# amoretti86/phylo

Measured on AMD Instinct MI355X. Metric: particle-site-likelihoods/sec, higher is better.
Workload: dtype f64; 1 GPU; primate.p N=12 S=898, GTR-init (jcmodel=false), K=2048 per GPU (K_total=2048), lambda=10, full sweep of 11 rank events; parallelism=particles sharded over 1 GPU(s), global resampling, sweeps_per_launch_set=16, contexts_in_flight=3, sweeps_in_flight=48, particles_in_flight=98304

## Files before the change

include/phylo_hip.h:

```cpp
#ifndef PHYLO_HIP_H
#define PHYLO_HIP_H

#include <stdint.h>

#ifdef __cplusplus
extern "C" {
#endif

typedef struct phylo_ctx phylo_ctx;

enum {
    PHYLO_OK = 0,
    PHYLO_EINVAL = -1,
    PHYLO_ENODEVICE = -2,
    PHYLO_EHIP = -3,
    PHYLO_ENOMEM = -4,
    PHYLO_ECOMM = -5,
    PHYLO_ESTATE = -6
};

enum {
    PHYLO_QUIRK_Q1_RAW_Q = 1u << 0,
    PHYLO_TWISTING = 1u << 1,
    PHYLO_TIME_KERNELS = 1u << 2,
// ... 31 lines not shown
                    const double* lam_r, int jc69_closed_form);

int phylo_expm_batched(phylo_ctx* ctx, const double* t, int n, double* P_nx4x4);

int phylo_cond_likelihood_K(phylo_ctx* ctx, const double* l_KxSx4, const double* r_KxSx4,
                            const double* tl_K, const double* tr_K, int K, int S, double* out_KxSx4);

int phylo_forest_loglik(phylo_ctx* ctx, const double* core_KxXxSx4, const int32_t* record_KxX, int K,
                        int X, int S, double* out_K);

int phylo_tree_loglik(phylo_ctx* ctx, int n_nodes, int n_leaves, int S, const int32_t* left,
                      const int32_t* right, const double* bl, const double* br, int root,
                      const double* leaves_LxSx4, const double* prior4, double* out_loglik,
                      double* root_data_Sx4);

int phylo_trees_loglik(phylo_ctx* ctx, int T, const int32_t* child, const double* blen, const double* prior4, double* loglik_T,
                       double* site_lik_TxS, phylo_stats* perf);
int phylo_trees_loglik_rates(phylo_ctx* ctx, int T, const int32_t* child, const double* blen, int C, const double* rate_C,
                             const double* weight_C, const double* prior4, double* loglik_T, double* site_lik_TxS,
                             double* cat_lik_TxCxS, phylo_stats* perf);
int phylo_trees_grad(phylo_ctx* ctx, int T, const int32_t* child, const double* blen, const double* prior4, double* loglik_T,
                     double* grad, double* curv, phylo_stats* perf);
int phylo_trees_grad_rates(phylo_ctx* ctx, int T, const int32_t* child, const double* blen, int C, const double* rate,
                           const double* weight, int per_tree, const double* prior4, double* loglik_T, double* grad, double* curv,
                           double* drate_TxC, double* dweight_TxC, phylo_stats* perf);
int phylo_trees_nni(phylo_ctx* ctx, int T, const int32_t* child, const double* blen, const double* prior4, double* loglik_T,
                    double* delta, phylo_stats* perf);
int phylo_trees_nni_rates(phylo_ctx* ctx, int T, const int32_t* child, const double* blen, int C, const double* rate,
                          const double* weight, int per_tree, const double* prior4, double* loglik_T, double* delta, phylo_stats* perf);
int phylo_debug_tree_schedule(int N, const int32_t* child, const double* blen, int32_t* ops, int32_t* depth);

int phylo_resample(phylo_ctx* ctx, const double* logw_K, int K, uint64_t seed, uint32_t step,
                   int64_t* idx_K);

int phylo_log_zsmc(phylo_ctx* ctx, const double* logw_RxK, int R, int K, double* out);

int phylo_sweep(phylo_ctx* ctx, uint64_t seed, uint32_t flags, int M, double* log_weights,
                double* log_lik, double* lbranch, double* rbranch, int32_t* merges, int64_t* ancestors,
                double* logZ, phylo_stats* perf);

int phylo_sweep_async(phylo_ctx* ctx, uint64_t seed, uint32_t flags, int M);
int phylo_sweep_fetch(phylo_ctx* ctx, double* log_weights, double* log_lik, double* lbranch,
                      double* rbranch, int32_t* merges, int64_t* ancestors, double* logZ,
                      phylo_stats* perf);
int phylo_synchronize(phylo_ctx* ctx);

int phylo_sweep_batch_async(phylo_ctx* ctx, const uint64_t* seeds, int G, uint32_t flags);
int phylo_sweep_batch_begin(phylo_ctx* ctx, const uint64_t* seeds, int G, uint32_t flags);
int phylo_sweep_fetch_logz(phylo_ctx* ctx, double* logZ_G, int G);

int phylo_sweep_begin(phylo_ctx* ctx, uint64_t seed, uint32_t flags, int M);
int phylo_sweep_step(phylo_ctx* ctx);
int phylo_sweep_step_a(phylo_ctx* ctx);
int phylo_sweep_step_group(phylo_ctx** ctxs, int n);
int phylo_sweep_finish(phylo_ctx* ctx);

int phylo_sweep_node(phylo_ctx* ctx, int r, int k, double* out_Sx4);

int phylo_sweep_backward(phylo_ctx* ctx, double* d_lam_l, double* d_lam_r, double* d_pi, double* d_Q,
                         phylo_stats* perf);
int phylo_sweep_backward_batch(phylo_ctx* ctx, double* d_lam_l, double* d_lam_r, double* d_pi, double* d_Q, int G,
                               phylo_stats* perf);

int phylo_vi_gradients(phylo_ctx* ctx, uint64_t seed, uint32_t flags, int M, int jc, const double* vars, double* logZ, double* grads,
                       phylo_stats* fwd, phylo_stats* bwd);
int phylo_vi_gradients_batch(phylo_ctx* ctx, const uint64_t* seeds, int G, uint32_t flags, int jc, const double* vars, double* logZ,
                             double* grads, phylo_stats* fwd, phylo_stats* bwd);
int phylo_vi_apply(int n_taxa, int jc, double* vars, const double* grads, int kind, double lr, double beta1, double beta2, double eps,
                   int64_t* t, double* m, double* v);

int phylo_debug_stamps(phylo_ctx* ctx, uint64_t* out, int n);

int phylo_debug_reverse_lists(int N, int K, const int64_t* ancestors, const int32_t* child, int early_free, int rows_form,
                              const int32_t* lookahead_nodes, int n_lookahead, int32_t* lists, int64_t n_lists, int32_t* meta,
                              int n_meta);

int phylo_debug_lookahead_lists(int N, int K, int S, int M, const int32_t* roots_ad, int32_t* slow_flag, int32_t* image,
                                int64_t n_image, int32_t* meta, int n_meta);

int phylo_debug_reverse_plan(int N, int K, int K_local, int S, int world, int twisted, int marks, uint32_t switches, int64_t n_slow,
                             int TS, int64_t coeff_wgs, int passes_in_flight, uint32_t* mask);
int phylo_debug_sweep_plan(int N, int K, int K_local, int S, int G, int M, int world, int transport, uint32_t flags, uint32_t switches,
                           uint32_t* mask, int32_t* launches);
int phylo_debug_scan_form(phylo_ctx* ctx, int Kg, int multi_min, int wanted);
int phylo_debug_persist_plan(int N, int K, int S, int G, uint32_t flags, uint32_t switches, int world, int transport, int n_cus,
                             int blocks_per_cu, int persist_wgs, int persist_nt, int64_t* out);
int phylo_debug_persist_of(phylo_ctx* ctx, int32_t* nt, int32_t* Wg, int32_t* m, int64_t* lds);
int phylo_debug_pack_leaf_codes(const uint8_t* codes, int N, int S, uint8_t* packed, int64_t cap, int64_t* need);
int phylo_debug_site_patterns(const uint8_t* codes, int N, int S, int32_t* U, int32_t* rep, uint16_t* image, uint32_t* rep_off,
                              uint8_t* rep_leaf, int64_t rep_leaf_cap);
int phylo_debug_site_patterns_rule(int S, int U, int coded, int ntiles, int sw);
int phylo_debug_site_patterns_of(phylo_ctx* ctx, int32_t* U, int32_t* taken);
int phylo_debug_reverse_plan_batch(int N, int K, int G, int S, uint32_t switches, int64_t n_slow, int TS, int64_t coeff_wgs,
                                   int passes_in_flight, uint32_t* mask);
int phylo_debug_tree_plan(int N, int K, int G, int world, int64_t n_clades, int64_t n_topologies, int kept_whole, int force_wide,
                          int64_t summary_temp, int64_t branches_temp, int64_t* scalars, int64_t* summary_slab, int64_t* branches_slab,
                          int32_t* sort_bits, int32_t* launches);
int phylo_debug_tree_branches_of(phylo_ctx* ctx, int32_t* wide, int32_t* cbits, int32_t* tbits);

int phylo_debug_device_lists(phylo_ctx* ctx, int32_t* lists, int64_t n_lists, int32_t* meta, int n_meta, int64_t* ancestors,
                             int32_t* child);
int phylo_debug_device_lists_of(phylo_ctx* ctx, const int64_t* ancestors, const int32_t* child, int32_t* lists, int64_t n_lists,
                                int32_t* meta, int n_meta);

int phylo_tree_summary(phylo_ctx* ctx, int64_t* n_clades, int32_t* n_topologies, int32_t* n_groups, phylo_stats* perf);
int phylo_tree_summary_fetch(phylo_ctx* ctx, uint64_t* clade_bits, uint64_t* clade_weight, int32_t* clade_group, uint64_t* topo_weight,
                             int32_t* topo_count, int32_t* topo_rep, int32_t* topo_group, int32_t* particle_topo, uint64_t* u, uint64_t* U);

int phylo_tree_branches(phylo_ctx* ctx, phylo_stats* perf);
int phylo_tree_branches_fetch(phylo_ctx* ctx, double* clade_stats, double* leaf_stats, int32_t* topo_clades, double* topo_stats);

int phylo_rell(phylo_ctx* ctx, int T, int S, const double* site_lik_TxS, int B, uint64_t seed, double* obs_T, int32_t* best_B,
               int64_t* wins_T, double* rep_loglik_TxB, int32_t* counts_BxS, double* site_loglik_TxS, phylo_stats* perf);
int phylo_debug_rell_host(int T, int S, const double* site_lik_TxS, int b0, int nB, uint64_t seed, int32_t* counts, double* x,
                          double* rl);

int phylo_math_probe(phylo_ctx* ctx, int op, const double* x, const double* y, int n, double* out);

int phylo_debug_frechet(phylo_ctx* ctx, int form, const double* A_nx16, const double* E_nx16, int n, double* L_nx16);

int phylo_debug_site_product(phylo_ctx* ctx, const double* p, const double* x1, const double* x2, int n, double* out_p, int32_t* out_E,
                             double* out_extra);

#define PHYLO_COMM_ID_BYTES 128
int phylo_comm_unique_id(char id[PHYLO_COMM_ID_BYTES]);
int phylo_comm_init(phylo_ctx* ctx, int rank, int world, const char id[PHYLO_COMM_ID_BYTES]);
int phylo_comm_share(phylo_ctx* ctx, phylo_ctx* owner);
int phylo_comm_allgather(phylo_ctx* ctx, const void* mine, size_t bytes, void* all);
int phylo_comm_max(phylo_ctx* ctx, double* value);
int phylo_comm_barrier(phylo_ctx* ctx);
int phylo_comm_exchange_kind(const phylo_ctx* ctx);
int phylo_debug_remote_cache(phylo_ctx* ctx, int* used, int* cap);

#ifdef __cplusplus
}
#endif
#endif
```

phylo_amd/_ffi.py:

```python
from __future__ import annotations

import ctypes as C
import os

import numpy as np

_HERE = os.path.dirname(os.path.abspath(__file__))
LIB_PATH = os.path.join(_HERE, "csrc", "libphylo_hip.so")

PHYLO_OK = 0
QUIRK_Q1_RAW_Q = 1 << 0
TWISTING = 1 << 1
TIME_KERNELS = 1 << 2
EAGER_NODES = 1 << 3
KEEP_GRAPH = 1 << 4
ONE_LAUNCH = 1 << 5
FLAGS_DEFAULT = QUIRK_Q1_RAW_Q
COMM_ID_BYTES = 128

EXPORTS = [
    "phylo_version", "phylo_last_error", "phylo_device_count", "phylo_create", "phylo_destroy",
    "phylo_set_leaves", "phylo_set_model", "phylo_expm_batched", "phylo_cond_likelihood_K",
    "phylo_forest_loglik", "phylo_tree_loglik", "phylo_trees_loglik", "phylo_trees_loglik_rates", "phylo_trees_grad", "phylo_trees_grad_rates", "phylo_trees_nni", "phylo_trees_nni_rates", "phylo_rell", "phylo_debug_rell_host", "phylo_debug_tree_schedule", "phylo_resample", "phylo_log_zsmc", "phylo_sweep",
    "phylo_sweep_async", "phylo_sweep_batch_async", "phylo_sweep_batch_begin", "phylo_sweep_fetch_logz", "phylo_sweep_begin", "phylo_sweep_step", "phylo_sweep_step_a", "phylo_sweep_step_group", "phylo_sweep_finish", "phylo_sweep_fetch",
    "phylo_synchronize", "phylo_sweep_node", "phylo_sweep_backward", "phylo_sweep_backward_batch",
    "phylo_tree_summary", "phylo_tree_summary_fetch", "phylo_tree_branches", "phylo_tree_branches_fetch",
    "phylo_math_probe", "phylo_debug_frechet", "phylo_debug_stamps", "phylo_debug_reverse_lists", "phylo_debug_lookahead_lists", "phylo_debug_reverse_plan", "phylo_debug_reverse_plan_batch", "phylo_debug_sweep_plan", "phylo_debug_pack_leaf_codes", "phylo_debug_site_patterns", "phylo_debug_site_patterns_rule", "phylo_debug_site_patterns_of", "phylo_debug_tree_plan", "phylo_debug_tree_branches_of", "phylo_debug_scan_form", "phylo_debug_persist_plan", "phylo_debug_persist_of", "phylo_debug_device_lists", "phylo_debug_device_lists_of", "phylo_debug_remote_cache", "phylo_debug_site_product",
    "phylo_vi_gradients", "phylo_vi_gradients_batch", "phylo_vi_apply",
    "phylo_site_tile", "phylo_set_site_tile", "phylo_get_site_tile",
    "phylo_comm_unique_id", "phylo_comm_init", "phylo_comm_share", "phylo_comm_allgather", "phylo_comm_max", "phylo_comm_barrier",
    "phylo_comm_exchange_kind",
]


class PhyloError(RuntimeError):
    def __init__(self, code, msg):
        super().__init__("libphylo_hip error %d: %s" % (code, msg))
        self.code = code


class Stats(C.Structure):
    _fields_ = [("sweep_ms", C.c_double), ("merge_ms", C.c_double), ("merge_launches", C.c_int32),
                ("n_launches", C.c_int32), ("units", C.c_double), ("alg_bytes", C.c_double)]


_lib = None


def load():
    global _lib
    if _lib is None:
        if not os.path.exists(LIB_PATH):
            raise OSError("%s not found: build it with phylo_amd/csrc/build.sh (needs hipcc); "
                          "there is no CPU fallback" % LIB_PATH)
        lib = C.CDLL(LIB_PATH)
        lib.phylo_version.restype = C.c_char_p
        lib.phylo_last_error.restype = C.c_char_p
        lib.phylo_last_error.argtypes = [C.c_void_p]
        _lib = lib
    return _lib


def _ptr(a):
    return None if a is None else a.ctypes.data_as(C.c_void_p)


def _f64(a):
    return np.ascontiguousarray(a, dtype=np.float64)


def debug_reverse_lists(N, K, ancestors, child, early_free=True, rows_form=True, lookahead_nodes=None):
    lib = load()
    R = N - 1
    nn = R * K
    cap = 2 * nn // 4 + 1
    n_lists = R * (K + 1) + 9 * nn + 1 + 2 * cap
    lists = np.zeros(n_lists, dtype=np.int32)
    meta = np.zeros(6 + 3 * (R + 1), dtype=np.int32)
    anc = None if R < 2 else np.ascontiguousarray(ancestors, dtype=np.int64)
    ch = np.ascontiguousarray(child, dtype=np.int32)
    la = None if lookahead_nodes is None or len(lookahead_nodes) == 0 else np.ascontiguousarray(lookahead_nodes, dtype=np.int32)
    rc = lib.phylo_debug_reverse_lists(C.c_int(N), C.c_int(K), _ptr(anc), _ptr(ch), C.c_int(int(early_free)), C.c_int(int(rows_form)),
                                       _ptr(la), C.c_int(0 if la is None else la.size), _ptr(lists), C.c_int64(n_lists), _ptr(meta),
                                       C.c_int(meta.size))
    if rc:
        raise PhyloError(rc, lib.phylo_last_error(None).decode())
    return _lists_dict(lists, meta, R, K)


def debug_lookahead_lists(N, K, S, M, roots_ad, slow_flag=None):
    lib = load()
    R = N - 1
    rad = np.ascontiguousarray(roots_ad, dtype=np.int32)
    if rad.shape != (R, K, N):
        raise ValueError("roots_ad must be [N-1][K][N]")
    flag = np.zeros(R * K, dtype=np.int32) if slow_flag is None else np.array(slow_flag, dtype=np.int32).reshape(R * K)
    n_image = R * (8 * K * N + 8192) + 1
    image = np.zeros(n_image, dtype=np.int32)
    meta = np.zeros(4 + 2 * (R + 1), dtype=np.int32)
    rc = lib.phylo_debug_lookahead_lists(C.c_int(N), C.c_int(K), C.c_int(S), C.c_int(M), _ptr(rad), _ptr(flag), _ptr(image),
                                         C.c_int64(n_image), _ptr(meta), C.c_int(meta.size))
    if rc:
        raise PhyloError(rc, lib.phylo_last_error(None).decode())
    ne, nc, nx = int(meta[0]), int(meta[1]), int(meta[2])
    out = {"n_xent": ne, "n_xchunks": nc, "n_xnodes": nx, "tw_max_chunks": int(meta[3]), "slow_flag": flag,
           "ev_chunk0": meta[4:4 + R + 1].copy(), "ev_node0": meta[4 + R + 1:4 + 2 * (R + 1)].copy()}
    o = 0
    for name, n in (("xent", ne), ("xchunk_node", nc), ("xchunk_beg", nc), ("xchunk_cnt", nc), ("xchunk_part", nc), ("xnode_id", nx),
                    ("xnode_chunk0", nx), ("xnode_nchunks", nx)):
        out[name] = image[o:o + n].copy()
        o += n
    return out


PLAN_BITS = ("rows_form", "whole", "early_free", "dev_lists", "sort_early", "bg_free", "two", "parents_first", "rows_all", "rows_overlap",
             "chunks_first", "interleave", "coeff_all")
PLAN_SWITCHES = ("rev_host_lists", "one_stream", "two_streams", "rows_chain", "coeff_chain")


def debug_reverse_plan(N, K, S, K_local=None, world=1, twisted=False, marks=True, switches=(), n_slow=0, TS=None, coeff_wgs=0,
                       passes_in_flight=1):
    lib = load()
    sw = sum(1 << PLAN_SWITCHES.index(name) for name in switches)
    mask = C.c_uint32(0)
    rc = lib.phylo_debug_reverse_plan(C.c_int(N), C.c_int(K), C.c_int(K if K_local is None else K_local), C.c_int(S), C.c_int(world),
                                      C.c_int(int(twisted)), C.c_int(int(marks)), C.c_uint32(sw), C.c_int64(n_slow),
                                      C.c_int((S + 255) // 256 if TS is None else TS), C.c_int64(coeff_wgs), C.c_int(passes_in_flight),
                                      C.byref(mask))
    if rc:
        raise PhyloError(rc, lib.phylo_last_error(None).decode())
    out = {name: bool(mask.value >> i & 1) for i, name in enumerate(PLAN_BITS)}
    out["mask"] = mask.value
    return out


SWEEP_PLAN_BITS = ("twist", "graph", "timek", "lazy", "shard_form", "replicated_book", "local_book", "book_mat", "mat_by_draws", "want_rdraw",
                   "use_rec", "sorted_prologue", "mat_grouped", "mat_draws_grouped", "step_a_work", "mat_after_book", "mat_barrier",
                   "fix_rootll", "fold_logz", "no_store_last", "final_missing", "last_graph_eager", "one_tile", "twist_ll", "twist_tables",
                   "tile_epilogue", "batched")
SWEEP_PLAN_SWITCHES = ("eager_nodes", "rehearse_sharded", "replicated_book", "jc", "coded_leaves", "device_exchange")


def debug_sweep_plan(N, K, S, K_local=None, G=1, M=1, world=1, transport=False, flags=0, switches=()):
    lib = load()
    sw = sum(1 << SWEEP_PLAN_SWITCHES.index(name) for name in switches)
    mask = C.c_uint32(0)
    launches = (C.c_int32 * (max(N, 1) + 1))()
    rc = lib.phylo_debug_sweep_plan(C.c_int(N), C.c_int(K), C.c_int(K if K_local is None else K_local), C.c_int(S), C.c_int(G), C.c_int(M),
                                    C.c_int(world), C.c_int(int(transport)), C.c_uint32(flags), C.c_uint32(sw), C.byref(mask), launches)
    if rc:
        raise PhyloError(rc, lib.phylo_last_error(None).decode())
    out = {name: bool(mask.value >> i & 1) for i, name in enumerate(SWEEP_PLAN_BITS)}
    out["book_width"] = (mask.value >> 28) * 8
    out["mask"] = mask.value
    out["launches"] = list(launches)
    return out


def debug_pack_leaf_codes(codes):
    lib = load()
    cd = np.ascontiguousarray(codes, dtype=np.uint8)
    if cd.ndim != 2:
        raise ValueError("codes must be [N][S]")
    N, S = cd.shape
    need = C.c_int64(0)
    rc = lib.phylo_debug_pack_leaf_codes(_ptr(cd), C.c_int(N), C.c_int(S), None, C.c_int64(0), C.byref(need))
    if rc:
        raise PhyloError(rc, lib.phylo_last_error(None).decode())
    out = np.full(need.value, 0xff, dtype=np.uint8)
    rc = lib.phylo_debug_pack_leaf_codes(_ptr(cd), C.c_int(N), C.c_int(S), _ptr(out), C.c_int64(out.size), C.byref(need))
    if rc:
        raise PhyloError(rc, lib.phylo_last_error(None).decode())
    return out.reshape(N, -1, 64, 16)


SITE_PATTERN_SWITCH = {"0": 0, None: 1, "force": 2}


def debug_site_patterns(codes):
    lib = load()
    cd = np.ascontiguousarray(codes, dtype=np.uint8)
    if cd.ndim != 2:
        raise ValueError("codes must be [N][S]")
    N, S = cd.shape
    nC = -(-(-(-S // 64)) // 16)
    U = C.c_int32(0)
    rep = np.full(S, -1, dtype=np.int32)
    image = np.full(nC * 1024, 0xffff, dtype=np.uint16)
    rep_off = np.full(1024, 0xffffffff, dtype=np.uint32)
    rep_leaf = np.full(N * 1024, 0xff, dtype=np.uint8)
    rc = lib.phylo_debug_site_patterns(_ptr(cd), C.c_int(N), C.c_int(S), C.byref(U), _ptr(rep), _ptr(image), _ptr(rep_off), _ptr(rep_leaf),
                                       C.c_int64(rep_leaf.size))
    if rc:
        raise PhyloError(rc, lib.phylo_last_error(None).decode())
    u = U.value
    return {"U": u, "rep": rep[:u].copy(), "image": image.reshape(nC, 2, 64, 8) if u <= 8191 else None,
            "rep_off": rep_off if u <= 512 else None,
            "rep_leaf": rep_leaf[:N * 1024 * (-(-(-(-u // 64)) // 16))].reshape(N, -1, 64, 16) if u <= 512 else None}


def debug_site_patterns_rule(S, U, coded=True, ntiles=1, switch=None):
    lib = load()
    rc = lib.phylo_debug_site_patterns_rule(C.c_int(S), C.c_int(U), C.c_int(int(coded)), C.c_int(ntiles), C.c_int(SITE_PATTERN_SWITCH[switch]))
    if rc < 0:
        raise PhyloError(rc, lib.phylo_last_error(None).decode())
    return bool(rc)


TREE_SUMMARY_BUFS = ("u", "U", "bits", "kA", "kB", "val", "scan", "weight", "srt", "hp", "o_cbits", "o_cw", "o_tw", "child", "slot", "o_cg",
                     "o_tn", "o_trep", "o_tg", "o_ptopo", "vA", "vB", "flag", "sid", "cid", "seg_start", "count", "group", "first", "tid", "pos",
                     "err", "vC", "vD", "temp")
TREE_BRANCHES_BUFS = ("ebr", "lbr", "gbl", "gbr", "o_cs", "o_ls", "o_ts", "wA", "wB", "cpos", "kA", "kB", "vA", "vB", "cstart", "toff", "o_tc",
                      "temp")


def debug_tree_plan(N, K, G=1, world=1, n_clades=1, n_topologies=1, kept_whole=False, summary_temp=0, branches_temp=0, force_wide=False):
    lib = load()
    ns, nb = len(TREE_SUMMARY_BUFS), len(TREE_BRANCHES_BUFS)
    sc = (C.c_int64 * 13)()
    ss, bs = (C.c_int64 * (2 * ns + 1))(), (C.c_int64 * (2 * nb + 1))()
    bits, launches = (C.c_int32 * 17)(), (C.c_int32 * 2)()
    rc = lib.phylo_debug_tree_plan(C.c_int(N), C.c_int(K), C.c_int(G), C.c_int(world), C.c_int64(n_clades), C.c_int64(n_topologies),
                                   C.c_int(int(kept_whole)), C.c_int(int(force_wide)), C.c_int64(summary_temp), C.c_int64(branches_temp),
                                   sc, ss, bs, bits, launches)
    if rc:
        raise PhyloError(rc, lib.phylo_last_error(None).decode())
    out = dict(zip(("R", "L", "W", "E", "Emax", "Kg", "cbits", "tbits"), sc[:8]))
    out["wide"], out["gather"] = bool(sc[8]), bool(sc[9])
    if (sc[11], sc[12]) != (ns, nb):
        raise RuntimeError("TREE_SUMMARY_BUFS / TREE_BRANCHES_BUFS do not name the library's buffers")
    for key, names, a in (("summary_slab", TREE_SUMMARY_BUFS, ss), ("branches_slab", TREE_BRANCHES_BUFS, bs)):
        n = len(names)
        out[key] = {"offsets": dict(zip(names, a[:n])), "sizes": dict(zip(names, a[n:2 * n])), "total": a[2 * n]}
    out["sort_bits"] = list(bits[:sc[10]])
    out["summary_launches"], out["branches_launches"] = launches[0], launches[1]
    return out


SCAN_FORMS = ("multi", "lds512", "lds1024", "in_place")
# ... 539 lines not shown
                                                       _ptr(z), _ptr(grads), C.byref(fwd), C.byref(bwd)))
        self._last_batch = G
        return z, grads, fwd, bwd

    def debug_device_lists(self, ancestors=None, child=None):
        R, K = self.N - 1, self.K
        nn = R * K
        cap = 2 * nn // 4 + 1
        n_lists = R * (K + 1) + 9 * nn + 1 + 2 * cap
        lists = np.zeros(n_lists, dtype=np.int32)
        meta = np.zeros(6 + 3 * (R + 1), dtype=np.int32)
        if child is not None:
            anc = np.ascontiguousarray(ancestors if R > 1 else np.zeros((0, K)), dtype=np.int64).reshape(max(R - 1, 0), K)
            child = np.ascontiguousarray(child, dtype=np.int32).reshape(R, K, 2)
            self._check(self._lib.phylo_debug_device_lists_of(self._h, _ptr(anc) if R > 1 else None, _ptr(child), _ptr(lists),
                                                              C.c_int64(n_lists), _ptr(meta), C.c_int(meta.size)))
        else:
            anc = np.zeros((max(R - 1, 0), K), dtype=np.int64)
            child = np.zeros((R, K, 2), dtype=np.int32)
            self._check(self._lib.phylo_debug_device_lists(self._h, _ptr(lists), C.c_int64(n_lists), _ptr(meta), C.c_int(meta.size),
                                                           _ptr(anc) if R > 1 else None, _ptr(child)))
        out = _lists_dict(lists, meta, R, K)
        out['ancestors'] = anc
        out['child'] = child
        return out

    def debug_stamps(self):
        out = np.zeros((self.N, 16), dtype=np.uint64)
        self._check(self._lib.phylo_debug_stamps(self._h, _ptr(out), C.c_int(out.size)))
        return out

    def comm_init(self, rank, world, comm_id):
        buf = C.create_string_buffer(bytes(comm_id), COMM_ID_BYTES)
        self._check(self._lib.phylo_comm_init(self._h, C.c_int(rank), C.c_int(world), buf))
        self.K_local = self.K // world
        self.k0 = rank * self.K_local

    def comm_share(self, owner):
        self._check(self._lib.phylo_comm_share(self._h, owner._h))
        self._owner = owner
        world = owner.K // owner.K_local
        self.K_local = self.K // world
        self.k0 = (owner.k0 // owner.K_local) * self.K_local

    def comm_allgather_columns(self, a):
        a = np.ascontiguousarray(a)
        world = self.K // self.K_local
        if world == 1:
            return a
        out = np.empty((world,) + a.shape, dtype=a.dtype)
        self._check(self._lib.phylo_comm_allgather(self._h, _ptr(a), C.c_size_t(a.nbytes), _ptr(out)))
        return np.concatenate(list(out), axis=-1)

    def comm_allgather_blob(self, a):
        a = np.ascontiguousarray(a)
        world = self.K // self.K_local
        if world == 1:
            return a[None]
        out = np.empty((world,) + a.shape, dtype=a.dtype)
        self._check(self._lib.phylo_comm_allgather(self._h, _ptr(a), C.c_size_t(a.nbytes), _ptr(out)))
        return out

    def debug_remote_cache(self):
        used, cap = C.c_int(0), C.c_int(0)
        self._check(self._lib.phylo_debug_remote_cache(self._h, C.byref(used), C.byref(cap)))
        return used.value, cap.value

    def debug_site_patterns(self):
        U, taken = C.c_int32(0), C.c_int32(0)
        self._check(self._lib.phylo_debug_site_patterns_of(self._h, C.byref(U), C.byref(taken)))
        return U.value, bool(taken.value)

    def debug_tree_branches(self):
        wide, cbits, tbits = C.c_int32(0), C.c_int32(0), C.c_int32(0)
        self._check(self._lib.phylo_debug_tree_branches_of(self._h, C.byref(wide), C.byref(cbits), C.byref(tbits)))
        return {'wide': bool(wide.value), 'cbits': cbits.value, 'tbits': tbits.value}

    def debug_scan_form(self, Kg, wanted=True):
        rc = self._lib.phylo_debug_scan_form(self._h, C.c_int(Kg), C.c_int(0), C.c_int(int(wanted)))
        if rc < 0:
            raise PhyloError(rc, self._lib.phylo_last_error(self._h).decode())
        return SCAN_FORMS[rc]

    def debug_persist(self):
        nt, Wg, m, lds = C.c_int32(0), C.c_int32(0), C.c_int32(0), C.c_int64(0)
        self._check(self._lib.phylo_debug_persist_of(self._h, C.byref(nt), C.byref(Wg), C.byref(m), C.byref(lds)))
        return {'nt': nt.value, 'Wg': Wg.value, 'm': m.value, 'lds': lds.value}

    def comm_exchange_kind(self):
        return ('none', 'rccl', 'hostshm', 'p2p')[int(self._lib.phylo_comm_exchange_kind(self._h))]

    def comm_max(self, value):
        v = C.c_double(float(value))
        self._check(self._lib.phylo_comm_max(self._h, C.byref(v)))
        return v.value

    def comm_barrier(self):
        self._check(self._lib.phylo_comm_barrier(self._h))


def sweep_step_group(ctxs):
    arr = (C.c_void_p * len(ctxs))(*[c._h for c in ctxs])
    rc = load().phylo_sweep_step_group(arr, C.c_int(len(ctxs)))
    if rc != PHYLO_OK:
        raise PhyloError(rc, (load().phylo_last_error(None) or b"").decode())


def comm_unique_id():
    buf = C.create_string_buffer(COMM_ID_BYTES)
    rc = load().phylo_comm_unique_id(buf)
    if rc != PHYLO_OK:
        raise PhyloError(rc, (load().phylo_last_error(None) or b"").decode())
    return buf.raw
```

phylo_amd/csrc/phylo_hip.hip:

```cpp
#include "../../include/phylo_hip.h"

#include <cstring>
#include <hip/hip_runtime.h>
#include <hip/hip_ext.h>
#include <rocprim/device/device_radix_sort.hpp>

#include <cstdarg>
#include <cstdio>
#include <cstdlib>
#include <atomic>
#include <chrono>
#include <mutex>
#include <string>
#include <vector>

#include "phylo_comm.h"
#include "phylo_kernels.h"
#include "phylo_packed_codes.h"
#include "phylo_site_patterns.h"
#include "phylo_persist.h"
#include "phylo_grad.h"
#include "phylo_revlists_dev.h"
#include "phylo_sweep_plan.h"
#include "phylo_train.h"
#include "phylo_trees.h"
#include "phylo_trees_plan.h"
#include "phylo_treeset.h"
#include "phylo_rell.h"
#include "phylo_treegrad.h"
#include "phylo_treegrad_rates.h"
#include "phylo_treenni.h"
#include "phylo_treenni_rates.h"

#include <algorithm>
#include <type_traits>

namespace {

thread_local std::string g_last_error;

struct DevBuf {
    void* p = nullptr;
    size_t bytes = 0;
};

}

struct sweep_run {
    uint64_t seed = 0;
    uint32_t flags = 0;
    int M = 1, launches = 0, next_r = 0;
    bool active = false;
    int a_done_r = -1;
    sweep_plan plan{};
};

struct env_switches {
    bool eager_nodes = false, rehearse_sharded = false, replicated_book = false, no_leaf_codes = false, one_launch = false,
         persist_stamps = false, grad_one_stream = false, grad_two_streams = false, rev_host_lists = false, no_remote_cache = false,
         no_p2p = false, grad_rows_chain = false, grad_coeff_chain = false, tree_wide_keys = false;
    int persist_wgs = 0;
    unsigned long long p2p_wait_ticks = PK_P2P_WAIT_TICKS;
    size_t p2p_copy_words = 65536;
    int persist_nt = 256;
    int remote_cache_cap = 0;
    int scan_multi_min = 4096;
    int site_patterns = PK_PAT_AUTO;
    int trees_chunk = 0;
    int rell_chunk = 0;
    void read() {
        eager_nodes = getenv("PHYLO_EAGER_NODES") != nullptr;
        rehearse_sharded = getenv("PHYLO_REHEARSE_SHARDED") != nullptr;
        replicated_book = getenv("PHYLO_REPLICATED_BOOK") != nullptr;
        grad_rows_chain = getenv("PHYLO_GRAD_ROWS_CHAIN") != nullptr;
        grad_coeff_chain = getenv("PHYLO_GRAD_COEFF_CHAIN") != nullptr;
        no_leaf_codes = getenv("PHYLO_NO_LEAF_CODES") != nullptr;
        one_launch = getenv("PHYLO_ONE_LAUNCH") != nullptr;
        persist_stamps = getenv("PHYLO_PERSIST_STAMPS") != nullptr;
        grad_one_stream = getenv("PHYLO_GRAD_ONE_STREAM") != nullptr;
        grad_two_streams = getenv("PHYLO_GRAD_TWO_STREAMS") != nullptr;
        rev_host_lists = getenv("PHYLO_REV_HOST_LISTS") != nullptr;
        no_remote_cache = getenv("PHYLO_NO_REMOTE_CACHE") != nullptr;
        { const char* e = getenv("PHYLO_TREE_WIDE_KEYS"); tree_wide_keys = e && atoi(e) != 0; }
        { const char* e = getenv("PHYLO_REMOTE_CACHE_CAP"); remote_cache_cap = e ? atoi(e) : 0; }
        { const char* e = getenv("PHYLO_SITE_PATTERNS"); site_patterns = !e ? PK_PAT_AUTO : !strcmp(e, "force") ? PK_PAT_FORCE : atoi(e) == 0 ? PK_PAT_OFF : PK_PAT_AUTO; }
        { const char* e = getenv("PHYLO_SCAN_MULTI_MIN"); scan_multi_min = e ? atoi(e) : 4096; }
        { const char* e = getenv("PHYLO_TREES_CHUNK"); trees_chunk = e ? atoi(e) : 0; }
        { const char* e = getenv("PHYLO_RELL_CHUNK"); rell_chunk = e ? atoi(e) : 0; }
        { const char* e = getenv("PHYLO_P2P"); no_p2p = e && atoi(e) == 0; }
        { const char* e = getenv("PHYLO_P2P_COPY_WORDS"); p2p_copy_words = e ? (size_t)atol(e) : 65536; }
        { const char* e = getenv("PHYLO_P2P_WAIT_S"); p2p_wait_ticks = e && atof(e) > 0 ? (unsigned long long)(atof(e) * 1e8) : PK_P2P_WAIT_TICKS; }
        const char* w = getenv("PHYLO_PERSIST_WGS");
        persist_wgs = w ? atoi(w) : 0;
        const char* t = getenv("PHYLO_PERSIST_NT");
        persist_nt = persist_nt_of(t ? atoi(t) : 0);
    }
};

struct phylo_ctx {
    int device = 0;
    env_switches env;
    int n_cus = 0;
    unsigned long long* d_rdraw = nullptr;
    unsigned long long* d_pctr = nullptr;
    unsigned long long pctr_base = 0;
    int pctr_Wg = 0, pctr_G = 0;
    bool pctr_dirty = false;
    int persist_blocks_per_cu = -1;
    bool last_persistent = false;
    int last_pp_nt = 0, last_pp_Wg = 0, last_pp_m = 0;
    size_t last_pp_lds = 0;
    unsigned long long* d_stamps = nullptr;
    int K = 0, N = 0, S = 0, A = 4;
    int Kloc = 0, k0 = 0;
    int rank = 0, world = 1;
    uint32_t flags = 0;
    hipStream_t stream = nullptr;
    hipEvent_t ev0 = nullptr, ev1 = nullptr;
    std::vector<hipEvent_t> kev;
    std::string err;
    bool have_leaves = false, have_model = false, swept = false, state_ready = false;
    int jc = 0;
    std::vector<double> h_lam_l, h_lam_r, h_ldf;
    double *d_Q = nullptr, *d_pi = nullptr, *d_lam_l = nullptr, *d_lam_r = nullptr, *d_ldf = nullptr;
    double* d_leaves = nullptr;
    uint8_t* d_leaf_codes = nullptr;
    uint8_t* d_leaf_packed = nullptr;
    uint8_t* d_pat = nullptr;
    int pat_U = 0;
    bool leaves_coded = false;
    uint32_t* d_pair_hist = nullptr;
    bool hist_ready = false, codes_valid = false;
    double* d_pool = nullptr;
    double* d_nodell = nullptr;
    double *d_bl = nullptr, *d_br = nullptr, *d_Pmat = nullptr;
    double *d_logw = nullptr, *d_ll = nullptr;
    double* d_aux = nullptr;
    unsigned long long* d_rec = nullptr;
    int tile_override = 0;
    int site_tile = 0, ntiles = 1;
    double* d_tilev = nullptr;
    double* d_lse = nullptr;
    uint64_t* d_group_seeds = nullptr;
    char* d_tables = nullptr;
    int32_t *d_roots[2] = {nullptr, nullptr}, *d_cnt[2] = {nullptr, nullptr};
    double* d_rootll[2] = {nullptr, nullptr};
    const char** d_tab_ptrs = nullptr;
    int32_t* d_child = nullptr;
    unsigned int* d_mark = nullptr;
    double* d_sync = nullptr;
    bool p2p = false;
    char* d_xslab = nullptr;
    size_t xslab_bytes = 0, x_flag_off[2] = {0, 0};
    char** d_xslab_ptrs = nullptr;
    unsigned long long x_epoch[2] = {0, 0};
    bool last_lazy = false;
    bool leaves_newer = false;
    int32_t* d_merges = nullptr;
    int64_t* d_anc = nullptr;
    uint64_t* d_cdf[2] = {nullptr, nullptr};
    unsigned int* d_counter = nullptr;
    const double** d_pool_ptrs = nullptr;
    int32_t* d_mirror = nullptr;
    double* d_cache = nullptr;
    int cache_cap = 0;
    int32_t *d_roots_ad = nullptr, *d_cnt_ad = nullptr;
    double *d_rootll_ad = nullptr, *d_chosen = nullptr, *d_tw_b = nullptr, *d_tw_P = nullptr, *d_pot = nullptr;
    size_t tw_capacity = 0;
    double* d_twbuf = nullptr;
    size_t twbuf_cap = 0;
    double *d_htw_b = nullptr, *d_htw_P = nullptr, *d_hpot = nullptr, *d_hchosen = nullptr;
    int32_t* d_hroots_ad = nullptr;
    double *d_tau = nullptr, *d_ctw = nullptr, *d_twpart = nullptr, *d_twnode = nullptr;
    int64_t* d_joff = nullptr;
    size_t htw_rows = 0;
    std::vector<int64_t> h_joff;
    bool last_graph_twist = false, last_graph_marks = false;
    bool last_graph_eager = false;
    int last_M = 1;
    int32_t *d_hroots = nullptr, *d_hcnt = nullptr, *d_pos = nullptr;
    double* d_hrootll = nullptr;
    double *d_adj = nullptr, *d_om = nullptr, *d_G = nullptr, *d_C = nullptr, *d_part = nullptr, *d_nodeg = nullptr;
    double *d_leafpi = nullptr, *d_leafterm = nullptr, *d_terms = nullptr, *d_gout = nullptr;
    int32_t *d_ad_off = nullptr, *d_ad_idx = nullptr, *d_par_off = nullptr, *d_par_idx = nullptr;
    int32_t *d_heavy = nullptr, *d_chunk_beg = nullptr, *d_chunk_cnt = nullptr;
    int32_t *d_slow_flag = nullptr, *d_slow_idx = nullptr, *d_adp = nullptr;
    bool graph_ready = false, last_graph = false;
    int last_G = 1;
    bool last_final_missing = false;
    std::vector<uint64_t> h_group_seeds;
    int64_t* h_anc_p = nullptr;
    std::vector<int64_t> h_anc_glob;
    std::vector<double> h_gout;
    double* h_model_p = nullptr;
    double* h_leaves_p = nullptr;
    hipEvent_t ev_leaves = nullptr;
    uint32_t *h_pub = nullptr, *hd_pub = nullptr;
    int32_t *h_dlmeta = nullptr, *hd_dlmeta = nullptr;
    const int32_t* d_dlmeta = nullptr;
    unsigned int* d_row_done = nullptr;
    unsigned int row_epoch = 0;
    hipEvent_t ev_dl = nullptr;
    size_t dl_temp_p = 0, dl_temp_nn = 0;
    hipGraphExec_t dl_graph = nullptr;
    const void* dl_graph_key[4] = {nullptr, nullptr, nullptr, nullptr};
    bool dl_no_graph = false;
    uint32_t *hd_csr = nullptr, *hd_anc = nullptr, *hd_child = nullptr, *hd_rad = nullptr;
    int32_t *h_child_p = nullptr, *h_rad_p = nullptr, *h_csr_p = nullptr;
    size_t h_csr_cap = 0;
    hipEvent_t ev_gcopy = nullptr;
    std::vector<int32_t> h_cur;
    std::vector<double> h_vi_lam;
    std::vector<double> h_vi_raw;
    int32_t* d_gchild = nullptr;
    double *d_gbl = nullptr, *d_gbr = nullptr, *d_gPmat = nullptr;
    int64_t* d_ganc = nullptr;
    unsigned long long* d_gx = nullptr;
    const unsigned long long** d_gx_src = nullptr;
    size_t gx_seg = 0, gx_cl = 0;
    std::vector<int32_t> h_xlists;
    hipEvent_t evb0 = nullptr, evb1 = nullptr, ev_model = nullptr;
    hipStream_t gstream = nullptr;
    hipEvent_t ev_gfork = nullptr, ev_gjoin = nullptr, ev_gup = nullptr;
    hipStream_t bgstream = nullptr;
    hipEvent_t ev_bgfork = nullptr, ev_bgdone = nullptr;
    std::vector<hipEvent_t> ev_coeff;
    phylo_stats stats{};
    sweep_run run;
    int n_merge_events = 0;
    DevBuf scratch[20];
    phylo_comm comm;
    pt_bufs ts;
    bool ts_done = false;
    int ts_G = 1, ts_nt = 0;
    long long ts_nc = 0;
    hipEvent_t ev_ts0 = nullptr, ev_ts1 = nullptr;
    pb_bufs tb;
    bool tb_done = false;
    int tb_wide = -1, tb_cbits = 0, tb_tbits = 0;
    unsigned long long sweep_serial = 0, ts_serial = 0;
    hipEvent_t ev_tb0 = nullptr, ev_tb1 = nullptr;
    hipEvent_t ev_tl0 = nullptr, ev_tl1 = nullptr;
    hipEvent_t ev_rl0 = nullptr, ev_rl1 = nullptr;
// ... 67 lines not shown
}

int launch_check(phylo_ctx* ctx, const char* what) {
    hipError_t e = hipGetLastError();
    if (e != hipSuccess) return fail(ctx, PHYLO_EHIP, "launch of %s failed: %s", what, hipGetErrorString(e));
    return PHYLO_OK;
}

void free_sweep_state(phylo_ctx* c) {
    if (c->gstream) (void)hipStreamSynchronize(c->gstream);
    if (c->bgstream) (void)hipStreamSynchronize(c->bgstream);
    if (c->d_xslab) {
        (void)hipFree(c->d_xslab);
        c->d_xslab = nullptr;
        c->d_logw = c->d_ll = c->d_nodell = c->d_sync = nullptr;
        c->d_chosen = nullptr;
    }
    if (c->d_xslab_ptrs) (void)hipFree((void*)c->d_xslab_ptrs);
    c->d_xslab_ptrs = nullptr;
    c->xslab_bytes = 0;
    c->x_epoch[0] = c->x_epoch[1] = 0;
    if (c->d_twbuf) (void)hipFree(c->d_twbuf);
    c->d_twbuf = nullptr;
    c->twbuf_cap = 0;
    void* tw[] = {c->d_roots_ad, c->d_cnt_ad, c->d_rootll_ad, c->d_chosen, c->d_tw_b, c->d_tw_P, c->d_pot};
    for (void* p : tw)
        if (p) (void)hipFree(p);
    c->d_roots_ad = c->d_cnt_ad = nullptr;
    c->d_rootll_ad = c->d_chosen = c->d_tw_b = c->d_tw_P = c->d_pot = nullptr;
    c->tw_capacity = 0;
    void* ht[] = {c->d_htw_b, c->d_htw_P, c->d_hpot, c->d_hchosen, c->d_hroots_ad, c->d_tau, c->d_ctw, c->d_twpart, c->d_twnode, c->d_joff};
    for (void* p : ht)
        if (p) (void)hipFree(p);
    c->d_htw_b = c->d_htw_P = c->d_hpot = c->d_hchosen = c->d_tau = c->d_ctw = c->d_twpart = c->d_twnode = nullptr;
    c->d_hroots_ad = nullptr;
    c->d_joff = nullptr;
    c->htw_rows = 0;
    c->last_graph_twist = false;
    void* gr[] = {c->d_hroots, c->d_hcnt, c->d_pos, c->d_hrootll, c->d_adj, c->d_om, c->d_G, c->d_C, c->d_part, c->d_nodeg,
                  c->d_leafpi, c->d_leafterm, c->d_terms, c->d_gout, c->d_ad_off, c->d_gchild, c->d_gbl, c->d_gbr, c->d_gPmat,
                  c->d_ganc, c->d_gx, (void*)c->d_gx_src};
    for (void* p : gr)
        if (p) (void)hipFree(p);
    c->d_hroots = c->d_hcnt = c->d_pos = nullptr;
    c->d_hrootll = c->d_adj = c->d_om = c->d_G = c->d_C = c->d_part = c->d_nodeg = nullptr;
    c->d_leafpi = c->d_leafterm = c->d_terms = c->d_gout = nullptr;
    c->d_gchild = nullptr; c->d_gbl = c->d_gbr = c->d_gPmat = nullptr; c->d_ganc = nullptr;
    c->d_gx = nullptr; c->d_gx_src = nullptr; c->gx_seg = c->gx_cl = 0;
    c->d_ad_off = c->d_ad_idx = c->d_par_off = c->d_par_idx = nullptr;
    c->d_heavy = c->d_chunk_beg = c->d_chunk_cnt = nullptr;
    c->d_slow_flag = c->d_slow_idx = c->d_adp = nullptr;
    if (c->h_csr_p) (void)hipHostFree(c->h_csr_p);
    if (c->h_anc_p) (void)hipHostFree(c->h_anc_p);
    if (c->h_child_p) (void)hipHostFree(c->h_child_p);
    if (c->h_rad_p) (void)hipHostFree(c->h_rad_p);
    if (c->h_pub) (void)hipHostFree(c->h_pub);
    if (c->d_row_done) (void)hipFree(c->d_row_done);
    c->d_row_done = nullptr;
    if (c->h_dlmeta) (void)hipHostFree(c->h_dlmeta);
    c->h_dlmeta = c->hd_dlmeta = nullptr;
    if (c->ev_dl) (void)hipEventDestroy(c->ev_dl);
    c->ev_dl = nullptr;
    if (c->dl_graph) (void)hipGraphExecDestroy(c->dl_graph);
    c->dl_graph = nullptr;
    c->h_pub = c->hd_pub = nullptr;
    c->h_csr_p = c->h_child_p = c->h_rad_p = nullptr;
    c->h_anc_p = nullptr;
    if (c->ev_gcopy) (void)hipEventDestroy(c->ev_gcopy);
    c->ev_gcopy = nullptr;
    c->graph_ready = false;
    c->last_graph = false;
    if (c->d_stamps) (void)hipFree(c->d_stamps);
    c->d_stamps = nullptr;
    if (c->d_rdraw) (void)hipFree(c->d_rdraw);
    if (c->d_pctr) (void)hipFree(c->d_pctr);
    c->d_rdraw = c->d_pctr = nullptr;
    c->pctr_base = 0;
    c->pctr_Wg = c->pctr_G = 0;
    c->pctr_dirty = false;
    if (c->d_tilev) (void)hipFree(c->d_tilev);
    c->d_tilev = nullptr;
    void* ptrs[] = {c->d_pool, c->d_nodell, c->d_bl, c->d_br, c->d_Pmat, c->d_logw, c->d_ll, c->d_aux, c->d_lse, c->d_group_seeds,
                    c->d_tables, (void*)c->d_tab_ptrs, c->d_child, c->d_merges, c->d_anc,
                    c->d_cdf[0], c->d_cdf[1], c->d_counter, (void*)c->d_pool_ptrs, c->d_mark, c->d_sync, c->d_mirror, c->d_cache, c->d_rec};
    for (void* p : ptrs)
        if (p) (void)hipFree(p);
    c->d_pool = c->d_nodell = c->d_bl = c->d_br = c->d_Pmat = c->d_logw = c->d_ll = c->d_aux = c->d_lse = nullptr;
    c->d_group_seeds = nullptr;
    c->d_rec = nullptr;
    c->d_roots[0] = c->d_roots[1] = c->d_cnt[0] = c->d_cnt[1] = c->d_child = c->d_merges = nullptr;
    c->d_anc = nullptr;
    c->d_cdf[0] = c->d_cdf[1] = nullptr;
    c->d_counter = nullptr;
    c->d_rootll[0] = c->d_rootll[1] = nullptr;
    c->d_tables = nullptr;
    c->d_tab_ptrs = nullptr;
    c->d_pool_ptrs = nullptr;
    c->d_mark = nullptr;
    c->d_sync = nullptr;
    c->d_mirror = nullptr;
    c->d_cache = nullptr;
    c->cache_cap = 0;
}

int alloc_sweep_state(phylo_ctx* c) {
    free_sweep_state(c);
    c->state_ready = false;
    const size_t R = (size_t)c->N - 1, K = c->K, Kl = c->Kloc, N = c->N, S = c->S;
    CHK(dalloc(c, &c->d_pool, R * Kl * S * 4));
    c->p2p = c->comm.transport != 0 && c->world > 1 && !c->env.no_p2p && R >= 2;
    if (c->p2p) {
        const size_t al = 32;
        auto up = [&](size_t n) { return (n + al - 1) / al * al; };
        const size_t n_logw = up(R * K), n_nod = up(N + R * K), n_ch = up(K), n_sy = up((size_t)c->world), n_fl = up((size_t)c->world);
        const size_t total = 2 * n_logw + n_nod + n_ch + n_sy + 2 * n_fl;
        void* slab = nullptr;
        if (hipExtMallocWithFlags(&slab, total * 8, hipDeviceMallocFinegrained) != hipSuccess) {
            (void)hipGetLastError();
            HIPCHK(c, hipMalloc(&slab, total * 8));
        }
        HIPCHK(c, hipMemset(slab, 0, total * 8));
        c->d_xslab = (char*)slab;
        c->xslab_bytes = total * 8;
        double* base = (double*)slab;
        c->d_logw = base; c->d_ll = base + n_logw; c->d_nodell = base + 2 * n_logw;
        c->d_chosen = c->d_nodell + n_nod;
        c->d_sync = c->d_chosen + n_ch;
        c->x_flag_off[0] = (size_t)((char*)(c->d_sync + n_sy) - c->d_xslab);
        c->x_flag_off[1] = c->x_flag_off[0] + n_fl * 8;
        c->x_epoch[0] = c->x_epoch[1] = 0;
    } else {
    CHK(dalloc(c, &c->d_nodell, N + R * K));
    }
    CHK(dalloc(c, &c->d_bl, R * Kl));
    CHK(dalloc(c, &c->d_br, R * Kl));
    CHK(dalloc(c, &c->d_Pmat, R * Kl * 32));
    if (!c->p2p) {
        CHK(dalloc(c, &c->d_logw, R * K));
        CHK(dalloc(c, &c->d_ll, R * K));
    }
    CHK(dalloc(c, &c->d_aux, Kl * PK_AUX));
    CHK(dalloc(c, &c->d_rec, Kl * PK_REC));
    if (c->ntiles > 1) CHK(dalloc(c, &c->d_tilev, Kl * (size_t)c->ntiles));
    CHK(dalloc(c, &c->d_lse, (R + 1) * PK_MAX_GROUPS));
    CHK(dalloc(c, &c->d_group_seeds, PK_MAX_GROUPS));
    CHK(dalloc(c, &c->d_tables, 32 * K * N));
    for (int i = 0; i < 2; ++i) {
        c->d_rootll[i] = reinterpret_cast<double*>(c->d_tables) + (size_t)i * K * N;
        c->d_roots[i] = reinterpret_cast<int32_t*>(c->d_tables + 16 * K * N) + (size_t)i * K * N;
        c->d_cnt[i] = reinterpret_cast<int32_t*>(c->d_tables + 24 * K * N) + (size_t)i * K * N;
    }
    CHK(dalloc(c, &c->d_child, R * Kl * 2));
    CHK(dalloc(c, &c->d_mark, ((R * K + R + 3) & ~(size_t)3)));
    if (!c->p2p) CHK(dalloc(c, &c->d_sync, (size_t)c->world));
    CHK(dalloc(c, &c->d_merges, R * Kl * 2));
    CHK(dalloc(c, &c->d_anc, (R > 0 ? R - 1 : 0) * Kl));
    CHK(dalloc(c, &c->d_cdf[0], K));
    CHK(dalloc(c, &c->d_cdf[1], K));
    CHK(dalloc(c, &c->d_counter, ((size_t)N + 3) & ~(size_t)3));
    HIPCHK(c, hipMemset(c->d_counter, 0, (((size_t)N + 3) & ~(size_t)3) * sizeof(unsigned int)));
    CHK(dalloc(c, &c->d_pool_ptrs, (size_t)c->world));
    std::vector<void*> ptrs;
    int rc = phylo_comm_map_pools(c->comm, c->d_pool, &ptrs, c->stream, &c->err);
    if (rc != PHYLO_OK) return rc;
    HIPCHK(c, hipMemcpy((void*)c->d_pool_ptrs, ptrs.data(), ptrs.size() * sizeof(void*), hipMemcpyHostToDevice));
    if ((c->world > 1 || c->env.rehearse_sharded) && !c->env.no_remote_cache) {
        const size_t node_bytes = (size_t)S * 32;
        size_t cap = ((size_t)512 << 20) / node_bytes;
        if (c->env.remote_cache_cap > 0) cap = (size_t)c->env.remote_cache_cap;
        if (cap > R * K) cap = R * K;
        if (cap < 1) cap = 1;
        c->cache_cap = (int)cap;
        CHK(dalloc(c, &c->d_mirror, R * K + 4));
        CHK(dalloc(c, &c->d_cache, cap * (size_t)S * 4));
    }
    CHK(dalloc(c, &c->d_tab_ptrs, (size_t)c->world));
    rc = phylo_comm_map_extra(c->comm, c->d_tables, &ptrs, c->stream, &c->err);
    if (rc != PHYLO_OK) return rc;
    HIPCHK(c, hipMemcpy((void*)c->d_tab_ptrs, ptrs.data(), ptrs.size() * sizeof(void*), hipMemcpyHostToDevice));
    if (c->p2p) {
        CHK(dalloc(c, &c->d_xslab_ptrs, (size_t)c->world));
        rc = phylo_comm_map_extra(c->comm, c->d_xslab, &ptrs, c->stream, &c->err);
        if (rc != PHYLO_OK) return rc;
        HIPCHK(c, hipMemcpy((void*)c->d_xslab_ptrs, ptrs.data(), ptrs.size() * sizeof(void*), hipMemcpyHostToDevice));
    }
    c->state_ready = true;
    return PHYLO_OK;
}

int ensure_sweep_state(phylo_ctx* c) {
    if (c->state_ready) return PHYLO_OK;
    return alloc_sweep_state(c);
}

int ensure_graph_state(phylo_ctx* c) {
    if (c->graph_ready) return PHYLO_OK;
    const size_t R = (size_t)c->N - 1, K = c->K, N = c->N, S = c->S;
    const size_t T = (S + PG_NT - 1) / PG_NT;
    CHK(dalloc(c, &c->d_hroots, (R + 1) * K * N));
    CHK(dalloc(c, &c->d_hcnt, (R + 1) * K * N));
    CHK(dalloc(c, &c->d_hrootll, (R + 1) * K * N));
    CHK(dalloc(c, &c->d_pos, R * K * N));
    CHK(dalloc(c, &c->d_adj, R * K * S * 4));
    CHK(dalloc(c, &c->d_om, R * K));
    CHK(dalloc(c, &c->d_G, R * K));
    CHK(dalloc(c, &c->d_C, R * K * N));
    CHK(dalloc(c, &c->d_part, R * K * T * PG_PART));
    CHK(dalloc(c, &c->d_nodeg, R * K * PG_NODEG));
    CHK(dalloc(c, &c->d_leafpi, N * 4));
    CHK(dalloc(c, &c->d_leafterm, K * 4));
    CHK(dalloc(c, &c->d_terms, R * K * 2));
    CHK(dalloc(c, &c->d_gout, (2 * R + 21) * PK_MAX_GROUPS));
    {
        c->h_csr_cap = pg_lists_ints(R, K);
        CHK(dalloc(c, &c->d_ad_off, c->h_csr_cap));
        HIPCHK(c, hipHostMalloc((void**)&c->h_csr_p, c->h_csr_cap * 4));
        HIPCHK(c, hipHostMalloc((void**)&c->h_anc_p, (R > 1 ? (R - 1) * K : 1) * 8));
        HIPCHK(c, hipHostMalloc((void**)&c->h_child_p, R * K * 2 * 4));
        HIPCHK(c, hipHostGetDevicePointer((void**)&c->hd_csr, c->h_csr_p, 0));
        HIPCHK(c, hipHostGetDevicePointer((void**)&c->hd_anc, c->h_anc_p, 0));
        HIPCHK(c, hipHostGetDevicePointer((void**)&c->hd_child, c->h_child_p, 0));
        HIPCHK(c, hipHostMalloc((void**)&c->h_pub, 16));
        HIPCHK(c, hipHostGetDevicePointer((void**)&c->hd_pub, c->h_pub, 0));
        HIPCHK(c, hipEventCreateWithFlags(&c->ev_gcopy, hipEventDisableTiming));
        HIPCHK(c, hipHostMalloc((void**)&c->h_dlmeta, ((size_t)PG_DL_META_INTS(R) + 4) * 4));
        c->h_dlmeta[PG_DL_META_INTS(R)] = 0;
        HIPCHK(c, hipHostGetDevicePointer((void**)&c->hd_dlmeta, c->h_dlmeta, 0));
        HIPCHK(c, hipEventCreateWithFlags(&c->ev_dl, hipEventDisableTiming));
        c->dl_temp_nn = 0;
        const pg_lists D = pg_lists_carve(c->d_ad_off, R, K);
        c->d_ad_idx = D.ad_idx; c->d_par_off = D.par_off; c->d_par_idx = D.par_idx;
        c->d_heavy = D.heavy; c->d_chunk_beg = D.chunk_beg; c->d_chunk_cnt = D.chunk_cnt;
        c->d_slow_flag = D.slow_flag; c->d_slow_idx = D.slow_idx; c->d_adp = D.adp;
    }
    if (c->world > 1) {
        const size_t Kl = c->Kloc, W = c->world;
        CHK(dalloc(c, &c->d_gchild, R * K * 2));
        CHK(dalloc(c, &c->d_gbl, R * K));
        CHK(dalloc(c, &c->d_gbr, R * K));
        CHK(dalloc(c, &c->d_gPmat, R * K * 32));
        CHK(dalloc(c, &c->d_ganc, (R > 1 ? R - 1 : 1) * K));
        c->gx_seg = R * Kl * 36 + (R > 1 ? (R - 1) * Kl : 0);
        c->gx_cl = c->gx_seg < PHYLO_SHM_SLOT / 8 ? c->gx_seg : PHYLO_SHM_SLOT / 8;
        const size_t words = (c->gx_seg + c->gx_cl - 1) / c->gx_cl * c->gx_cl * W;
        void* buf = nullptr;
        if (hipExtMallocWithFlags(&buf, words * 8, hipDeviceMallocFinegrained) != hipSuccess) {
            (void)hipGetLastError();
            HIPCHK(c, hipMalloc(&buf, words * 8));
        }
        c->d_gx = (unsigned long long*)buf;
        CHK(dalloc(c, &c->d_gx_src, W));
        std::vector<void*> src(W, buf);
        if (c->p2p) {
            int rc = phylo_comm_map_extra(c->comm, buf, &src, c->stream, &c->err);
            if (rc != PHYLO_OK) return rc;
        }
        HIPCHK(c, hipMemcpy((void*)c->d_gx_src, src.data(), W * sizeof(void*), hipMemcpyHostToDevice));
    }
    if (!c->evb0) {
        HIPCHK(c, hipEventCreate(&c->evb0));
        HIPCHK(c, hipEventCreate(&c->evb1));
        HIPCHK(c, hipStreamCreateWithFlags(&c->gstream, hipStreamNonBlocking));
        HIPCHK(c, hipEventCreateWithFlags(&c->ev_gfork, hipEventDisableTiming));
        HIPCHK(c, hipEventCreateWithFlags(&c->ev_gjoin, hipEventDisableTiming));
        HIPCHK(c, hipEventCreateWithFlags(&c->ev_gup, hipEventDisableTiming));
        {
            int least = 0, greatest = 0;
            HIPCHK(c, hipDeviceGetStreamPriorityRange(&least, &greatest));
            HIPCHK(c, hipStreamCreateWithPriority(&c->bgstream, hipStreamNonBlocking, least));
        }
        HIPCHK(c, hipEventCreateWithFlags(&c->ev_bgfork, hipEventDisableTiming));
        HIPCHK(c, hipEventCreateWithFlags(&c->ev_bgdone, hipEventDisableTiming));
        c->ev_coeff.assign((size_t)R, nullptr);
        for (auto& e : c->ev_coeff) HIPCHK(c, hipEventCreateWithFlags(&e, hipEventDisableTiming));
    }
    c->graph_ready = true;
    return PHYLO_OK;
}

template <typename... P, typename... A>
void launch_stamped(void (*kernel)(P...), dim3 grid, dim3 block, size_t lds, hipStream_t s, hipEvent_t e0, hipEvent_t e1, A&&... args) {
    if (e0) hipExtLaunchKernelGGL(kernel, grid, block, lds, s, e0, e1, 0, args...);
    else hipLaunchKernelGGL(kernel, grid, block, lds, s, args...);
}

static sweep_limits sweep_limits_of() {
    sweep_limits L{};
    L.max_groups = PK_MAX_GROUPS; L.twist_max_m = PK_TWIST_MAX_M; L.twist_max_j = PK_TWIST_MAX_J;
    L.mat_group = PK_MAT_GROUP; L.scan_fold_max_kg = PP_SCAN_KERNEL_MAX_KG; L.kept_bits_taxa = PG_KEPT_BITS_TAXA;
    L.scan_lds512_max_kg = 4096;
    L.one_tile_max_s = 4096;
    L.small_max_kg = 4096; L.small_max_kloc = 8192;
    L.book_packed8_min = 8192;
    L.sorted_min_draws = 262144;
    return L;
}
static const sweep_limits k_sweep_limits = sweep_limits_of();

int launch_scan(phylo_ctx* c, const double* logw, int Kg, int G, uint64_t* cdf, double* lse, int lse_stride, int logz_R = 0) {
    const sweep_scan_form form = sweep_scan_form_of(Kg, c->env.scan_multi_min, cdf || lse, k_sweep_limits);
    if (form == SCAN_MULTI) {
        pp_scan_multi_args a{};
        a.logw = logw; a.Kg = Kg; a.B = (Kg + PP_SCAN_TILE - 1) / PP_SCAN_TILE;
        void* ws = nullptr;
        const size_t nb = (size_t)G * a.B;
        CHK(scratch_get(c, 11, (nb * 2 + (size_t)G * Kg) * 8, &ws));
        a.gmax = (double*)ws; a.bsum = (unsigned long long*)ws + nb; a.wbits = (unsigned long long*)ws + 2 * nb;
        a.cdf = (unsigned long long*)cdf; a.lse_out = lse; a.lse_stride = lse_stride; a.logz_R = logz_R;
        hipLaunchKernelGGL(pp_scan_multi_max, dim3(a.B, G), dim3(512), 0, c->stream, a);
        CHK(launch_check(c, "pp_scan_multi_max"));
        hipLaunchKernelGGL(pp_scan_multi_exp, dim3(a.B, G), dim3(512), 0, c->stream, a);
        CHK(launch_check(c, "pp_scan_multi_exp"));
        if (cdf) hipLaunchKernelGGL(pp_scan_multi_cdf, dim3(a.B + 1, G), dim3(512), 0, c->stream, a);
        else { a.lse_only = 1; hipLaunchKernelGGL(pp_scan_multi_cdf, dim3(1, G), dim3(512), 0, c->stream, a); }
        return launch_check(c, "pp_scan_multi_cdf");
    }
    if (form == SCAN_LDS_512) {
        hipLaunchKernelGGL(pp_resample_scan<512>, dim3(G), dim3(512), pp_resample_scan_lds(Kg), c->stream, logw, Kg, cdf, lse, lse_stride, logz_R);
        return launch_check(c, "pp_resample_scan");
    }
    if (form == SCAN_LDS_1024) {
        const size_t lds = pp_resample_scan_lds(Kg);
        static bool raised = false;
        if (lds > 65536 && !raised) {
            HIPCHK(c, hipFuncSetAttribute((const void*)pp_resample_scan<1024>, hipFuncAttributeMaxDynamicSharedMemorySize,
                                          (int)pp_resample_scan_lds(PP_SCAN_KERNEL_MAX_KG)));
            raised = true;
        }
        hipLaunchKernelGGL(pp_resample_scan<1024>, dim3(G), dim3(1024), lds, c->stream, logw, Kg, cdf, lse, lse_stride, logz_R);
        return launch_check(c, "pp_resample_scan");
    }
    if (G > 1) hipLaunchKernelGGL(pk_resample_scan_groups, dim3(G), dim3(PK_COLS), 0, c->stream, logw, Kg, cdf, lse, lse_stride);
    else hipLaunchKernelGGL(pk_resample_scan, dim3(1), dim3(PK_COLS), 0, c->stream, logw, Kg, cdf, lse);
    return launch_check(c, "pk_resample_scan");
}

int wait_event_spin(phylo_ctx* c, hipEvent_t ev) {
    const auto t0 = std::chrono::steady_clock::now();
    for (;;) {
        const hipError_t e = hipEventQuery(ev);
        if (e == hipSuccess) return PHYLO_OK;
        if (e != hipErrorNotReady) return fail(c, PHYLO_EHIP, "hipEventQuery: %s", hipGetErrorString(e));
        if (std::chrono::steady_clock::now() - t0 > std::chrono::milliseconds(2)) break;
        __builtin_ia32_pause();
    }
    HIPCHK(c, hipEventSynchronize(ev));
    return PHYLO_OK;
}

int tile_for(const phylo_ctx* c, int S) { return c->tile_override ? c->tile_override : pm_site_tile(S); }

int refresh_leaf_ll(phylo_ctx* c) {
    if (!(c->have_leaves && c->have_model && c->state_ready)) return PHYLO_OK;
    hipLaunchKernelGGL(pk_row_loglik, dim3(c->N), dim3(64), 0, c->stream, c->d_leaves, c->d_pi, c->S, c->site_tile,
                       c->d_nodell);
    return launch_check(c, "pk_row_loglik(leaves)");
}

}

extern "C" {

const char* phylo_version(void) { return "phylo_hip 0.1 (gfx950)"; }

const char* phylo_last_error(const phylo_ctx* ctx) { return ctx ? ctx->err.c_str() : g_last_error.c_str(); }

int phylo_device_count(void) {
    int n = 0;
    if (hipGetDeviceCount(&n) != hipSuccess) return 0;
    return n;
}

int phylo_create(const int* device_ids, int n_gpus, int K, int N, int S, int A, uint32_t flags,
                 phylo_ctx** out) {
    if (!out) return fail(nullptr, PHYLO_EINVAL, "out is NULL");
    *out = nullptr;
    if (n_gpus != 1)
        return fail(nullptr, PHYLO_EINVAL, "n_gpus must be 1 (one process per GPU; join ranks with phylo_comm_init)");
    if (A != 4) return fail(nullptr, PHYLO_EINVAL, "A must be 4 (DNA alphabet), got %d", A);
    if (K < 1 || N < 2 || S < 1) return fail(nullptr, PHYLO_EINVAL, "need K >= 1, N >= 2, S >= 1 (K=%d N=%d S=%d)", K, N, S);
    if (N > PK_MAX_TAXA) return fail(nullptr, PHYLO_EINVAL, "N = %d exceeds the supported maximum %d", N, PK_MAX_TAXA);
    if ((double)(N - 1) * K + N > 2.0e9) return fail(nullptr, PHYLO_EINVAL, "node ids overflow int32");
    int ndev = 0;
    hipError_t e = hipGetDeviceCount(&ndev);
    if (e != hipSuccess || ndev < 1)
        return fail(nullptr, PHYLO_ENODEVICE, "no HIP device available (%s); this library has no CPU path",
                    e != hipSuccess ? hipGetErrorString(e) : "device count 0");
    const int dev = device_ids ? device_ids[0] : 0;
    if (dev < 0 || dev >= ndev) return fail(nullptr, PHYLO_ENODEVICE, "device id %d out of range [0,%d)", dev, ndev);
    phylo_ctx* c = new phylo_ctx();
    c->device = dev;
    c->K = K; c->N = N; c->S = S; c->A = A;
    c->Kloc = K; c->k0 = 0;
    c->flags = flags;
    c->env.read();
    {
        const char* t = getenv("PHYLO_SITE_TILE");
        int T = t ? atoi(t) : pm_site_tile(S);
        if (T < 64 || (T & 63) || T > PK_MAX_SITE_TILE) { delete c; return fail(nullptr, PHYLO_EINVAL, "PHYLO_SITE_TILE must be a multiple of 64 in [64, %d] (got %d)", PK_MAX_SITE_TILE, T); }
        c->tile_override = t ? T : 0;
        c->site_tile = T;
        c->ntiles = (S + T - 1) / T;
    }
    int rc = PHYLO_OK;
    do {
        if ((rc = bind(c)) != PHYLO_OK) break;
        {
            hipDeviceProp_t prop;
            if (hipGetDeviceProperties(&prop, dev) != hipSuccess) { rc = fail(c, PHYLO_EHIP, "hipGetDeviceProperties failed"); break; }
            c->n_cus = prop.multiProcessorCount;
// ... 1200 lines not shown
        CHK(dalloc(c, &c->d_hpot, rows));
        CHK(dalloc(c, &c->d_tau, rows));
        CHK(dalloc(c, &c->d_twpart, rows * PG_PART));
        c->htw_rows = rows;
    }
    if (!c->d_hroots_ad) {
        CHK(dalloc(c, &c->d_hroots_ad, (size_t)R * K * N));
        CHK(dalloc(c, &c->d_hchosen, (size_t)R * K));
        CHK(dalloc(c, &c->d_ctw, (size_t)R * K * N));
        CHK(dalloc(c, &c->d_twnode, (size_t)R * K * PG_NODEG));
        CHK(dalloc(c, &c->d_joff, (size_t)R + 1));
        HIPCHK(c, hipHostMalloc((void**)&c->h_rad_p, (size_t)R * K * N * 4));
        HIPCHK(c, hipHostGetDevicePointer((void**)&c->hd_rad, c->h_rad_p, 0));
    }
    HIPCHK(c, hipMemcpyAsync(c->d_joff, c->h_joff.data(), ((size_t)R + 1) * 8, hipMemcpyHostToDevice, c->stream));
    return PHYLO_OK;
}

static int sweep_alloc(phylo_ctx* c, const sweep_plan& p, int M) {
    if (p.twist) CHK(sweep_alloc_twist(c, M));
    while (p.timek && (int)c->kev.size() < 2 * p.R) {
        hipEvent_t e;
        HIPCHK(c, hipEventCreate(&e));
        c->kev.push_back(e);
    }
    if (p.graph) {
        CHK(ensure_graph_state(c));
        if (p.twist) CHK(sweep_alloc_twist_history(c, M));
    }
    if (p.want_rdraw && !c->d_rdraw) CHK(dalloc(c, &c->d_rdraw, (size_t)p.R * c->K));
    return PHYLO_OK;
}

static int sweep_prologue(phylo_ctx* c, const sweep_plan& p, uint64_t seed, const uint64_t* group_seeds) {
    const int N = c->N, K = c->K, Kl = c->Kloc, R = p.R, G = p.G;
    const size_t mark_words = ((size_t)R * K + R + 3) & ~(size_t)3;
    int32_t* t_roots = p.graph ? c->d_hroots : c->d_roots[0];
    int32_t* t_cnt = p.graph ? c->d_hcnt : c->d_cnt[0];
    double* t_rootll = p.graph ? c->d_hrootll : c->d_rootll[0];
    if (!p.twist) {
        if (G > 1) HIPCHK(c, hipMemcpyAsync(c->d_group_seeds, group_seeds, (size_t)G * 8, hipMemcpyHostToDevice, c->stream));
        pk_prologue_args pa{};
        pa.Q = c->d_Q; pa.lam_l = c->d_lam_l; pa.lam_r = c->d_lam_r; pa.jc = c->jc; pa.seed = seed; pa.R = R; pa.Kloc = Kl; pa.k0 = c->k0;
        pa.bl = c->d_bl; pa.br = c->d_br; pa.Pmat = c->d_Pmat; pa.Kg = p.Kg;
        pa.group_seeds = G > 1 ? (const uint64_t*)c->d_group_seeds : (const uint64_t*)nullptr;
        pa.rdraw = p.want_rdraw ? c->d_rdraw : (unsigned long long*)nullptr;
        pa.roots = t_roots; pa.cnt = t_cnt; pa.rootll = t_rootll; pa.nodell = c->d_nodell; pa.K = K; pa.N = N;
        pa.mark = p.lazy ? c->d_mark : (unsigned int*)nullptr;
        pa.mark_words = p.lazy ? (unsigned int)mark_words : 0u;
        const int NT = p.sorted_prologue ? 256 : 64;
        pa.draw_blocks = p.sorted_prologue ? cdiv(2L * R * Kl, PK_DRAW_ITEMS) : cdiv(2L * R * Kl, 64);
        pa.init_blocks = cdiv((long)K * N, 4 * NT);
        pa.mark_blocks = p.lazy ? cdiv((long)mark_words, 4 * NT) : 0;
        const int rdraw_blocks = p.want_rdraw ? cdiv((long)(R - 1) * K, NT) : 0;
        const dim3 pgrid(pa.draw_blocks + pa.init_blocks + pa.mark_blocks + rdraw_blocks);
        if (p.sorted_prologue) hipLaunchKernelGGL(pk_sweep_prologue_sorted, pgrid, dim3(256), 0, c->stream, pa);
        else hipLaunchKernelGGL(pk_sweep_prologue, pgrid, dim3(64), 0, c->stream, pa);
        CHK(launch_check(c, "pk_sweep_prologue"));
    } else {
        if (p.lazy) HIPCHK(c, hipMemsetAsync(c->d_mark, 0, mark_words * sizeof(unsigned int), c->stream));
        hipLaunchKernelGGL(pk_init_tables, dim3(cdiv((long)K * N, 256)), dim3(256), 0, c->stream, t_roots, t_cnt, t_rootll,
                           (const double*)c->d_nodell, K, N);
    }
    CHK(launch_check(c, "pk_init_tables"));
    if (c->d_mirror) HIPCHK(c, hipMemsetAsync(c->d_mirror, 0, ((size_t)R * K + 4) * 4, c->stream));
    return PHYLO_OK;
}

static int sweep_begin_impl(phylo_ctx* c, uint64_t seed, uint32_t flags, int M, const uint64_t* group_seeds, int G) {
    CHK(sweep_bind(c));
    const sweep_facts f = sweep_facts_of(c, flags, M, G);
    char why[160];
    if (sweep_refuses_batch(f, k_sweep_limits, why, sizeof why)) return fail(c, PHYLO_EINVAL, "%s", why);
    CHK(sweep_ready(c));
    if (sweep_refuses_form(f, k_sweep_limits, why, sizeof why)) return fail(c, PHYLO_EINVAL, "%s", why);
    const sweep_plan p = sweep_plan_form(f, k_sweep_limits);
    CHK(sweep_alloc(c, p, M));
    c->swept = false; ++c->sweep_serial;
    HIPCHK(c, hipEventRecord(c->ev0, c->stream));
    CHK(sweep_prologue(c, p, seed, group_seeds));
    c->run = sweep_run{};
    c->run.seed = seed; c->run.flags = flags; c->run.M = M;
    c->run.plan = p;
    c->run.launches = sweep_plan_launches(p, -1);
    c->run.active = true;
    c->last_persistent = false;
    return PHYLO_OK;
}

static std::mutex g_persist_mu;
static hipEvent_t g_persist_done[64] = {};
static int persist_chain(phylo_ctx* c, bool after_launch) {
    std::lock_guard<std::mutex> lock(g_persist_mu);
    if (c->device < 0 || c->device >= 64) return fail(c, PHYLO_EINVAL, "device id out of range for the one-launch sweep");
    hipEvent_t& ev = g_persist_done[c->device];
    if (!after_launch) {
        if (ev) HIPCHK(c, hipStreamWaitEvent(c->stream, ev, 0));
        return PHYLO_OK;
    }
    if (!ev) HIPCHK(c, hipEventCreateWithFlags(&ev, hipEventDisableTiming));
    HIPCHK(c, hipEventRecord(ev, c->stream));
    return PHYLO_OK;
}

static size_t persist_lds_bytes(int N, int m, int Kg) { return pp_layout(N, m, Kg).total; }
static const persist_limits k_persist_limits = {32, PP_MAX_KG, PP_MAX_M, 8192, (size_t)150 * 1024, persist_lds_bytes};

static persist_facts persist_facts_flags(int N, int K, int S, int G, int world, bool transport, uint32_t flags, bool env_one_launch,
                                         bool env_eager_nodes) {
    persist_facts f{};
    f.N = N; f.K = K; f.S = S; f.G = G; f.world = world; f.transport = transport;
    f.one_launch = env_one_launch || (flags & PHYLO_ONE_LAUNCH);
    f.twisting = (flags & PHYLO_TWISTING) != 0; f.keep_graph = (flags & PHYLO_KEEP_GRAPH) != 0;
    f.time_kernels = (flags & PHYLO_TIME_KERNELS) != 0; f.eager_nodes = (flags & PHYLO_EAGER_NODES) != 0;
    f.env_eager_nodes = env_eager_nodes;
    return f;
}

static bool persist_plan(phylo_ctx* c, uint32_t flags, int G, int* Wg_out, int* m_out) {
    persist_facts f = persist_facts_flags(c->N, c->K, c->S, G, c->world, c->comm.transport != 0, flags, c->env.one_launch, c->env.eager_nodes);
    if (persist_refuses_shape(f, k_persist_limits)) return false;
    if (c->persist_blocks_per_cu < 0) {
        int nb = 0;
        const size_t lds = pp_layout(c->N, PP_CHUNK, 2048).total;
        hipError_t e = c->env.persist_nt == 512
            ? hipOccupancyMaxActiveBlocksPerMultiprocessor(&nb, pp_sweep<512>, 512, lds)
            : hipOccupancyMaxActiveBlocksPerMultiprocessor(&nb, pp_sweep<256>, 256, lds);
        c->persist_blocks_per_cu = (e == hipSuccess && nb >= 1) ? (nb >= 3 ? 2 : 1) : 0;
    }
    f.n_cus = c->n_cus; f.blocks_per_cu = c->persist_blocks_per_cu;
    f.persist_wgs = c->env.persist_wgs; f.persist_nt = c->env.persist_nt;
    const persist_grid p = persist_plan_of(f, k_persist_limits);
    if (!p.taken) return false;
    *Wg_out = p.Wg;
    *m_out = p.m;
    return true;
}

static int sweep_persistent(phylo_ctx* c, uint64_t seed, uint32_t flags, const uint64_t* group_seeds, int G, int Wg, int m) {
    CHK(sweep_bind(c));
    CHK(sweep_ready(c));
    const int N = c->N, K = c->K, S = c->S, R = N - 1, Kg = K / G;
    if (!c->d_rdraw) CHK(dalloc(c, &c->d_rdraw, (size_t)R * K));
    if (!c->d_pctr) {
        CHK(dalloc(c, &c->d_pctr, (size_t)PK_MAX_GROUPS * PP_CTR_STRIDE));
        c->pctr_Wg = 0;
    }
    if (c->pctr_Wg != Wg || c->pctr_G != G || c->pctr_dirty) {
        HIPCHK(c, hipMemsetAsync(c->d_pctr, 0, (size_t)PK_MAX_GROUPS * PP_CTR_STRIDE * 8, c->stream));
        c->pctr_base = 0;
        c->pctr_Wg = Wg;
        c->pctr_G = G;
        c->pctr_dirty = false;
    }
    pp_args a{};
    a.N = N; a.S = S; a.K = K; a.Kg = Kg; a.G = G; a.R = R; a.Wg = Wg; a.m = m;
    a.T = c->site_tile;
    a.seed = seed; a.flags = flags; a.jc = c->jc;
    if (G > 1) {
        HIPCHK(c, hipMemcpyAsync(c->d_group_seeds, group_seeds, (size_t)G * 8, hipMemcpyHostToDevice, c->stream));
        a.group_seeds = c->d_group_seeds;
    }
    a.Q = c->d_Q; a.lam_l = c->d_lam_l; a.lam_r = c->d_lam_r; a.pi = c->d_pi; a.ldf = c->d_ldf;
    a.leaves = c->d_leaves; a.leaf_codes = c->leaves_coded ? c->d_leaf_codes : nullptr; a.pool = c->d_pool;
    for (int i = 0; i < 2; ++i) { a.roots[i] = c->d_roots[i]; a.cnt[i] = c->d_cnt[i]; a.rootll[i] = c->d_rootll[i]; }
    a.nodell = c->d_nodell; a.bl = c->d_bl; a.br = c->d_br; a.Pmat = c->d_Pmat; a.logw = c->d_logw; a.ll = c->d_ll;
    a.child = c->d_child; a.merges = c->d_merges; a.anc = c->d_anc; a.mark = c->d_mark;
    a.rdraw = c->d_rdraw;
    a.lse = c->d_lse; a.lse_stride = R + 1;
    a.ctr = c->d_pctr; a.ctr_base = c->pctr_base;
    a.timeout_word = c->d_counter + 1;
    if (c->env.persist_stamps) {
        if (!c->d_stamps) CHK(dalloc(c, &c->d_stamps, (size_t)(R + 1) * PP_NSTAMP));
        a.stamps = c->d_stamps;
    }
    const size_t lds = pp_layout(N, m, Kg).total;
    c->swept = false; ++c->sweep_serial;
    CHK(persist_chain(c, false));
    HIPCHK(c, hipEventRecord(c->ev0, c->stream));
    if (c->env.persist_nt == 512) hipLaunchKernelGGL((pp_sweep<512>), dim3(G * Wg), dim3(512), lds, c->stream, a);
    else hipLaunchKernelGGL((pp_sweep<256>), dim3(G * Wg), dim3(256), lds, c->stream, a);
    CHK(launch_check(c, "pp_sweep"));
    HIPCHK(c, hipEventRecord(c->ev1, c->stream));
    CHK(persist_chain(c, true));
    c->pctr_base += (unsigned long long)R * Wg;
    sweep_publish(c, true, false, G, false, 0, 1, (double)K * S * R);
    c->last_persistent = true;
    c->last_pp_nt = c->env.persist_nt; c->last_pp_Wg = Wg; c->last_pp_m = m; c->last_pp_lds = lds;
    return PHYLO_OK;
}


int phylo_sweep_begin(phylo_ctx* c, uint64_t seed, uint32_t flags, int M) { return sweep_begin_impl(c, seed, flags, M, nullptr, 1); }

static int comm_exchange(phylo_ctx* c, double* const* arrays, int n_arrays, size_t count, int purpose) {
    if (c->comm.transport == 0) return PHYLO_OK;
    if (!c->p2p) {
        if (n_arrays == 0) { double* rows[1] = {c->d_sync}; return phylo_comm_allgather_inplace(c->comm, rows, 1, 1, c->stream, &c->err); }
        return phylo_comm_allgather_inplace(c->comm, arrays, n_arrays, count, c->stream, &c->err);
    }
    if (n_arrays > 4) return fail(c, PHYLO_EINVAL, "comm_exchange: at most four arrays");
    pk_p2p_args a{};
    a.slabs = c->d_xslab_ptrs; a.world = c->world; a.me = c->rank;
    a.n_seg = n_arrays; a.seg_count = (int)count;
    for (int i = 0; i < n_arrays; ++i) {
        const ptrdiff_t off = (const char*)arrays[i] - c->d_xslab;
        if (off < 0 || (size_t)off + (size_t)c->world * count * 8 > c->xslab_bytes) return fail(c, PHYLO_EINVAL, "comm_exchange: array outside the exchange slab");
        a.seg_off[i] = (size_t)off;
    }
    a.flag_off = c->x_flag_off[purpose];
    a.epoch = ++c->x_epoch[purpose];
    a.timeout_word = c->d_counter + 1;
    a.wait_ticks = c->env.p2p_wait_ticks;
    const size_t words = (size_t)n_arrays * count * (size_t)(c->world - 1);
    if (words > c->env.p2p_copy_words) {
        const size_t wgs = (words + 4095) / 4096;
        hipLaunchKernelGGL(pk_p2p_copy, dim3((unsigned)(wgs < 512 ? wgs : 512)), dim3(1024), 0, c->stream, a);
        CHK(launch_check(c, "pk_p2p_copy"));
        a.n_seg = 0;
    }
    hipLaunchKernelGGL(pk_p2p_exchange, dim3(1), dim3(1024), 0, c->stream, a);
    return launch_check(c, "pk_p2p_exchange");
}

static bool pat_on(const phylo_ctx* c) { return pk_pat_take(c->S, c->pat_U, c->leaves_coded, c->ntiles, c->env.site_patterns); }

static pk_rank_args rank_args(const phylo_ctx* c, int r) {
    const sweep_plan& p = c->run.plan;
    const int N = c->N, K = c->K, Kl = c->Kloc, cur = r & 1, nxt = cur ^ 1;
    const size_t plane = (size_t)K * N;
    pk_rank_args b{};
    b.r = r; b.n = N - r; b.N = N; b.S = c->S; b.K = K; b.Kloc = Kl; b.k0 = c->k0;
    b.seed = c->run.seed; b.flags = c->run.flags;
    b.Kg = p.Kg; b.group_seeds = p.G > 1 ? c->d_group_seeds : nullptr;
    b.no_store = (r == p.R - 1 && p.no_store_last) ? 1 : 0;
    if (p.graph) {
        b.roots_old = c->d_hroots + plane * r; b.cnt_old = c->d_hcnt + plane * r;
        b.roots_new = c->d_hroots + plane * (r + 1); b.cnt_new = c->d_hcnt + plane * (r + 1);
        b.rootll_old = c->d_hrootll + plane * r; b.rootll_new = c->d_hrootll + plane * (r + 1);
        b.pos_hist = c->d_pos + plane * r;
    } else {
        b.roots_old = c->d_roots[cur]; b.cnt_old = c->d_cnt[cur];
        b.roots_new = c->d_roots[nxt]; b.cnt_new = c->d_cnt[nxt];
        b.rootll_old = c->d_rootll[cur]; b.rootll_new = c->d_rootll[nxt];
    }
    if (p.local_book) {
        b.tab_ptrs = c->d_tab_ptrs;
        b.tab_off_rootll = (size_t)cur * K * N * 8;
        b.tab_off_roots = (size_t)16 * K * N + (size_t)cur * K * N * 4;
        b.tab_off_cnt = (size_t)24 * K * N + (size_t)cur * K * N * 4;
    }
    b.cdf = c->d_cdf[cur];
    b.rdraw = p.want_rdraw ? c->d_rdraw + (size_t)r * K : nullptr;
    b.ll_prev = r > 0 ? c->d_ll + (size_t)(r - 1) * K : nullptr;
    b.nodell = c->d_nodell;
    b.ldf = c->d_ldf; b.ldf_n = N;
    b.bl = c->d_bl; b.br = c->d_br;
    b.lam_l = c->h_lam_l[r]; b.lam_r = c->h_lam_r[r];
    b.loglam_l = pm_log(b.lam_l); b.loglam_r = pm_log(b.lam_r);
    b.ll_tilde0 = pm_log(1.0 / (double)p.Kg);
    b.leaves = c->d_leaves; b.pool = c->d_pool; b.pool_ptrs = c->d_pool_ptrs;
    b.mirror = (p.twist || p.replicated_book) ? nullptr : c->d_mirror; b.cache = c->d_cache; b.cache_cap = c->cache_cap;
    b.leaf_codes = c->leaves_coded ? c->d_leaf_codes : nullptr;
    b.leaf_packed = c->leaves_coded ? c->d_leaf_packed : nullptr;
    b.packed_leaf_bytes = pk_packed_leaf_bytes(c->S);
    b.Pmat = c->d_Pmat + (size_t)r * Kl * 32;
    b.pi = c->d_pi;
    b.logw_r = c->d_logw + (size_t)r * K;
    b.ll_r = c->d_ll + (size_t)r * K;
    b.merges = c->d_merges; b.ancestors = c->d_anc;
    b.child = c->d_child + (size_t)r * Kl * 2; b.aux = c->d_aux;
    b.rec = p.use_rec ? c->d_rec : nullptr;
    b.lazy = p.lazy ? 1 : 0; b.mark = c->d_mark; b.child_all = c->d_child; b.Pmat_all = c->d_Pmat;
    b.T = c->site_tile; b.ntiles = c->ntiles; b.tilev = c->d_tilev;
    return b;
}

static int step_materialize(phylo_ctx* c, const pk_rank_args& b) {
    const sweep_plan& p = c->run.plan;
    const int Kl = c->Kloc, S = c->S;
    if (p.mat_by_draws) {
        const int grouped = p.mat_draws_grouped ? 1 : 0;
        hipLaunchKernelGGL(pk_materialize_by_draws, dim3(grouped ? Kl / PK_MAT_GROUP : Kl), dim3(PK_COLS), 0, c->stream, b, grouped);
        CHK(launch_check(c, "pk_materialize_by_draws"));
    } else {
        if (p.step_a_work) {
            hipLaunchKernelGGL(pk_all_marks, dim3(cdiv(c->K, 4)), dim3(64), 0, c->stream, b);
            CHK(launch_check(c, "pk_all_marks"));
        }
        if (p.mat_grouped) hipLaunchKernelGGL(pk_materialize_adopted_grouped, dim3(cdiv(Kl, PK_MAT_GROUP)), dim3(PK_COLS), 0, c->stream, b);
        else hipLaunchKernelGGL(pk_materialize_adopted, dim3(p.one_tile ? 1 : cdiv(S, PK_MAT_TILE), Kl), dim3(PK_COLS), 0, c->stream, b);
        CHK(launch_check(c, "pk_materialize_adopted"));
    }
    if (p.mat_barrier) CHK(comm_exchange(c, nullptr, 0, 0, 1));
    return PHYLO_OK;
}

static int sweep_step_a(phylo_ctx* c) {
    CHK(bind(c));
    if (!c->run.active) return fail(c, PHYLO_ESTATE, "phylo_sweep_step without phylo_sweep_begin");
    const int R = c->N - 1, r = c->run.next_r;
    if (r >= R) return fail(c, PHYLO_ESTATE, "all %d rank events of this sweep have been issued", R);
    c->run.a_done_r = r;
    if (!c->run.plan.step_a_work || r == 0) return PHYLO_OK;
    return step_materialize(c, rank_args(c, r));
}

static int step_twist(phylo_ctx* c, const pk_rank_args& b) {
    const sweep_plan& p = c->run.plan;
    const int N = c->N, K = c->K, Kl = c->Kloc, r = b.r;
    pk_twist_args ta{};
    ta.a = b;
    ta.M = c->run.M;
    ta.J = ((N - r) * (N - r - 1) / 2) * ta.M;
    ta.roots_ad = c->d_roots_ad; ta.cnt_ad = c->d_cnt_ad; ta.rootll_ad = c->d_rootll_ad;
    ta.tw_b = c->d_tw_b; ta.tw_P = c->d_tw_P; ta.pot = c->d_pot; ta.chosen = c->d_chosen;
    if (p.graph) {
        const size_t j0 = (size_t)c->h_joff[r];
        ta.tw_b = c->d_htw_b + j0 * 2; ta.tw_P = c->d_htw_P + j0 * 32; ta.pot = c->d_hpot + j0;
        ta.roots_ad = c->d_hroots_ad + (size_t)K * N * r; ta.chosen = c->d_hchosen + (size_t)r * K;
    }
    ta.Pmat_r = c->d_Pmat + (size_t)r * Kl * 32;
    ta.pair_hist = p.twist_ll ? c->d_pair_hist : nullptr;
    ta.codes = p.twist_ll ? c->d_leaf_codes : nullptr;
    ta.bl_r = c->d_bl + (size_t)r * Kl; ta.br_r = c->d_br + (size_t)r * Kl;
    ta.own_tables = p.twist_tables ? 0 : 1;
    ta.wbuf = c->d_twbuf;
    hipLaunchKernelGGL(pk_twist_adopt_draws, dim3(K + cdiv(2L * Kl * ta.J, 64)), dim3(64), 0, c->stream, ta, (const double*)c->d_Q, c->jc);
    CHK(launch_check(c, "pk_twist_adopt_draws"));
    if (p.twist_ll) {
        hipLaunchKernelGGL(pk_twist_potentials_ll, dim3((ta.J + 7) / 8, Kl), dim3(256), 0, c->stream, ta);
        CHK(launch_check(c, "pk_twist_potentials_ll"));
    }
    const bool any_rows = !(p.twist_ll && r == 0);
    const dim3 pgrid((unsigned)((((size_t)Kl * ta.J + 7) / 8) * 8));
    if (p.timek) {
        if (any_rows) hipExtLaunchKernelGGL(pk_twist_potentials, pgrid, dim3(64), 0, c->stream, c->kev[2 * r], c->kev[2 * r + 1], 0, ta);
        else { HIPCHK(c, hipEventRecord(c->kev[2 * r], c->stream)); HIPCHK(c, hipEventRecord(c->kev[2 * r + 1], c->stream)); }
    } else if (any_rows) {
        hipLaunchKernelGGL(pk_twist_potentials, pgrid, dim3(64), 0, c->stream, ta);
    }
    CHK(launch_check(c, "pk_twist_potentials"));
    hipLaunchKernelGGL(pk_twist_choose, dim3(Kl), dim3(64), (size_t)(ta.J <= PK_TWIST_LDS_J ? ta.J : 0) * 8, c->stream, ta);
    CHK(launch_check(c, "pk_twist_choose"));
    if (p.twist_tables) {
        double* rows[1] = {c->d_chosen};
        CHK(comm_exchange(c, rows, 1, (size_t)Kl, 1));
        hipLaunchKernelGGL(pk_twist_tables, dim3(cdiv(K, 128)), dim3(128), 0, c->stream, ta);
        CHK(launch_check(c, "pk_twist_tables"));
    }
    return PHYLO_OK;
}

static int step_book(phylo_ctx* c, const pk_rank_args& b) {
    const sweep_plan& p = c->run.plan;
    const int K = c->K, w = p.book_width;
    const size_t lds = pk_book_lds_bytes(c->N);
    if (p.book_mat && b.r > 0) {
        const int lp = w < 16 ? 16 : w, per = PK_COLS / lp;
        const int bb = cdiv(K, per);
        const dim3 grid(bb + K);
        switch (lp) {
        case 16: hipLaunchKernelGGL(pk_rank_book_mat<16>, grid, dim3(PK_COLS), lds * per, c->stream, b, bb); break;
        case 32: hipLaunchKernelGGL(pk_rank_book_mat<32>, grid, dim3(PK_COLS), lds * per, c->stream, b, bb); break;
        case 64: hipLaunchKernelGGL(pk_rank_book_mat<64>, grid, dim3(PK_COLS), lds * per, c->stream, b, bb); break;
        default: return fail(c, PHYLO_ESTATE, "step_book: no pk_rank_book_mat of %d lanes", lp);
        }
        return launch_check(c, "pk_rank_book_mat");
    }
    const int per = 64 / (w > 0 ? w : 64);
    const dim3 grid(cdiv(p.local_book ? c->Kloc : K, per));
    switch (w) {
    case 8: hipLaunchKernelGGL(pk_rank_book_packed<8>, grid, dim3(64), lds * per, c->stream, b); break;
    case 16: hipLaunchKernelGGL(pk_rank_book_packed<16>, grid, dim3(64), lds * per, c->stream, b); break;
    case 32: hipLaunchKernelGGL(pk_rank_book_packed<32>, grid, dim3(64), lds * per, c->stream, b); break;
    case 64: hipLaunchKernelGGL(pk_rank_book_packed<64>, grid, dim3(64), lds * per, c->stream, b); break;
    default: return fail(c, PHYLO_ESTATE, "step_book: no pk_rank_book_packed of %d lanes", w);
    }
    return launch_check(c, "pk_rank_book_packed");
}

static int step_merge(phylo_ctx* c, const pk_rank_args& b) {
    const sweep_plan& p = c->run.plan;
    const int S = c->S;
    const dim3 mgrid((unsigned)((size_t)c->Kloc * c->ntiles));
    hipEvent_t e0 = nullptr, e1 = nullptr;
    if (p.timek && !p.twist) { e0 = c->kev[2 * b.r]; e1 = c->kev[2 * b.r + 1]; }
    if (!(b.lazy || b.no_store)) {
        const size_t lds = (size_t)(c->site_tile < S ? c->site_tile : S) * 8 + 16 + PK_STORE_STAGE_BYTES;
        launch_stamped(pk_rank_merge, mgrid, dim3(PK_COLS), lds, c->stream, e0, e1, b);
    } else if (b.rec) {
        pk_pi4 pi4;
        memcpy(pi4.v, c->h_model_p + 16, sizeof pi4.v);
        pk_pat_args pat = {nullptr, nullptr, 0, 0};
        size_t lds = 0;
        if (pat_on(c)) {
            pat.pimg = (const char*)c->d_pat;
            pat.roff = (const char*)c->d_pat + pk_pat_image_bytes(S);
            pat.rep_delta = (long long)((c->d_pat + pk_pat_image_bytes(S) + pk_pat_rep_bytes()) - c->d_leaf_packed);
            pat.U = c->pat_U;
            lds = pk_pat_lds_bytes(c->pat_U);
        }
        launch_stamped(pk_rank_merge_nostore, mgrid, dim3(64), lds, c->stream, e0, e1, (const unsigned long long*)b.rec, b.Pmat, S, b.T,
                       b.ntiles, b.tilev, pi4, pat);
    } else {
        launch_stamped(pk_rank_merge_nostore_ids, mgrid, dim3(64), 0, c->stream, e0, e1, b);
    }
    return launch_check(c, "pk_rank_merge");
}

static int step_tiles(phylo_ctx* c, const pk_rank_args& b) {
    hipLaunchKernelGGL(pk_tile_epilogue, dim3(cdiv(c->Kloc, 256)), dim3(256), 0, c->stream, b);
    return launch_check(c, "pk_tile_epilogue");
}

static int step_exchange(phylo_ctx* c, int r) {
    const size_t K = c->K;
    double* rows[3] = {c->d_logw + r * K, c->d_ll + r * K, c->d_nodell + c->N + r * K};
    return comm_exchange(c, rows, 3, (size_t)c->Kloc, 0);
}

static int step_fix_rootll(phylo_ctx* c, int r) {
    const int N = c->N, K = c->K;
    double* rootll_new = c->run.plan.graph ? c->d_hrootll + (size_t)K * N * (r + 1) : c->d_rootll[(r & 1) ^ 1];
    hipLaunchKernelGGL(pk_fix_rootll, dim3(cdiv(K, 256)), dim3(256), 0, c->stream, rootll_new,
                       (const double*)(c->d_nodell + N + (size_t)r * K), K, N, N - r, c->k0, c->Kloc);
    return launch_check(c, "pk_fix_rootll");
}

static int step_scan(phylo_ctx* c, int r) {
    const sweep_plan& p = c->run.plan;
    const bool last = r + 1 == p.R;
    return launch_scan(c, (const double*)(c->d_logw + (size_t)r * c->K), p.Kg, p.G, last ? (uint64_t*)nullptr : c->d_cdf[(r & 1) ^ 1],
                       c->d_lse + r, p.lse_stride, (last && p.fold_logz) ? p.R : 0);
}

static int sweep_step_impl(phylo_ctx* c, int phase) {
    CHK(bind(c));
    if (!c->run.active) return fail(c, PHYLO_ESTATE, "phylo_sweep_step without phylo_sweep_begin");
    const sweep_plan& p = c->run.plan;
    const int r = c->run.next_r;
    if (r >= p.R) return fail(c, PHYLO_ESTATE, "all %d rank events of this sweep have been issued", p.R);
    if (phase != 2) {
        if (c->run.a_done_r != r) CHK(sweep_step_a(c));
        const pk_rank_args b = rank_args(c, r);
        if (p.twist) CHK(step_twist(c, b));
        else CHK(step_book(c, b));
        if (p.mat_after_book && r > 0) CHK(step_materialize(c, b));
        CHK(step_merge(c, b));
        if (p.tile_epilogue) CHK(step_tiles(c, b));
    }
    if (phase == 0) CHK(step_exchange(c, r));
    if (phase == 1) return PHYLO_OK;
    if (p.fix_rootll) CHK(step_fix_rootll(c, r));
    CHK(step_scan(c, r));
    c->run.launches += sweep_plan_launches(p, r);
    ++c->run.next_r;
    return PHYLO_OK;
}

int phylo_sweep_step(phylo_ctx* c) { return sweep_step_impl(c, 0); }

int phylo_sweep_step_a(phylo_ctx* c) { return sweep_step_a(c); }

int phylo_sweep_step_group(phylo_ctx** ctxs, int n) {
    if (!ctxs || n < 1) return fail(nullptr, PHYLO_EINVAL, "phylo_sweep_step_group needs at least one context");
    for (int i = 0; i < n; ++i)
        if (!ctxs[i]) return fail(nullptr, PHYLO_EINVAL, "NULL context");
    if (n == 1 || ctxs[0]->comm.transport == 0) {
        for (int i = 0; i < n; ++i) CHK(sweep_step_impl(ctxs[i], 0));
        return PHYLO_OK;
    }
    for (int i = 0; i < n; ++i) {
        if (!ctxs[i]->run.active || ctxs[i]->run.next_r != ctxs[0]->run.next_r)
            return fail(ctxs[i], PHYLO_ESTATE, "the sweeps of a group must be at the same rank event");
        if (&phylo_comm_link(ctxs[i]->comm) != &phylo_comm_link(ctxs[0]->comm))
            return fail(ctxs[i], PHYLO_EINVAL, "the contexts of a group must share one communicator (phylo_comm_share)");
    }
    for (int i = 0; i < n; ++i) CHK(sweep_step_impl(ctxs[i], 1));
    std::vector<phylo_comm*> comms(n);
    std::vector<double*> rows((size_t)3 * n);
    std::vector<hipStream_t> streams(n);
    for (int i = 0; i < n; ++i) {
        phylo_ctx* c = ctxs[i];
        const size_t r = (size_t)c->run.next_r, K = c->K;
        comms[i] = &c->comm;
        streams[i] = c->stream;
        rows[3 * i] = c->d_logw + r * K;
        rows[3 * i + 1] = c->d_ll + r * K;
        rows[3 * i + 2] = c->d_nodell + c->N + r * K;
    }
    if (ctxs[0]->p2p) {
        for (int i = 0; i < n; ++i) {
            if (!ctxs[i]->p2p) return fail(ctxs[i], PHYLO_EINVAL, "the contexts of a group must use the same exchange");
            CHK(comm_exchange(ctxs[i], rows.data() + 3 * (size_t)i, 3, (size_t)ctxs[i]->Kloc, 0));
        }
    } else {
        phylo_ctx* c0 = ctxs[0];
        std::vector<size_t> counts(n);
        for (int i = 0; i < n; ++i) counts[i] = (size_t)ctxs[i]->Kloc;
        int rc = phylo_comm_allgather_group(comms.data(), rows.data(), 3, counts.data(), streams.data(), n, &c0->err);
        if (rc != PHYLO_OK) { g_last_error = c0->err; return rc; }
    }
    for (int i = 0; i < n; ++i) CHK(sweep_step_impl(ctxs[i], 2));
    return PHYLO_OK;
}

static int graph_gather(phylo_ctx* c) {
    const int K = c->K, Kl = c->Kloc, R = c->N - 1;
    pk_gx_args a{};
    a.world = c->world; a.me = c->rank; a.Kloc = Kl; a.K = K;
    a.seg = c->gx_seg; a.cl = c->gx_cl;
    a.xbuf = c->d_gx; a.xsrc = c->d_gx_src;
    int nf = 0;
    auto field = [&](const void* src, size_t stride, size_t off, void* dst, int rows, int w, int wide) {
        pk_gx_field& f = a.f[nf++];
        f.src = src; f.src_stride = stride; f.src_off = off; f.dst = dst; f.rows = rows; f.w = w; f.wide = wide;
// ... 899 lines not shown
int phylo_debug_reverse_lists(int N, int K, const int64_t* ancestors, const int32_t* child, int early_free, int rows_form,
                              const int32_t* lookahead_nodes, int n_lookahead, int32_t* lists, int64_t n_lists, int32_t* meta, int n_meta) {
    if (N < 2 || K < 1 || !child || !lists || !meta || (N > 2 && !ancestors) || (n_lookahead > 0 && !lookahead_nodes))
        return fail(nullptr, PHYLO_EINVAL, "phylo_debug_reverse_lists: bad arguments");
    const int R = N - 1;
    if (n_lists < (int64_t)pg_lists_ints((size_t)R, (size_t)K) || n_meta < 6 + 3 * (R + 1))
        return fail(nullptr, PHYLO_EINVAL, "phylo_debug_reverse_lists: lists needs %zu ints, meta %d", pg_lists_ints((size_t)R, (size_t)K), 6 + 3 * (R + 1));
    const pg_lists L = pg_lists_carve(lists, (size_t)R, (size_t)K);
    pg_lists_clear(L, R, K);
    std::vector<int32_t> cur;
    pg_list_counts n;
    pg_build_adopters(R, K, ancestors, L, cur, n);
    if (early_free) pg_mark_adopted(R, K, ancestors, L);
    for (int i = 0; i < n_lookahead; ++i) {
        if (lookahead_nodes[i] < N || lookahead_nodes[i] >= N + R * K) return fail(nullptr, PHYLO_EINVAL, "phylo_debug_reverse_lists: node id out of range");
        L.slow_flag[lookahead_nodes[i] - N] |= 2;
    }
    pg_build_parents(N, R, K, child, rows_form != 0, rows_form != 0 && early_free != 0, L, cur, n);
    debug_lists_meta(n, L.cap, R, meta);
    return PHYLO_OK;
}

int phylo_debug_lookahead_lists(int N, int K, int S, int M, const int32_t* roots_ad, int32_t* slow_flag, int32_t* image, int64_t n_image,
                                int32_t* meta, int n_meta) {
    if (N < 2 || K < 1 || S < 1 || M < 1 || !roots_ad || !slow_flag || !image || !meta)
        return fail(nullptr, PHYLO_EINVAL, "phylo_debug_lookahead_lists: bad arguments");
    const int R = N - 1;
    if (n_meta < 4 + 2 * (R + 1)) return fail(nullptr, PHYLO_EINVAL, "phylo_debug_lookahead_lists: meta needs %d ints", 4 + 2 * (R + 1));
    for (int r = 1; r < R; ++r)
        for (int k = 0; k < K; ++k)
            for (int i = 0; i < N - r; ++i) {
                const int32_t x = roots_ad[((size_t)r * K + k) * N + i];
                if (x < 0 || x >= N + r * K) return fail(nullptr, PHYLO_EINVAL, "phylo_debug_lookahead_lists: root id out of range");
            }
    std::vector<int32_t> pk;
    pg_lookahead x;
    pg_build_lookahead(N, K, S, PG_XCH, roots_ad, slow_flag, pk, x);
    if ((int64_t)pk.size() > n_image) return fail(nullptr, PHYLO_EINVAL, "phylo_debug_lookahead_lists: image needs %zu ints", pk.size());
    memcpy(image, pk.data(), pk.size() * 4);
    meta[0] = (int32_t)x.n_xent; meta[1] = (int32_t)x.n_xchunks; meta[2] = (int32_t)x.n_xnodes; meta[3] = (int32_t)x.max_chunks;
    for (int r = 0; r <= R; ++r) {
        meta[4 + r] = x.ev_chunk0[r];
        meta[4 + (R + 1) + r] = x.ev_node0[r];
    }
    return PHYLO_OK;
}

int phylo_debug_reverse_plan(int N, int K, int K_local, int S, int world, int twisted, int marks, uint32_t switches, int64_t n_slow, int TS,
                             int64_t coeff_wgs, int passes_in_flight, uint32_t* mask) {
    if (N < 2 || K < 1 || K_local < 1 || S < 1 || world < 1 || TS < 1 || n_slow < 0 || coeff_wgs < 0 || !mask)
        return fail(nullptr, PHYLO_EINVAL, "phylo_debug_reverse_plan: bad arguments");
    pg_plan_in in{};
    in.N = N; in.K = K; in.K_local = K_local; in.S = S; in.world = world;
    in.twist = twisted != 0; in.marks = marks != 0;
    in.rev_host_lists = switches & 1; in.one_stream = switches & 2; in.two_streams = switches & 4;
    in.rows_chain = switches & 8; in.coeff_chain = switches & 16;
    in.dl_max_k = PG_DL_MAX_K;
    pg_plan p = pg_plan_form(in);
    pg_plan_chains(p, (long)n_slow, TS, (long)coeff_wgs, passes_in_flight, N - 1);
    *mask = pg_plan_mask(p);
    return PHYLO_OK;
}

int phylo_debug_sweep_plan(int N, int K, int K_local, int S, int G, int M, int world, int transport, uint32_t flags, uint32_t switches,
                           uint32_t* mask, int32_t* launches) {
    if (N < 2 || N > PK_MAX_TAXA || K < 1 || K_local < 1 || K_local > K || S < 1 || world < 1 || !mask || !launches)
        return fail(nullptr, PHYLO_EINVAL, "phylo_debug_sweep_plan: bad arguments");
    sweep_facts f{};
    f.N = N; f.K = K; f.Kloc = K_local; f.S = S; f.G = G; f.M = M; f.world = world;
    f.ntiles = (S + pm_site_tile(S) - 1) / pm_site_tile(S);
    f.transport = transport != 0;
    sweep_facts_flags(f, flags);
    f.env_eager_nodes = switches & 1; f.env_rehearse_sharded = switches & 2; f.env_replicated_book = switches & 4;
    f.jc = switches & 8; f.coded_leaves = switches & 16; f.device_exchange = switches & 32;
    char why[160];
    if (sweep_refuses_batch(f, k_sweep_limits, why, sizeof why) || sweep_refuses_form(f, k_sweep_limits, why, sizeof why))
        return fail(nullptr, PHYLO_EINVAL, "%s", why);
    const sweep_plan p = sweep_plan_form(f, k_sweep_limits);
    *mask = sweep_plan_mask(p);
    for (int r = -1; r <= p.R; ++r) launches[r + 1] = sweep_plan_launches(p, r);
    return PHYLO_OK;
}

int phylo_debug_pack_leaf_codes(const uint8_t* codes, int N, int S, uint8_t* packed, int64_t cap, int64_t* need) {
    if (N < 1 || S < 1 || !need || (packed && !codes)) return fail(nullptr, PHYLO_EINVAL, "phylo_debug_pack_leaf_codes: bad arguments");
    *need = (int64_t)pk_packed_bytes(N, S);
    if (!packed) return PHYLO_OK;
    if (cap < *need) return fail(nullptr, PHYLO_EINVAL, "phylo_debug_pack_leaf_codes: the image takes %lld bytes (got %lld)", (long long)*need, (long long)cap);
    pk_pack_leaf_codes(codes, N, S, packed);
    return PHYLO_OK;
}

int phylo_debug_site_patterns(const uint8_t* codes, int N, int S, int32_t* U, int32_t* rep, uint16_t* image, uint32_t* rep_off,
                              uint8_t* rep_leaf, int64_t rep_leaf_cap) {
    if (N < 1 || S < 1 || !codes || !U) return fail(nullptr, PHYLO_EINVAL, "phylo_debug_site_patterns: bad arguments");
    std::vector<int32_t> pat((size_t)S), rp((size_t)S);
    *U = pk_pat_columns(codes, N, S, pat.data(), rp.data());
    if (rep) memcpy(rep, rp.data(), (size_t)*U * sizeof(int32_t));
    if (image && *U <= PK_PAT_IMAGE_MAX_U) pk_pat_pack_image(pat.data(), S, *U, image);
    if (rep_off && *U <= PK_PAT_MAX_U) pk_pat_rep_offsets(rp.data(), *U, rep_off);
    if (rep_leaf && *U <= PK_PAT_MAX_U) {
        if (rep_leaf_cap < (int64_t)pk_packed_bytes(N, *U))
            return fail(nullptr, PHYLO_EINVAL, "phylo_debug_site_patterns: the representative leaf image takes %lld bytes (got %lld)",
                        (long long)pk_packed_bytes(N, *U), (long long)rep_leaf_cap);
        pk_pat_rep_leaf_image(codes, N, S, rp.data(), *U, rep_leaf, pk_packed_leaf_bytes(*U));
    }
    return PHYLO_OK;
}

int phylo_debug_site_patterns_rule(int S, int U, int coded, int ntiles, int sw) {
    if (S < 1 || U < 0 || ntiles < 1 || sw < PK_PAT_OFF || sw > PK_PAT_FORCE) {
        (void)fail(nullptr, PHYLO_EINVAL, "phylo_debug_site_patterns_rule: bad arguments");
        return -1;
    }
    return pk_pat_take(S, U, coded != 0, ntiles, sw) ? 1 : 0;
}

int phylo_debug_site_patterns_of(phylo_ctx* c, int32_t* U, int32_t* taken) {
    if (!c || !U || !taken) return fail(c, PHYLO_EINVAL, "phylo_debug_site_patterns_of: NULL argument");
    if (!c->have_leaves) return fail(c, PHYLO_ESTATE, "phylo_debug_site_patterns_of needs leaves");
    *U = c->pat_U;
    *taken = pat_on(c) ? 1 : 0;
    return PHYLO_OK;
}

int phylo_debug_tree_plan(int N, int K, int G, int world, int64_t n_clades, int64_t n_topologies, int kept_whole, int force_wide,
                          int64_t summary_temp, int64_t branches_temp, int64_t* scalars, int64_t* summary_slab, int64_t* branches_slab,
                          int32_t* sort_bits, int32_t* launches) {
    if (K < 1 || G < 1 || K % G != 0 || N > PK_MAX_TAXA || world < 1 || summary_temp < 0 || branches_temp < 0 || !scalars || !summary_slab ||
        !branches_slab || !sort_bits || !launches)
        return fail(nullptr, PHYLO_EINVAL, "phylo_debug_tree_plan: bad arguments");
    char why[160];
    const pt_facts f{N, K, G, world};
    if (pt_refuses(f, why, sizeof why)) return fail(nullptr, PHYLO_EINVAL, "%s", why);
    const pb_facts fb{N, K, G, world, n_clades, n_topologies, kept_whole != 0, force_wide != 0};
    if (pb_refuses(fb, why, sizeof why)) return fail(nullptr, PHYLO_ESTATE, "%s", why);
    pt_plan p = pt_plan_form(f);
    pt_plan_slab(p, (size_t)summary_temp);
    pb_plan q = pb_plan_form(fb);
    pb_plan_slab(q, (size_t)branches_temp);
    unsigned bits[PT_MAX_WORDS + 9];
    const int n_sorts = pt_plan_sorts(p, bits);
    for (int i = 0; i < n_sorts; ++i) sort_bits[i] = (int32_t)bits[i];
    const int64_t sc[] = {p.R, p.L, p.W, p.E, p.Emax, p.Kg, q.cbits, q.tbits, q.wide, q.gather, n_sorts, pt_slab::NBUF, pb_slab::NBUF};
    memcpy(scalars, sc, sizeof sc);
    for (int i = 0; i < pt_slab::NBUF; ++i) { summary_slab[i] = (int64_t)p.slab.off[i]; summary_slab[pt_slab::NBUF + i] = (int64_t)p.slab.bytes[i]; }
    summary_slab[2 * pt_slab::NBUF] = (int64_t)p.slab.total;
    for (int i = 0; i < pb_slab::NBUF; ++i) { branches_slab[i] = (int64_t)q.slab.off[i]; branches_slab[pb_slab::NBUF + i] = (int64_t)q.slab.bytes[i]; }
    branches_slab[2 * pb_slab::NBUF] = (int64_t)q.slab.total;
    launches[0] = pt_plan_launches(p);
    launches[1] = pb_plan_launches(q);
    return PHYLO_OK;
}

int phylo_debug_scan_form(phylo_ctx* c, int Kg, int multi_min, int wanted) {
    if (Kg < 1) {
        (void)fail(c, PHYLO_EINVAL, "phylo_debug_scan_form: bad arguments");
        return -1;
    }
    return (int)sweep_scan_form_of(Kg, c ? c->env.scan_multi_min : multi_min, wanted != 0, k_sweep_limits);
}

int phylo_debug_persist_plan(int N, int K, int S, int G, uint32_t flags, uint32_t switches, int world, int transport, int n_cus,
                             int blocks_per_cu, int persist_wgs, int persist_nt, int64_t* out) {
    if (N < 1 || K < 1 || S < 1 || G < 1 || K % G != 0 || world < 1 || !out)
        return fail(nullptr, PHYLO_EINVAL, "phylo_debug_persist_plan: bad arguments");
// ... 651 lines not shown
```

phylo_amd/csrc/phylo_kernels.h:

```cpp
#pragma once
#include <hip/hip_runtime.h>
#include <stdint.h>

#include "phylo_math.h"
#include "phylo_packed_codes.h"
#include "phylo_site_patterns.h"

#define PK_COLS 256
#define PK_AUX 8
#define PK_MAX_TAXA 512
#define PK_MAX_GROUPS 64

enum { AUX_SUM_REM = 0, AUX_FPRIOR, AUX_LPRIOR, AUX_RPRIOR, AUX_LL_TILDE, AUX_PAREN, AUX_LOGV, AUX_Q };
#define PK_REC 16
enum { REC_BASE_L = PK_AUX, REC_BASE_R, REC_NODELL, REC_ROOTLL, REC_LL, REC_LOGW, REC_FLAGS  };
#define PK_REC_SLOTS (REC_FLAGS + 1)
static_assert(PK_REC_SLOTS <= PK_REC && PK_REC_SLOTS <= 16, "one lane per slot: with 16 lanes or more per particle the bookkeeping writes the record in one trip (pk_book_tail)");

__device__ __forceinline__ double pk_block_canon_sum(double col, double* sh4) {
#pragma unroll
    for (int off = 1; off < 64; off <<= 1) col = col + __shfl_xor(col, off, 64);
    __syncthreads();
    if ((threadIdx.x & 63) == 0) sh4[threadIdx.x >> 6] = col;
    __syncthreads();
// ... 473 lines not shown
        if (cdf[mid] > thr) hi = mid; else lo = mid + 1;
    }
    return lo < K ? lo : K - 1;
}

__global__ void pk_resample_search(const uint64_t* __restrict__ cdf, int K, int n_draw, int k0, uint64_t seed,
                                   uint32_t step, int64_t* __restrict__ idx) {
    const int k = blockIdx.x * blockDim.x + threadIdx.x;
    if (k >= n_draw) return;
    const pm_u32x4 x = pm_philox4x32((uint32_t)(k0 + k), step, PM_STREAM_RESAMPLE, 0u, seed);
    const uint64_t R = ((uint64_t)x.y << 32) | x.x;
    idx[k] = pk_cdf_search(cdf, K, pm_mulhi64(R, cdf[K - 1]));
}

__global__ void pk_logz_total(const double* __restrict__ lse, int R, double* __restrict__ out) {
    if (threadIdx.x == 0 && blockIdx.x == 0) {
        double z = 0.0;
        for (int r = 0; r < R; ++r) z = z + lse[r];
        *out = z;
    }
}

__global__ void pk_logz_total_groups(double* __restrict__ lse, int R, int stride) {
    if (threadIdx.x == 0) {
        double* l = lse + (size_t)blockIdx.x * stride;
        double z = 0.0;
        for (int r = 0; r < R; ++r) z = z + l[r];
        l[R] = z;
    }
}

__global__ void pk_init_tables(int32_t* __restrict__ roots, int32_t* __restrict__ cnt, double* __restrict__ rootll,
                               const double* __restrict__ nodell, int K, int N) {
    const int i = blockIdx.x * blockDim.x + threadIdx.x;
    if (i >= K * N) return;
    roots[i] = i % N;
    cnt[i] = 1;
    rootll[i] = nodell[i % N];
}

struct pk_rank_args {
    int r, n, N, S, K , Kloc, k0;
    uint64_t seed;
    uint32_t flags;
    const int32_t* roots_old; const int32_t* cnt_old;
    int32_t* roots_new; int32_t* cnt_new;
    const double* rootll_old; double* rootll_new;
    const uint64_t* cdf;
    const double* ll_prev;
    double* nodell;
    const double* ldf; int ldf_n;
    const double* bl; const double* br;
    double lam_l, lam_r, loglam_l, loglam_r, ll_tilde0;
    const double* leaves;
    const uint8_t* leaf_codes;
    const uint8_t* leaf_packed;
    size_t packed_leaf_bytes;
    double* pool;
    const double* const* pool_ptrs;
    int32_t* mirror;
    double* cache;
    int cache_cap;
    const double* Pmat;
    const double* pi;
    double* logw_r; double* ll_r;
    int32_t* merges;
    int64_t* ancestors;
    int lazy;
    unsigned int* mark;
    const int32_t* child_all;
    const double* Pmat_all;
    int32_t* child;
    double* aux;
    int32_t* pos_hist;
    const char* const* tab_ptrs;
    size_t tab_off_rootll, tab_off_roots, tab_off_cnt;
    int Kg;
    const uint64_t* group_seeds;
    int no_store;
    const unsigned long long* rdraw;
    int T, ntiles;
    double* tilev;
    unsigned long long* rec;
};

struct pk_book_lds {
    double *ord_ll, *ord_ldf, *hbl, *hbr, *anc_ll, *ldf;
    uint32_t* key; int32_t *ro, *co, *ord_cnt;
    double* aux; int32_t* misc;
};
__host__ __device__ inline size_t pk_book_lds_bytes(int N) {
    const size_t n4 = ((size_t)N + 3) & ~(size_t)3;
    return (6 * n4 + 4) * 8 + PK_AUX * 8 + (4 * n4) * 4 + 16 ;
}
__device__ __forceinline__ pk_book_lds pk_book_carve(char* base, int N) {
    const size_t n4 = ((size_t)N + 3) & ~(size_t)3;
    pk_book_lds L;
    L.ord_ll = (double*)base;
    L.ord_ldf = L.ord_ll + n4;
    L.hbl = L.ord_ldf + n4;
    L.hbr = L.hbl + n4;
    L.anc_ll = L.hbr + n4;
    L.ldf = L.anc_ll + n4;
    L.aux = L.ldf + n4 + 4;
    L.key = (uint32_t*)(L.aux + PK_AUX);
    L.ro = (int32_t*)(L.key + n4);
    L.co = L.ro + n4;
    L.ord_cnt = L.co + n4;
    L.misc = L.ord_cnt + n4;
    return L;
}

__device__ __forceinline__ void pk_rec_write(const pk_rank_args& a, int k, int kg, int t, const pk_book_lds& L) {
    const size_t node_sz = (size_t)a.S * 4;
    unsigned long long v;
    if (t < PK_AUX) {
        v = (unsigned long long)__double_as_longlong(L.aux[t]);
    } else if (t <= REC_BASE_R) {
        const int id = L.misc[t - REC_BASE_L];
        if (id >= a.N) v = (unsigned long long)(a.pool + (size_t)(id - a.N) * node_sz);
        else if (a.leaf_codes) v = (unsigned long long)(a.leaf_packed + (size_t)id * a.packed_leaf_bytes);
        else v = (unsigned long long)(a.leaves + (size_t)id * node_sz);
    } else if (t == REC_NODELL) {
        v = (unsigned long long)(a.nodell + (a.N + a.r * a.K + kg));
    } else if (t == REC_ROOTLL) {
        v = (unsigned long long)(a.rootll_new + ((size_t)kg * a.N + (a.n - 2)));
    } else if (t == REC_LL) {
        v = (unsigned long long)(a.ll_r + kg);
    } else if (t == REC_LOGW) {
        v = (unsigned long long)(a.logw_r + kg);
    } else {
        v = a.leaf_codes ? (unsigned long long)((L.misc[0] < a.N ? 1 : 0) | (L.misc[1] < a.N ? 2 : 0)) : 0ull;
    }
    a.rec[(size_t)k * PK_REC + t] = v;
}


template <int LP>
__device__ __forceinline__ int pk_cdf_search_group(const uint64_t* cdf, int K, uint64_t R, int sl, int lane) {
    const int gshift = lane & ~(LP - 1);
    const unsigned long long gmask = LP == 64 ? ~0ull : ((1ull << (LP & 63)) - 1ull);
    int lo = 0, hi = K;
    int step = (K + LP - 1) / LP;
    int p = (sl + 1) * step - 1;
    if (p > K - 1) p = K - 1;
    const uint64_t total = cdf[K - 1];
    uint64_t c = cdf[p];
    const uint64_t thr = pm_mulhi64(R, total);
    bool done = false;
    for (;;) {
        const unsigned long long ball = __ballot(!done && c > thr);
        if (!done) {
            const unsigned long long mask = (ball >> gshift) & gmask;
            const int f = mask ? __ffsll((long long)mask) - 1 : LP - 1;
            int pf = lo + (f + 1) * step - 1;
            if (pf > hi - 1) pf = hi - 1;
            lo = lo + f * step;
            hi = pf + 1;
            if (lo >= hi) lo = hi - 1;
            if (hi - lo <= 1) done = true;
            else {
                step = (hi - lo + LP - 1) / LP;
                p = lo + (sl + 1) * step - 1;
                if (p > hi - 1) p = hi - 1;
                c = cdf[p];
            }
        }
        if (__all(done)) break;
    }
    return lo;
}

template <int LP, bool KEY_LOOP>
__device__ __forceinline__ void pk_book_packed(const pk_rank_args& a, int kg, bool local, const pk_book_lds& L, int sl, int lane) {
    const int n = a.n, N = a.N, k = kg - a.k0;
    const int grp = a.group_seeds ? kg / a.Kg : 0;
    const int gbase = grp * a.Kg;
    const uint64_t seed = a.group_seeds ? a.group_seeds[grp] : a.seed;
    const uint32_t kin = (uint32_t)(kg - gbase);
    {
        #pragma unroll 1
        for (int j = sl; j <= a.r; j += LP) {
            L.hbl[j] = local ? a.bl[(size_t)j * a.Kloc + k] : 0.0;
            L.hbr[j] = local ? a.br[(size_t)j * a.Kloc + k] : 0.0;
        }
        #pragma unroll 1
        for (int j = sl; j <= a.ldf_n; j += LP) L.ldf[j] = a.ldf[j];
        const int nb = (n + 3) / 4;
        uint64_t Rdraw;
        if (KEY_LOOP && nb > LP - 1) {
            #pragma unroll 1
            for (int b = sl; b < nb; b += LP) {
                const pm_u32x4 x = pm_philox4x32(kin, (uint32_t)a.r, PM_STREAM_PAIR, (uint32_t)b, seed);
                L.key[b * 4 + 0] = x.x; L.key[b * 4 + 1] = x.y; L.key[b * 4 + 2] = x.z; L.key[b * 4 + 3] = x.w;
            }
            const pm_u32x4 x = pm_philox4x32(kin, (uint32_t)a.r, PM_STREAM_RESAMPLE, 0u, seed);
            Rdraw = ((uint64_t)x.y << 32) | x.x;
        } else {
            const bool res = sl == LP - 1;
            const pm_u32x4 x = pm_philox4x32(kin, (uint32_t)a.r, res ? PM_STREAM_RESAMPLE : PM_STREAM_PAIR, res ? 0u : (uint32_t)sl, seed);
            if (sl < nb) { L.key[sl * 4 + 0] = x.x; L.key[sl * 4 + 1] = x.y; L.key[sl * 4 + 2] = x.z; L.key[sl * 4 + 3] = x.w; }
            const int src = (lane & ~(LP - 1)) + LP - 1;
            Rdraw = ((uint64_t)(uint32_t)__shfl((int)x.y, src, 64) << 32) | (uint32_t)__shfl((int)x.x, src, 64);
        }
        int anc = kg;
        if (a.r > 0) anc = gbase + pk_cdf_search_group<LP>(a.cdf + gbase, a.group_seeds ? a.Kg : a.K, Rdraw, sl, lane);
        const int32_t* ro = a.roots_old + (size_t)anc * N;
        const int32_t* co = a.cnt_old + (size_t)anc * N;
        const double* rl = a.rootll_old + (size_t)anc * N;
        if (a.tab_ptrs) {
            const char* base = a.tab_ptrs[anc / a.Kloc];
            ro = reinterpret_cast<const int32_t*>(base + a.tab_off_roots) + (size_t)anc * N;
            co = reinterpret_cast<const int32_t*>(base + a.tab_off_cnt) + (size_t)anc * N;
            rl = reinterpret_cast<const double*>(base + a.tab_off_rootll) + (size_t)anc * N;
        }
        #pragma unroll 1
        for (int i = sl; i < n; i += LP) { L.ro[i] = ro[i]; L.co[i] = co[i]; L.anc_ll[i] = rl[i]; }
        if (sl == 0) {
            L.misc[3] = anc;
            if (local) L.aux[AUX_LL_TILDE] = (a.r > 0) ? a.ll_prev[anc] : a.ll_tilde0;
        }
    }
    __syncthreads();
    {
        unsigned long long best = 0ull;
        #pragma unroll 1
        for (int i = sl; i < n; i += LP) {
            const unsigned long long c = ((unsigned long long)L.key[i] << 32) | (0xffffffffu - (uint32_t)i);
            best = c > best ? c : best;
        }
#pragma unroll
        for (int off = 1; off < LP; off <<= 1) {
            const unsigned long long o = __shfl_xor(best, off, 64);
            best = o > best ? o : best;
        }
        const int il = (int)(0xffffffffu - (uint32_t)best);
        best = 0ull;
        #pragma unroll 1
        for (int i = sl; i < n; i += LP) {
            const unsigned long long c = ((unsigned long long)L.key[i] << 32) | (0xffffffffu - (uint32_t)i);
            if (i != il) best = c > best ? c : best;
        }
#pragma unroll
        for (int off = 1; off < LP; off <<= 1) {
            const unsigned long long o = __shfl_xor(best, off, 64);
            best = o > best ? o : best;
        }
        const int ir = (int)(0xffffffffu - (uint32_t)best);
        int32_t* rn = a.roots_new + (size_t)kg * N;
        int32_t* cn = a.cnt_new + (size_t)kg * N;
        double* rln = a.rootll_new + (size_t)kg * N;
        #pragma unroll 1
        for (int i = sl; i < n; i += LP) {
            if (i == il || i == ir) continue;
            const unsigned long long mine = ((unsigned long long)L.key[i] << 32) | (uint32_t)i;
            int rank = 0;
            #pragma unroll 1
            for (int j = 0; j < n; ++j) {
                const unsigned long long cj = ((unsigned long long)L.key[j] << 32) | (uint32_t)j;
                rank += (j != il && j != ir && cj < mine) ? 1 : 0;
            }
            const int node = L.ro[i], c = L.co[i];
            const double xll = L.anc_ll[i];
            rn[rank] = node;
            cn[rank] = c;
            rln[rank] = xll;
            if (a.pos_hist) a.pos_hist[(size_t)kg * N + i] = rank;
            L.ord_cnt[rank] = c;
            L.ord_ll[rank] = xll;
            L.ord_ldf[rank] = L.ldf[c < a.ldf_n ? c : a.ldf_n];
        }
        if (sl == 0) {
            const int cnew = L.co[il] + L.co[ir];
            rn[n - 2] = N + a.r * a.K + kg;
            cn[n - 2] = cnew;
            L.ord_cnt[n - 2] = cnew;
            L.ord_ldf[n - 2] = L.ldf[cnew < a.ldf_n ? cnew : a.ldf_n];
            L.misc[0] = L.ro[il];
            L.misc[1] = L.ro[ir];
            if (a.pos_hist) { a.pos_hist[(size_t)kg * N + il] = -1; a.pos_hist[(size_t)kg * N + ir] = -1; }
            if (local) {
                a.merges[((size_t)a.r * a.Kloc + k) * 2 + 0] = il;
                a.merges[((size_t)a.r * a.Kloc + k) * 2 + 1] = ir;
                if (a.r > 0) a.ancestors[(size_t)(a.r - 1) * a.Kloc + k] = L.misc[3] - gbase;
            }
        }
    }
    __syncthreads();
    if (local) {
// ... 204 lines not shown
    const int tid = threadIdx.x;
    const int grp = a.group_seeds ? kg / a.Kg : 0, gbase = grp * a.Kg, Kg = a.group_seeds ? a.Kg : a.K, kin = kg - gbase;
    const unsigned long long lo = kin > 0 ? a.cdf[gbase + kin - 1] : 0ull, hi = a.cdf[gbase + kin], total = a.cdf[gbase + Kg - 1];
    unsigned int hit = 0u;
    #pragma unroll 4
    for (int i = tid; i < Kg; i += PK_COLS) {
        const unsigned long long t = pm_mulhi64(a.rdraw[gbase + i], total);
        hit |= (unsigned int)(t >= lo) & (unsigned int)(t < hi);
    }
    if (!__syncthreads_or((int)hit)) return;
    pk_materialize_node<1>(a, a.r - 1, kg, tid, PK_COLS, 0, a.S);
    if (tid == 0) a.mark[(size_t)(a.r - 1) * a.K + kg] = 1u;
}
__device__ __forceinline__ void pk_mat_by_thresholds_grouped(const pk_rank_args& a, int k0) {
    __shared__ unsigned long long gcdf[PK_MAT_GROUP];
    __shared__ unsigned int maskw[2];
    const int tid = threadIdx.x;
    const int grp = a.group_seeds ? k0 / a.Kg : 0, gbase = grp * a.Kg, Kg = a.group_seeds ? a.Kg : a.K, kin0 = k0 - gbase;
    const int cnt = Kg - kin0 < PK_MAT_GROUP ? Kg - kin0 : PK_MAT_GROUP;
    if (tid < PK_MAT_GROUP) gcdf[tid] = a.cdf[gbase + kin0 + (tid < cnt ? tid : cnt - 1)];
    if (tid < 2) maskw[tid] = 0u;
    const unsigned long long lo = kin0 > 0 ? a.cdf[gbase + kin0 - 1] : 0ull, total = a.cdf[gbase + Kg - 1];
    __syncthreads();
    const unsigned long long hi = gcdf[cnt - 1];
    unsigned long long mine = 0ull;
    #pragma unroll 2
    for (int i = tid; i < Kg; i += PK_COLS) {
        const unsigned long long t = pm_mulhi64(a.rdraw[gbase + i], total);
        if (t >= lo && t < hi) {
            int l = 0, h = cnt - 1;
            while (l < h) {
                const int m = (l + h) >> 1;
                if (gcdf[m] > t) h = m; else l = m + 1;
            }
            mine |= 1ull << l;
        }
    }
#pragma unroll
    for (int off = 1; off < 64; off <<= 1) mine |= __shfl_xor(mine, off, 64);
    if ((tid & 63) == 0 && mine) {
        if ((unsigned int)mine) atomicOr(&maskw[0], (unsigned int)mine);
        if ((unsigned int)(mine >> 32)) atomicOr(&maskw[1], (unsigned int)(mine >> 32));
    }
    __syncthreads();
    unsigned long long todo = ((unsigned long long)maskw[1] << 32) | maskw[0];
    while (todo) {
        const int j = __ffsll((long long)todo) - 1;
        todo &= todo - 1;
        pk_materialize_node<1>(a, a.r - 1, k0 + j, tid, PK_COLS, 0, a.S);
        if (tid == 0) a.mark[(size_t)(a.r - 1) * a.K + k0 + j] = 1u;
    }
}
__global__ __launch_bounds__(PK_COLS) void pk_materialize_by_draws(const pk_rank_args a, int grouped) {
    if (grouped) pk_mat_by_thresholds_grouped(a, a.k0 + (int)blockIdx.x * PK_MAT_GROUP);
    else pk_mat_by_thresholds(a, a.k0 + (int)blockIdx.x);
}

template <int LP>
__global__ __launch_bounds__(PK_COLS, 5) void pk_rank_book_mat(const pk_rank_args a, int book_blocks) {
    extern __shared__ __attribute__((aligned(16))) char smem[];
    if ((int)blockIdx.x >= book_blocks) {
        pk_mat_by_thresholds(a, (int)blockIdx.x - book_blocks);
        return;
    }
    const int tid = threadIdx.x, lane = tid & 63, sub = tid / LP, sl = tid & (LP - 1);
    int idx = blockIdx.x * (PK_COLS / LP) + sub;
    if (idx >= a.K) idx = a.K - 1;
    const int kg = idx;
    const pk_book_lds L = pk_book_carve(smem + (size_t)sub * pk_book_lds_bytes(a.N), a.N);
    pk_book_packed<LP, false>(a, kg, true, L, sl, lane);
    pk_book_tail<LP>(a, kg, true, a.r > 0, false, L, sl, lane);
}

__device__ __forceinline__ const double* pk_node_ptr(const pk_rank_args& a, int id) {
    const size_t node_sz = (size_t)a.S * 4;
    if (id < a.N) return a.leaves + (size_t)id * node_sz;
    if (a.Kloc == a.K) return a.pool + (size_t)(id - a.N) * node_sz;
    const int x = id - a.N, rho = x / a.K, kap = x - rho * a.K, owner = kap / a.Kloc;
    if (a.mirror && owner * a.Kloc != a.k0) {
        const int slot = a.mirror[x];
        if (slot > 0) return a.cache + (size_t)(slot - 1) * node_sz;
    }
    return a.pool_ptrs[owner] + ((size_t)rho * a.Kloc + (kap - owner * a.Kloc)) * node_sz;
}

__device__ __forceinline__ void pk_build_leaf_table(const double* __restrict__ P , double (*tab)[4], int t) {
    if (t < 16) tab[t >> 2][t & 3] = P[t];
    else if (t < 20) {
        const int j = t - 16;
        tab[4][j] = pm_fma(1.0, P[12 + j], pm_fma(1.0, P[8 + j], pm_fma(1.0, P[4 + j], 1.0 * P[j])));
    }
}

__device__ __forceinline__ void pk_merge_epilogue(const pk_rank_args& a, int k, int kg, double tot) {
    const double* ax = a.aux + (size_t)k * PK_AUX;
    const double fl = ax[AUX_SUM_REM] + tot;
    const double ll = ((fl + ax[AUX_FPRIOR]) + ax[AUX_LPRIOR]) + ax[AUX_RPRIOR];
    const double lw = (((ll - ax[AUX_LL_TILDE]) - ax[AUX_PAREN]) + ax[AUX_LOGV]) - ax[AUX_Q];
    a.nodell[a.N + a.r * a.K + kg] = tot;
    a.rootll_new[(size_t)kg * a.N + (a.n - 2)] = tot;
    a.ll_r[kg] = ll;
    a.logw_r[kg] = lw;
}

__global__ __launch_bounds__(256) void pk_tile_epilogue(const pk_rank_args a) {
    const int k = blockIdx.x * blockDim.x + threadIdx.x;
    if (k >= a.Kloc) return;
    const double* tv = a.tilev + (size_t)k * a.ntiles;
    double tot = tv[0];
    for (int t = 1; t < a.ntiles; ++t) tot = tot + tv[t];
    pk_merge_epilogue(a, k, a.k0 + k, tot);
}

__global__ void pk_fix_rootll(double* __restrict__ rootll_new, const double* __restrict__ nodell_row, int K, int N, int n,
                              int k0, int Kloc) {
    const int kg = blockIdx.x * blockDim.x + threadIdx.x;
    if (kg >= K || (kg >= k0 && kg < k0 + Kloc)) return;
    rootll_new[(size_t)kg * N + (n - 2)] = nodell_row[kg];
}

#define PK_TWIST_MAX_M 1024
#define PK_TWIST_MAX_J (1 << 20)
#define PK_TWIST_LDS_J 8192
#define PK_TWIST_DRAW_BLOCK 0xFFFFFFFFu

struct pk_twist_args {
    pk_rank_args a;
    int M, J;
    int32_t* roots_ad; int32_t* cnt_ad; double* rootll_ad;
    double* tw_b;
    double* tw_P;
    double* pot;
    double* chosen;
    double* Pmat_r;
    double* bl_r; double* br_r;
    const uint32_t* pair_hist;
    const uint8_t* codes;
    int own_tables;
    double* wbuf;
};

__global__ __launch_bounds__(256) void pk_pair_hist(const uint8_t* __restrict__ codes, int N, int S, uint32_t* __restrict__ hist) {
    __shared__ unsigned int h[32];
    const int a = blockIdx.x, b = blockIdx.y, tid = threadIdx.x;
    if (tid < 32) h[tid] = 0u;
    __syncthreads();
    const uint8_t* ca = codes + (size_t)a * S;
    const uint8_t* cb = codes + (size_t)b * S;
    for (int s = tid; s < S; s += 256) atomicAdd(&h[ca[s] * 5 + cb[s]], 1u);
    __syncthreads();
    if (tid < 32) hist[((size_t)a * N + b) * 32 + tid] = h[tid];
}

__device__ __forceinline__ void pk_twist_adopt_body(const pk_twist_args& ta, int kg) {
    const pk_rank_args& a = ta.a;
    const int lane = threadIdx.x, N = a.N, n = a.n;
    int anc = kg;
    if (a.r > 0) {
        const pm_u32x4 x = pm_philox4x32((uint32_t)kg, (uint32_t)a.r, PM_STREAM_RESAMPLE, 0u, a.seed);
        anc = pk_cdf_search_group<64>(a.cdf, a.K, ((uint64_t)x.y << 32) | x.x, lane, lane);
    }
    for (int i = lane; i < n; i += 64) {
        ta.roots_ad[(size_t)kg * N + i] = a.roots_old[(size_t)anc * N + i];
        ta.cnt_ad[(size_t)kg * N + i] = a.cnt_old[(size_t)anc * N + i];
        ta.rootll_ad[(size_t)kg * N + i] = a.rootll_old[(size_t)anc * N + i];
    }
// ... 1289 lines not shown
```

phylo_amd/csrc/phylo_persist.h:

```cpp
#pragma once
#include "phylo_kernels.h"

#define PP_CHUNK 16
#define PP_CTR_STRIDE 16
#define PP_MAX_M 1024
#define PP_MAX_KG 8192
#define PP_SPIN_LIMIT (1u << 21)

struct pp_args {
    int N, S, K, Kg, G, R;
    int T;
    int Wg, m;
    uint64_t seed;
    const uint64_t* group_seeds;
    uint32_t flags;
    int jc;
    const double* Q; const double* lam_l; const double* lam_r; const double* pi; const double* ldf;
    const double* leaves; const uint8_t* leaf_codes; double* pool;
    int32_t* roots[2]; int32_t* cnt[2]; double* rootll[2];
    double* nodell; double* bl; double* br; double* Pmat; double* logw; double* ll;
    int32_t* child; int32_t* merges; int64_t* anc; unsigned int* mark;
    unsigned long long* rdraw;
    double* lse; int lse_stride;
    unsigned long long* ctr;
// ... 159 lines not shown
    double v[E];
    double m = -pm_inf();
    for (int base = 0; base < Kg; base += 2048) {
#pragma unroll
        for (int j = 0; j < E; ++j) {
            const int k = base + tid + NT * j;
            v[j] = pp_gld(logw + (k < Kg ? k : Kg - 1));
        }
#pragma unroll
        for (int j = 0; j < E; ++j) {
            if (base + tid + NT * j >= Kg) v[j] = pm_nan();
            if (!pm_isnan(v[j]) && v[j] > m) m = v[j];
        }
    }
    m = pp_wave_max(m);
    if (lane == 0) sh->d[wv] = m;
    __syncthreads();
    m = sh->d[0];
#pragma unroll
    for (int i = 1; i < NW; ++i) m = sh->d[i] > m ? sh->d[i] : m;
    const bool all_bad = !(m > -pm_inf()) || m == pm_inf();
    for (int base = 0; base < Kg; base += 2048) {
        if (!one_tile) {
#pragma unroll
            for (int j = 0; j < E; ++j) {
                const int k = base + tid + NT * j;
                v[j] = pp_gld(logw + (k < Kg ? k : Kg - 1));
            }
        }
        double w[E];
#pragma unroll
        for (int j = 0; j < E; ++j) {
            const bool nan = pm_isnan(v[j]);
            const double e = pm_exp_nonpos(nan ? 0.0 : v[j] - m);
            w[j] = all_bad ? 1.0 : (nan ? 0.0 : e);
        }
#pragma unroll
        for (int j = 0; j < E; ++j) {
            const int k = base + tid + NT * j;
            if (k < Kg) cdf[k] = pm_bits(w[j]);
        }
    }
    __syncthreads();
    if (tid < 256) {
        double col = 0.0;
        for (int k = tid; k < Kg; k += 256) col = col + pm_from_bits(cdf[k]);
        col = pp_wave_tree_sum(col);
        if (lane == 0) sh->d[wv] = col;
    }
    __syncthreads();
    if (tid == 0 && lse_out) {
        const double sum = ((sh->d[0] + sh->d[1]) + sh->d[2]) + sh->d[3];
        const double mm = all_bad ? 0.0 : m;
        *lse_out = (mm + pp_log(sum)) - pp_log((double)Kg);
    }
    if (!want_cdf) return;
    unsigned long long carry = 0;
    for (int base = 0; base < Kg; base += 2048) {
        const int lo = base + E * tid;
        unsigned long long e[E];
#pragma unroll
        for (int j = 0; j < E; ++j)
            e[j] = (lo + j < Kg) ? (all_bad ? 1ull : (unsigned long long)(pm_from_bits(cdf[lo + j]) * PM_CDF_SCALE)) : 0ull;
#pragma unroll
        for (int j = 1; j < E; ++j) e[j] += e[j - 1];
        const unsigned long long local = e[E - 1];
        const unsigned long long incl = pp_wave_incl_scan_u64(local, lane);
        if (base > 0) __syncthreads();
        if (lane == 63) sh->u[wv] = incl;
        __syncthreads();
        unsigned long long run = carry + incl - local, all = 0;
#pragma unroll
        for (int i = 0; i < NW; ++i) {
            if (i < wv) run += sh->u[i];
            all += sh->u[i];
        }
#pragma unroll
        for (int j = 0; j < E; ++j)
            if (lo + j < Kg) cdf[lo + j] = run + e[j];
        carry += all;
    }
}

template <int NT>
__global__ __launch_bounds__(NT) void pp_resample_scan(const double* logw, int Kg, uint64_t* __restrict__ cdf, double* lse_out, int lse_stride,
                                                       int logz_R) {
    extern __shared__ __attribute__((aligned(16))) char smem[];
    pp_scan_lds* sh = reinterpret_cast<pp_scan_lds*>(smem);
    unsigned long long* lcdf = reinterpret_cast<unsigned long long*>(smem + ((sizeof(pp_scan_lds) + 15) & ~(size_t)15));
    const int g = blockIdx.x;
    pp_scan<NT>(logw + (size_t)g * Kg, Kg, lcdf, lse_out ? lse_out + (size_t)g * lse_stride : (double*)nullptr, sh, cdf != nullptr);
    if (logz_R > 0 && lse_out && threadIdx.x == 0) {
        double* row = lse_out + (size_t)g * lse_stride - (logz_R - 1);
        double z = 0.0;
        for (int r = 0; r < logz_R; ++r) z = z + row[r];
        row[logz_R] = z;
    }
    if (!cdf) return;
    __syncthreads();
    unsigned long long* out = reinterpret_cast<unsigned long long*>(cdf) + (size_t)g * Kg;
    for (int k = threadIdx.x; k < Kg; k += NT) out[k] = lcdf[k];
}
#define PP_SCAN_TILE 2048
struct pp_scan_multi_args {
    const double* logw;
    int Kg, B;
    double* gmax;
    unsigned long long* bsum;
    unsigned long long* wbits;
    unsigned long long* cdf;
    double* lse_out;
    int lse_stride, logz_R;
    int lse_only;
};
__device__ __forceinline__ double pp_scan_multi_group_max(const pp_scan_multi_args& a, int g) {
    double m = pp_gld(a.gmax + (size_t)g * a.B);
    for (int b = 1; b < a.B; ++b) {
        const double o = pp_gld(a.gmax + (size_t)g * a.B + b);
        m = o > m ? o : m;
    }
    return m;
}
__global__ __launch_bounds__(512) void pp_scan_multi_max(const pp_scan_multi_args a) {
    __shared__ double sh[8];
    const int b = blockIdx.x, g = blockIdx.y, tid = threadIdx.x, lane = tid & 63, wv = tid >> 6;
    const double* logw = a.logw + (size_t)g * a.Kg;
    double m = -pm_inf();
#pragma unroll
    for (int j = 0; j < 4; ++j) {
        const int k = b * PP_SCAN_TILE + tid + 512 * j;
        const double v = pp_gld(logw + (k < a.Kg ? k : a.Kg - 1));
        if (k < a.Kg && !pm_isnan(v) && v > m) m = v;
    }
    m = pp_wave_max(m);
    if (lane == 0) sh[wv] = m;
    __syncthreads();
    if (tid == 0) {
        m = sh[0];
#pragma unroll
        for (int i = 1; i < 8; ++i) m = sh[i] > m ? sh[i] : m;
        a.gmax[(size_t)g * a.B + b] = m;
    }
}
__global__ __launch_bounds__(512) void pp_scan_multi_exp(const pp_scan_multi_args a) {
    __shared__ unsigned long long sh[8];
    const int b = blockIdx.x, g = blockIdx.y, tid = threadIdx.x, lane = tid & 63, wv = tid >> 6;
    const double* logw = a.logw + (size_t)g * a.Kg;
    const double m = pp_scan_multi_group_max(a, g);
    const bool all_bad = !(m > -pm_inf()) || m == pm_inf();
    double v[4], w[4];
#pragma unroll
    for (int j = 0; j < 4; ++j) {
        const int k = b * PP_SCAN_TILE + tid + 512 * j;
        v[j] = pp_gld(logw + (k < a.Kg ? k : a.Kg - 1));
    }
#pragma unroll
    for (int j = 0; j < 4; ++j) {
        const bool nan = pm_isnan(v[j]);
        const double e = pm_exp_nonpos(nan ? 0.0 : v[j] - m);
        w[j] = all_bad ? 1.0 : (nan ? 0.0 : e);
    }
    unsigned long long local = 0;
#pragma unroll
    for (int j = 0; j < 4; ++j) {
        const int k = b * PP_SCAN_TILE + tid + 512 * j;
        if (k < a.Kg) {
            a.wbits[(size_t)g * a.Kg + k] = pm_bits(w[j]);
            local += all_bad ? 1ull : (unsigned long long)(w[j] * PM_CDF_SCALE);
        }
    }
    const unsigned long long incl = pp_wave_incl_scan_u64(local, lane);
    if (lane == 63) sh[wv] = incl;
    __syncthreads();
    if (tid == 0) {
        unsigned long long t = 0;
#pragma unroll
        for (int i = 0; i < 8; ++i) t += sh[i];
        a.bsum[(size_t)g * a.B + b] = t;
    }
}
__global__ __launch_bounds__(512) void pp_scan_multi_cdf(const pp_scan_multi_args a) {
    __shared__ pp_scan_lds sh;
    const int b = blockIdx.x, g = blockIdx.y, tid = threadIdx.x, lane = tid & 63, wv = tid >> 6;
    const unsigned long long* wb = a.wbits + (size_t)g * a.Kg;
    const double m = pp_scan_multi_group_max(a, g);
    const bool all_bad = !(m > -pm_inf()) || m == pm_inf();
    if (b == a.B || a.lse_only) {
        if (!a.lse_out) return;
        if (tid < 256) {
            double col = 0.0;
            for (int k0 = tid; k0 < a.Kg; k0 += 256 * 16) {
                unsigned long long q[16];
#pragma unroll
                for (int u = 0; u < 16; ++u) {
                    const int k = k0 + 256 * u;
                    q[u] = pp_gld(wb + (k < a.Kg ? k : a.Kg - 1));
                }
#pragma unroll
                for (int u = 0; u < 16; ++u)
                    if (k0 + 256 * u < a.Kg) col = col + pm_from_bits(q[u]);
            }
            col = pp_wave_tree_sum(col);
            if (lane == 0) sh.d[wv] = col;
        }
        __syncthreads();
        if (tid == 0) {
            const double sum = ((sh.d[0] + sh.d[1]) + sh.d[2]) + sh.d[3];
            const double mm = all_bad ? 0.0 : m;
            double* out = a.lse_out + (size_t)g * a.lse_stride;
            *out = (mm + pp_log(sum)) - pp_log((double)a.Kg);
            if (a.logz_R > 0) {
                double* row = out - (a.logz_R - 1);
                double z = 0.0;
                for (int r = 0; r < a.logz_R; ++r) z = z + row[r];
                row[a.logz_R] = z;
            }
        }
        return;
    }
    unsigned long long carry = 0;
    for (int i = 0; i < b; ++i) carry += pp_gld(a.bsum + (size_t)g * a.B + i);
    const int lo = b * PP_SCAN_TILE + 4 * tid;
    unsigned long long e[4];
#pragma unroll
    for (int j = 0; j < 4; ++j)
        e[j] = (lo + j < a.Kg) ? (all_bad ? 1ull : (unsigned long long)(pm_from_bits(pp_gld(wb + lo + j)) * PM_CDF_SCALE)) : 0ull;
#pragma unroll
    for (int j = 1; j < 4; ++j) e[j] += e[j - 1];
    const unsigned long long local = e[3];
    const unsigned long long incl = pp_wave_incl_scan_u64(local, lane);
    if (lane == 63) sh.u[wv] = incl;
    __syncthreads();
    unsigned long long run = carry + incl - local;
#pragma unroll
    for (int i = 0; i < 8; ++i)
        if (i < wv) run += sh.u[i];
    unsigned long long* out = a.cdf + (size_t)g * a.Kg;
#pragma unroll
    for (int j = 0; j < 4; ++j)
        if (lo + j < a.Kg) out[lo + j] = run + e[j];
}
#define PP_SCAN_KERNEL_MAX_KG 16384
__host__ inline size_t pp_resample_scan_lds(int Kg) { return ((sizeof(pp_scan_lds) + 15) & ~(size_t)15) + (size_t)Kg * 8; }

template <bool STAGE>
__device__ __forceinline__ void pp_part_a(const pp_args& a, int r, int kg, uint32_t kin, uint64_t seed, const pp_slot& L, int lane,
                                          double lam_l, double lam_r, double loglam_l, double loglam_r) {
    const int N = a.N, n = N - r, K = a.K;
    const int nb = (n + 3) / 4;
    pp_stamp(a, r, 13);
    if (lane < nb) {
        const pm_u32x4 x = pm_philox4x32(kin, (uint32_t)r, PM_STREAM_PAIR, (uint32_t)lane, seed);
        L.key[lane * 4 + 0] = x.x; L.key[lane * 4 + 1] = x.y; L.key[lane * 4 + 2] = x.z; L.key[lane * 4 + 3] = x.w;
    }
    const double hbl = lane <= r ? pp_gld(a.bl + (size_t)lane * K + kg) : 0.0;
    const double hbr = lane <= r ? pp_gld(a.br + (size_t)lane * K + kg) : 0.0;
    if constexpr (STAGE) { if (lane < 32) L.P[lane] = pp_gld(a.Pmat + ((size_t)r * K + kg) * 32 + lane); }
    pp_lds_fence();
    unsigned long long best = lane < n ? (((unsigned long long)L.key[lane] << 32) | (0xffffffffu - (uint32_t)lane)) : 0ull;
#pragma unroll
    for (int off = 1; off < 64; off <<= 1) {
        const unsigned long long o = __shfl_xor(best, off, 64);
        best = o > best ? o : best;
    }
    const int il = (int)(0xffffffffu - (uint32_t)best);
    best = (lane < n && lane != il) ? (((unsigned long long)L.key[lane] << 32) | (0xffffffffu - (uint32_t)lane)) : 0ull;
#pragma unroll
    for (int off = 1; off < 64; off <<= 1) {
        const unsigned long long o = __shfl_xor(best, off, 64);
        best = o > best ? o : best;
    }
    const int ir = (int)(0xffffffffu - (uint32_t)best);
    if (lane < n) {
        int rank = -1;
        if (lane != il && lane != ir) {
            const unsigned long long mine = ((unsigned long long)L.key[lane] << 32) | (uint32_t)lane;
            rank = 0;
            #pragma unroll 1
            for (int j = 0; j < n; ++j) {
                const unsigned long long cj = ((unsigned long long)L.key[j] << 32) | (uint32_t)j;
                rank += (j != il && j != ir && cj < mine) ? 1 : 0;
            }
            L.inv[rank] = lane;
        }
        L.rank[lane] = rank;
    }
    if constexpr (STAGE) {
        if (lane < 20) pk_build_leaf_table(L.P, reinterpret_cast<double (*)[4]>(L.tab), lane);
        else if (lane >= 32 && lane < 52) pk_build_leaf_table(L.P + 16, reinterpret_cast<double (*)[4]>(L.tab + 20), lane - 32);
        pp_lds_fence();
        pk_build_lik25(reinterpret_cast<const double (*)[4]>(L.tab), reinterpret_cast<const double (*)[4]>(L.tab + 20), a.pi, L.lik25, lane);
    }
    double lp = 0.0, rp = 0.0;
    #pragma unroll 1
    for (int j = 0; j <= r; ++j) {
        lp = lp + ((-lam_l) * pp_readlane(hbl, j) + loglam_l);
        rp = rp + ((-lam_r) * pp_readlane(hbr, j) + loglam_r);
    }
    const double b_l = pp_readlane(hbl, r), b_r = pp_readlane(hbr, r);
    if (lane == 0) {
        const double q = 1.0 / ((double)((n - 1) * n) / 2.0);
        L.aux[AUX_LPRIOR] = lp;
        L.aux[AUX_RPRIOR] = rp;
        L.aux[AUX_PAREN] = ((loglam_l - lam_l * b_l) + loglam_r) - lam_r * b_r;
        L.aux[AUX_Q] = (a.flags & 1u) ? q : pp_log(q);
        L.misc[0] = il;
        L.misc[1] = ir;
    }
    pp_lds_fence();
    pp_stamp(a, r, 14);
}

template <bool CL, bool CR, int BS>
struct pp_blk {
    pk_d2 La[CL ? 1 : BS][2], Ra[CR ? 1 : BS][2];
    int cl[CL ? BS : 1], cr[CR ? BS : 1];
};
template <bool CL, bool CR, int BS>
__device__ __forceinline__ void pp_blk_load(pp_blk<CL, CR, BS>& b, int s0, int s1, int it0, const double* Lp, const double* Rp, const uint8_t* Lc,
                                            const uint8_t* Rc, int lane) {
#pragma unroll
    for (int u = 0; u < BS; ++u) {
        int s = s0 + lane + 64 * (it0 + u);
        s = s < s1 ? s : s1 - 1;
        if constexpr (CL) b.cl[u] = Lc[s]; else { b.La[u][0] = pk_gload2(Lp + (size_t)s * 4); b.La[u][1] = pk_gload2(Lp + (size_t)s * 4 + 2); }
        if constexpr (CR) b.cr[u] = Rc[s]; else { b.Ra[u][0] = pk_gload2(Rp + (size_t)s * 4); b.Ra[u][1] = pk_gload2(Rp + (size_t)s * 4 + 2); }
// ... 389 lines not shown
```

phylo_amd/csrc/phylo_sweep_plan.h:

```cpp
#pragma once

#include <cstddef>
#include <cstdint>
#include <cstdio>

struct sweep_limits {
    int max_groups;
    int twist_max_m, twist_max_j;
    int mat_group;
    int scan_fold_max_kg;
    int scan_lds512_max_kg;
    int kept_bits_taxa;
    int one_tile_max_s;
    int small_max_kg, small_max_kloc;
    int book_packed8_min;
    int sorted_min_draws;
};

struct sweep_facts {
    int N, K, Kloc, S, G, M, world;
    int ntiles;
    bool transport;
    bool device_exchange;
    bool jc;
// ... 37 lines not shown

inline int sweep_book_width(int N, int nbook, const sweep_limits& L) {
    if (N <= 16) return nbook >= L.book_packed8_min ? 8 : 16;
    return N <= 32 ? 32 : 64;
}

inline bool sweep_refuses_batch(const sweep_facts& f, const sweep_limits& L, char* msg, size_t n) {
    const bool sharded = f.world != 1;
    if (f.G < 1 || f.G > L.max_groups || f.K % f.G != 0)
        return snprintf(msg, n, "a batch needs 1 <= G <= %d sweeps and K = %d divisible by G (got %d)", L.max_groups, f.K, f.G), true;
    if (f.G > 1 && f.twisting) return snprintf(msg, n, "batched sweeps need the plain proposal (PHYLO_TWISTING is set)"), true;
    if (f.G > 1 && f.keep_graph) {
        if (sharded || f.transport) return snprintf(msg, n, "batched sweeps with PHYLO_KEEP_GRAPH need an unsharded context"), true;
        if (f.S > L.one_tile_max_s)
            return snprintf(msg, n, "batched sweeps with PHYLO_KEEP_GRAPH need S <= 4096 sites (got %d)", f.S), true;
    }
    return false;
}
inline bool sweep_refuses_form(const sweep_facts& f, const sweep_limits& L, char* msg, size_t n) {
    const bool sharded = f.world != 1;
    if (f.twisting) {
        if (f.M < 1 || f.M > L.twist_max_m)
            return snprintf(msg, n, "twisting needs 1 <= M <= %d (got %d)", L.twist_max_m, f.M), true;
        const size_t Jmax = (size_t)(f.N * (f.N - 1) / 2) * (size_t)f.M;
        if (Jmax > (size_t)L.twist_max_j) return snprintf(msg, n, "twisting: C(N,2)*M = %zu exceeds %d", Jmax, L.twist_max_j), true;
    }
    if (f.keep_graph && sharded) {
        if (f.twisting) return snprintf(msg, n, "PHYLO_KEEP_GRAPH with PHYLO_TWISTING needs an unsharded context"), true;
        if (f.S > L.one_tile_max_s)
            return snprintf(msg, n, "PHYLO_KEEP_GRAPH on a sharded context needs S <= 4096 sites (got %d)", f.S), true;
    }
    return false;
}

inline sweep_plan sweep_plan_form(const sweep_facts& f, const sweep_limits& L) {
    sweep_plan p{};
    const int N = f.N, K = f.K, Kl = f.Kloc, S = f.S;
    p.R = N - 1; p.G = f.G; p.Kg = K / f.G;
    p.twist = f.twisting; p.graph = f.keep_graph; p.timek = f.time_kernels;
    const bool eager = sweep_eager_nodes(f.eager_nodes, f.env_eager_nodes);
    const bool one_tile = p.one_tile = S <= L.one_tile_max_s;
    p.lazy = !p.twist && (!p.graph || one_tile) && !eager;
    p.shard_form = f.world > 1 || (f.transport && f.env_rehearse_sharded);
    p.replicated_book = f.env_replicated_book || (p.graph && f.world > 1);
    p.local_book = !p.twist && p.shard_form && !p.replicated_book;
    p.book_mat = p.lazy && f.world == 1 && !f.transport && N <= 64 && one_tile && f.G == 1 && Kl <= L.small_max_kloc;
    const bool mat_small = p.Kg <= L.small_max_kg && Kl <= L.small_max_kloc;
    p.mat_by_draws = p.lazy && p.local_book && one_tile && (mat_small || (p.Kg % L.mat_group == 0 && Kl % L.mat_group == 0));
    p.mat_draws_grouped = !mat_small;
    p.want_rdraw = p.book_mat || p.mat_by_draws;
    p.no_store_last = !p.graph && !eager;
    p.final_missing = p.no_store_last && !p.lazy;
    p.use_rec = !p.twist && Kl == K && p.lazy;
    p.sorted_prologue = !p.twist && !f.jc && 2L * p.R * Kl >= L.sorted_min_draws;
    p.mat_grouped = one_tile && Kl > L.small_max_kloc;
    p.step_a_work = p.lazy && p.local_book;
    p.mat_after_book = p.lazy && !p.local_book && !p.book_mat;
    p.mat_barrier = f.transport;
    p.book_width = p.twist ? 0 : sweep_book_width(N, p.local_book ? Kl : K, L);
    p.twist_ll = p.twist && f.coded_leaves;
    p.twist_tables = p.twist && f.transport;
    p.tile_epilogue = f.ntiles > 1;
    p.fix_rootll = f.transport && !p.local_book;
    p.fold_logz = p.Kg <= L.scan_fold_max_kg;
    p.lse_stride = f.G > 1 ? p.R + 1 : 0;
    p.last_graph_eager = p.graph && !p.lazy && !p.twist && one_tile && f.world == 1 && Kl == K && N > L.kept_bits_taxa;
    p.gather_launches = (p.graph && f.world > 1) ? (f.device_exchange ? 4 : 2) : 0;
    return p;
}

enum sweep_scan_form {
    SCAN_MULTI = 0,
    SCAN_LDS_512 = 1,
    SCAN_LDS_1024 = 2,
    SCAN_IN_PLACE = 3
};
inline sweep_scan_form sweep_scan_form_of(int Kg, int multi_min, bool wanted, const sweep_limits& L) {
    if (Kg > multi_min && wanted) return SCAN_MULTI;
    if (Kg <= L.scan_lds512_max_kg) return SCAN_LDS_512;
    if (Kg <= L.scan_fold_max_kg) return SCAN_LDS_1024;
    return SCAN_IN_PLACE;
}

inline int sweep_plan_launches(const sweep_plan& p, int r) {
    if (r < 0) return 1;
    if (r >= p.R) return (p.fold_logz ? 0 : 1) + p.gather_launches;
    int n = 0;
    if (p.step_a_work && r > 0) n += p.mat_by_draws ? 1 : 2;
    n += p.twist ? 3 + (p.twist_ll ? 1 : 0) + (p.twist_tables ? 1 : 0) : 1;
    if (p.mat_after_book && r > 0) n += 1;
    n += 1 + (p.tile_epilogue ? 1 : 0);
    n += (p.fix_rootll ? 1 : 0) + 1;
    return n;
}

struct persist_limits {
    int max_taxa;
    int max_kg;
    int max_m;
    int max_s;
    size_t max_lds;
    size_t (*lds_bytes)(int N, int m, int Kg);
};

struct persist_facts {
    int N, K, S, G, world;
    bool transport;
    bool one_launch;
    bool twisting, keep_graph, time_kernels, eager_nodes, env_eager_nodes;
    int n_cus;
    int blocks_per_cu;
    int persist_wgs;
    int persist_nt;
};

struct persist_grid {
    bool taken;
    int Wg, m, nt;
    size_t lds;
};

inline int persist_nt_of(int requested) { return requested == 512 ? 512 : 256; }

inline bool persist_refuses_shape(const persist_facts& f, const persist_limits& L) {
    if (!f.one_launch) return true;
    if (f.world != 1 || f.transport) return true;
    if (f.twisting || f.keep_graph || f.time_kernels) return true;
    if (sweep_eager_nodes(f.eager_nodes, f.env_eager_nodes)) return true;
    if (f.N > L.max_taxa || f.N < 2) return true;
    if (f.K / f.G > L.max_kg) return true;
    if (f.S > L.max_s) return true;
    return false;
}

inline persist_grid persist_plan_of(const persist_facts& f, const persist_limits& L) {
    const persist_grid no{};
    if (persist_refuses_shape(f, L)) return no;
    if (f.blocks_per_cu < 1 || f.n_cus < 1) return no;
    const int Kg = f.K / f.G;
    int Wt = f.persist_wgs > 0 ? f.persist_wgs : f.n_cus;
    if (Wt > f.n_cus * f.blocks_per_cu) Wt = f.n_cus * f.blocks_per_cu;
    if (Wt < f.G) return no;
    int Wg = Wt / f.G;
    if (Wg > Kg) Wg = Kg;
    while (Wg > 1 && Kg % Wg) --Wg;
    const int m = Kg / Wg;
    if (m > L.max_m) return no;
    const size_t lds = L.lds_bytes(f.N, m, Kg);
    if (lds > L.max_lds) return no;
    return persist_grid{true, Wg, m, f.persist_nt, lds};
}

inline uint32_t sweep_plan_mask(const sweep_plan& p) {
    const bool b[] = {p.twist, p.graph, p.timek, p.lazy, p.shard_form, p.replicated_book, p.local_book, p.book_mat, p.mat_by_draws,
                      p.want_rdraw, p.use_rec, p.sorted_prologue, p.mat_grouped, p.mat_draws_grouped, p.step_a_work, p.mat_after_book,
                      p.mat_barrier, p.fix_rootll, p.fold_logz, p.no_store_last, p.final_missing, p.last_graph_eager,
                      p.one_tile, p.twist_ll, p.twist_tables, p.tile_epilogue, p.lse_stride != 0};
    static_assert(sizeof b / sizeof b[0] <= 28, "bits 28..31 hold book_width / 8");
    uint32_t m = (uint32_t)(p.book_width / 8) << 28;
    for (size_t i = 0; i < sizeof b / sizeof b[0]; ++i) m |= b[i] ? 1u << i : 0u;
    return m;
}
```

Baseline: 672.5 billion particle-site-likelihoods/s.

## Draw ancestors inside the resampling scan and fold materialization into book kernel

The resampling scan kernel now also draws next-round ancestors via binary search over the LDS-resident cdf. It compacts the set of adopted parents into a per-group list. The book kernel is launched with extra workgroups that materialize only the adopted parents' partial likelihoods, and the separate materialize launch is skipped. This removes one launch per rank and avoids materializing unadopted particles, at the cost of extra LDS and serial binary-search work in the single-workgroup-per-group scan.

```diff
diff --git a/include/phylo_hip.h b/include/phylo_hip.h
--- a/include/phylo_hip.h
+++ b/include/phylo_hip.h
@@ -137,6 +137,11 @@
                              int TS, int64_t coeff_wgs, int passes_in_flight, uint32_t* mask);
 int phylo_debug_sweep_plan(int N, int K, int K_local, int S, int G, int M, int world, int transport, uint32_t flags, uint32_t switches,
                            uint32_t* mask, int32_t* launches);
+int phylo_debug_sweep_chain(int N, int K, int K_local, int S, int G, int M, int world, int transport, uint32_t flags, uint32_t switches,
+                            int multi_min, int scan_ancestors, int32_t* out);
+int phylo_debug_sweep_chain_of(phylo_ctx* ctx, int32_t* taken);
+int phylo_debug_scan_ancestors(phylo_ctx* ctx, const double* logw, int Kg, int G, const uint64_t* seeds, uint32_t r_next, int32_t* anc,
+                               int32_t* list, int32_t* cnt);
 int phylo_debug_scan_form(phylo_ctx* ctx, int Kg, int multi_min, int wanted);
 int phylo_debug_persist_plan(int N, int K, int S, int G, uint32_t flags, uint32_t switches, int world, int transport, int n_cus,
                              int blocks_per_cu, int persist_wgs, int persist_nt, int64_t* out);
diff --git a/phylo_amd/_ffi.py b/phylo_amd/_ffi.py
--- a/phylo_amd/_ffi.py
+++ b/phylo_amd/_ffi.py
@@ -25,7 +25,7 @@
     "phylo_sweep_async", "phylo_sweep_batch_async", "phylo_sweep_batch_begin", "phylo_sweep_fetch_logz", "phylo_sweep_begin", "phylo_sweep_step", "phylo_sweep_step_a", "phylo_sweep_step_group", "phylo_sweep_finish", "phylo_sweep_fetch",
     "phylo_synchronize", "phylo_sweep_node", "phylo_sweep_backward", "phylo_sweep_backward_batch",
     "phylo_tree_summary", "phylo_tree_summary_fetch", "phylo_tree_branches", "phylo_tree_branches_fetch",
-    "phylo_math_probe", "phylo_debug_frechet", "phylo_debug_stamps", "phylo_debug_reverse_lists", "phylo_debug_lookahead_lists", "phylo_debug_reverse_plan", "phylo_debug_reverse_plan_batch", "phylo_debug_sweep_plan", "phylo_debug_pack_leaf_codes", "phylo_debug_site_patterns", "phylo_debug_site_patterns_rule", "phylo_debug_site_patterns_of", "phylo_debug_tree_plan", "phylo_debug_tree_branches_of", "phylo_debug_scan_form", "phylo_debug_persist_plan", "phylo_debug_persist_of", "phylo_debug_device_lists", "phylo_debug_device_lists_of", "phylo_debug_remote_cache", "phylo_debug_site_product",
+    "phylo_math_probe", "phylo_debug_frechet", "phylo_debug_stamps", "phylo_debug_reverse_lists", "phylo_debug_lookahead_lists", "phylo_debug_reverse_plan", "phylo_debug_reverse_plan_batch", "phylo_debug_sweep_plan", "phylo_debug_sweep_chain", "phylo_debug_sweep_chain_of", "phylo_debug_scan_ancestors", "phylo_debug_pack_leaf_codes", "phylo_debug_site_patterns", "phylo_debug_site_patterns_rule", "phylo_debug_site_patterns_of", "phylo_debug_tree_plan", "phylo_debug_tree_branches_of", "phylo_debug_scan_form", "phylo_debug_persist_plan", "phylo_debug_persist_of", "phylo_debug_device_lists", "phylo_debug_device_lists_of", "phylo_debug_remote_cache", "phylo_debug_site_product",
     "phylo_vi_gradients", "phylo_vi_gradients_batch", "phylo_vi_apply",
     "phylo_site_tile", "phylo_set_site_tile", "phylo_get_site_tile",
     "phylo_comm_unique_id", "phylo_comm_init", "phylo_comm_share", "phylo_comm_allgather", "phylo_comm_max", "phylo_comm_barrier",
@@ -155,6 +155,18 @@
     out["mask"] = mask.value
     out["launches"] = list(launches)
     return out
+
+
+def debug_sweep_chain(N, K, S, K_local=None, G=1, M=1, world=1, transport=False, flags=0, switches=(), multi_min=4096, scan_ancestors=1):
+    lib = load()
+    sw = sum(1 << SWEEP_PLAN_SWITCHES.index(name) for name in switches)
+    out = (C.c_int32 * 3)()
+    rc = lib.phylo_debug_sweep_chain(C.c_int(N), C.c_int(K), C.c_int(K if K_local is None else K_local), C.c_int(S), C.c_int(G), C.c_int(M),
+                                     C.c_int(world), C.c_int(int(transport)), C.c_uint32(flags), C.c_uint32(sw), C.c_int(multi_min),
+                                     C.c_int(scan_ancestors), out)
+    if rc:
+        raise PhyloError(rc, lib.phylo_last_error(None).decode())
+    return {"taken": bool(out[0]), "item_waves": out[1], "parts": out[2]}
 
 
 def debug_pack_leaf_codes(codes):
@@ -860,6 +872,26 @@
             raise PhyloError(rc, self._lib.phylo_last_error(self._h).decode())
         return SCAN_FORMS[rc]
 
+    def debug_sweep_chain(self):
+        taken = C.c_int32(0)
+        self._check(self._lib.phylo_debug_sweep_chain_of(self._h, C.byref(taken)))
+        return bool(taken.value)
+
+    def debug_scan_ancestors(self, logw, seeds, r_next):
+        w = np.ascontiguousarray(logw, dtype=np.float64)
+        if w.ndim != 2:
+            raise ValueError("logw must be [G][Kg]")
+        G, Kg = w.shape
+        sd = np.ascontiguousarray(seeds, dtype=np.uint64)
+        if sd.shape != (G,):
+            raise ValueError("one seed per group")
+        anc = np.full((G, Kg), -2, dtype=np.int32)
+        lst = np.full((G, Kg), -2, dtype=np.int32)
+        cnt = np.full(G, -2, dtype=np.int32)
+        self._check(self._lib.phylo_debug_scan_ancestors(self._h, _ptr(w), C.c_int(Kg), C.c_int(G), _ptr(sd), C.c_uint32(r_next), _ptr(anc),
+                                                         _ptr(lst), _ptr(cnt)))
+        return anc, lst, cnt
+
     def debug_persist(self):
         nt, Wg, m, lds = C.c_int32(0), C.c_int32(0), C.c_int32(0), C.c_int64(0)
         self._check(self._lib.phylo_debug_persist_of(self._h, C.byref(nt), C.byref(Wg), C.byref(m), C.byref(lds)))
diff --git a/phylo_amd/csrc/phylo_hip.hip b/phylo_amd/csrc/phylo_hip.hip
--- a/phylo_amd/csrc/phylo_hip.hip
+++ b/phylo_amd/csrc/phylo_hip.hip
@@ -53,6 +53,7 @@
     bool active = false;
     int a_done_r = -1;
     sweep_plan plan{};
+    sweep_chain_form chain{};
 };
 
 struct env_switches {
@@ -65,6 +66,7 @@
     int persist_nt = 256;
     int remote_cache_cap = 0;
     int scan_multi_min = 4096;
+    int scan_ancestors = 1;
     int site_patterns = PK_PAT_AUTO;
     int trees_chunk = 0;
     int rell_chunk = 0;
@@ -85,6 +87,7 @@
         { const char* e = getenv("PHYLO_REMOTE_CACHE_CAP"); remote_cache_cap = e ? atoi(e) : 0; }
         { const char* e = getenv("PHYLO_SITE_PATTERNS"); site_patterns = !e ? PK_PAT_AUTO : !strcmp(e, "force") ? PK_PAT_FORCE : atoi(e) == 0 ? PK_PAT_OFF : PK_PAT_AUTO; }
         { const char* e = getenv("PHYLO_SCAN_MULTI_MIN"); scan_multi_min = e ? atoi(e) : 4096; }
+        { const char* e = getenv("PHYLO_SCAN_ANCESTORS"); scan_ancestors = e ? atoi(e) : 1; }
         { const char* e = getenv("PHYLO_TREES_CHUNK"); trees_chunk = e ? atoi(e) : 0; }
         { const char* e = getenv("PHYLO_RELL_CHUNK"); rell_chunk = e ? atoi(e) : 0; }
         { const char* e = getenv("PHYLO_P2P"); no_p2p = e && atoi(e) == 0; }
@@ -159,6 +162,10 @@
     int32_t* d_merges = nullptr;
     int64_t* d_anc = nullptr;
     uint64_t* d_cdf[2] = {nullptr, nullptr};
+    int32_t* d_anc_next = nullptr;
+    int32_t* d_adopt_list = nullptr;
+    int32_t* d_adopt_cnt = nullptr;
+    int last_chain = 0;
     unsigned int* d_counter = nullptr;
     const double** d_pool_ptrs = nullptr;
     int32_t* d_mirror = nullptr;
@@ -392,7 +399,7 @@
     c->d_tilev = nullptr;
     void* ptrs[] = {c->d_pool, c->d_nodell, c->d_bl, c->d_br, c->d_Pmat, c->d_logw, c->d_ll, c->d_aux, c->d_lse, c->d_group_seeds,
                     c->d_tables, (void*)c->d_tab_ptrs, c->d_child, c->d_merges, c->d_anc,
-                    c->d_cdf[0], c->d_cdf[1], c->d_counter, (void*)c->d_pool_ptrs, c->d_mark, c->d_sync, c->d_mirror, c->d_cache, c->d_rec};
+                    c->d_cdf[0], c->d_cdf[1], c->d_anc_next, c->d_adopt_list, c->d_adopt_cnt, c->d_counter, (void*)c->d_pool_ptrs, c->d_mark, c->d_sync, c->d_mirror, c->d_cache, c->d_rec};
     for (void* p : ptrs)
         if (p) (void)hipFree(p);
     c->d_pool = c->d_nodell = c->d_bl = c->d_br = c->d_Pmat = c->d_logw = c->d_ll = c->d_aux = c->d_lse = nullptr;
@@ -401,6 +408,7 @@
     c->d_roots[0] = c->d_roots[1] = c->d_cnt[0] = c->d_cnt[1] = c->d_child = c->d_merges = nullptr;
     c->d_anc = nullptr;
     c->d_cdf[0] = c->d_cdf[1] = nullptr;
+    c->d_anc_next = c->d_adopt_list = c->d_adopt_cnt = nullptr;
     c->d_counter = nullptr;
     c->d_rootll[0] = c->d_rootll[1] = nullptr;
     c->d_tables = nullptr;
@@ -467,6 +475,12 @@
     CHK(dalloc(c, &c->d_anc, (R > 0 ? R - 1 : 0) * Kl));
     CHK(dalloc(c, &c->d_cdf[0], K));
     CHK(dalloc(c, &c->d_cdf[1], K));
+    CHK(dalloc(c, &c->d_anc_next, K));
+    CHK(dalloc(c, &c->d_adopt_list, K));
+    CHK(dalloc(c, &c->d_adopt_cnt, (size_t)PK_MAX_GROUPS));
+    HIPCHK(c, hipMemset(c->d_anc_next, 0, K * 4));
+    HIPCHK(c, hipMemset(c->d_adopt_list, 0, K * 4));
+    HIPCHK(c, hipMemset(c->d_adopt_cnt, 0, (size_t)PK_MAX_GROUPS * 4));
     CHK(dalloc(c, &c->d_counter, ((size_t)N + 3) & ~(size_t)3));
     HIPCHK(c, hipMemset(c->d_counter, 0, (((size_t)N + 3) & ~(size_t)3) * sizeof(unsigned int)));
     CHK(dalloc(c, &c->d_pool_ptrs, (size_t)c->world));
@@ -607,8 +621,12 @@
 }
 static const sweep_limits k_sweep_limits = sweep_limits_of();
 
-int launch_scan(phylo_ctx* c, const double* logw, int Kg, int G, uint64_t* cdf, double* lse, int lse_stride, int logz_R = 0) {
+int launch_scan(phylo_ctx* c, const double* logw, int Kg, int G, uint64_t* cdf, double* lse, int lse_stride, int logz_R = 0,
+                const pp_anc_out* anc = nullptr) {
+    const pp_anc_out ao = anc ? *anc : pp_anc_out{};
     const sweep_scan_form form = sweep_scan_form_of(Kg, c->env.scan_multi_min, cdf || lse, k_sweep_limits);
+    if (ao.anc && (!cdf || logz_R > 0 || (form != SCAN_LDS_512 && form != SCAN_LDS_1024)))
+        return fail(c, PHYLO_ESTATE, "launch_scan: the resampling outcome needs a cdf and a scan that holds it in LDS (Kg = %d)", Kg);
     if (form == SCAN_MULTI) {
         pp_scan_multi_args a{};
         a.logw = logw; a.Kg = Kg; a.B = (Kg + PP_SCAN_TILE - 1) / PP_SCAN_TILE;
@@ -626,16 +644,26 @@
         return launch_check(c, "pp_scan_multi_cdf");
     }
     if (form == SCAN_LDS_512) {
-        hipLaunchKernelGGL(pp_resample_scan<512>, dim3(G), dim3(512), pp_resample_scan_lds(Kg), c->stream, logw, Kg, cdf, lse, lse_stride, logz_R);
+        if (ao.anc) hipLaunchKernelGGL(pp_resample_scan_anc<512>, dim3(G), dim3(512), pp_resample_scan_lds(Kg, true), c->stream, logw, Kg, cdf, lse, lse_stride, ao);
+        else hipLaunchKernelGGL(pp_resample_scan<512>, dim3(G), dim3(512), pp_resample_scan_lds(Kg), c->stream, logw, Kg, cdf, lse, lse_stride, logz_R);
         return launch_check(c, "pp_resample_scan");
     }
     if (form == SCAN_LDS_1024) {
-        const size_t lds = pp_resample_scan_lds(Kg);
-        static bool raised = false;
-        if (lds > 65536 && !raised) {
+        const size_t lds = pp_resample_scan_lds(Kg, ao.anc != nullptr);
+        static bool raised = false, raised_anc = false;
+        if (lds > 65536 && !raised && !ao.anc) {
             HIPCHK(c, hipFuncSetAttribute((const void*)pp_resample_scan<1024>, hipFuncAttributeMaxDynamicSharedMemorySize,
                                           (int)pp_resample_scan_lds(PP_SCAN_KERNEL_MAX_KG)));
             raised = true;
+        }
+        if (ao.anc) {
+            if (lds > 65536 && !raised_anc) {
+                HIPCHK(c, hipFuncSetAttribute((const void*)pp_resample_scan_anc<1024>, hipFuncAttributeMaxDynamicSharedMemorySize,
+                                              (int)pp_resample_scan_lds(PP_SCAN_KERNEL_MAX_KG, true)));
+                raised_anc = true;
+            }
+            hipLaunchKernelGGL(pp_resample_scan_anc<1024>, dim3(G), dim3(1024), lds, c->stream, logw, Kg, cdf, lse, lse_stride, ao);
+            return launch_check(c, "pp_resample_scan_anc");
         }
         hipLaunchKernelGGL(pp_resample_scan<1024>, dim3(G), dim3(1024), lds, c->stream, logw, Kg, cdf, lse, lse_stride, logz_R);
         return launch_check(c, "pp_resample_scan");
@@ -2002,6 +2030,8 @@
     c->run = sweep_run{};
     c->run.seed = seed; c->run.flags = flags; c->run.M = M;
     c->run.plan = p;
+    c->run.chain = sweep_chain_form_of(p, c->S, c->env.scan_multi_min, c->env.scan_ancestors, k_sweep_limits);
+    c->last_chain = c->run.chain.taken ? 1 : 0;
     c->run.launches = sweep_plan_launches(p, -1);
     c->run.active = true;
     c->last_persistent = false;
@@ -2106,6 +2136,7 @@
     c->pctr_base += (unsigned long long)R * Wg;
     sweep_publish(c, true, false, G, false, 0, 1, (double)K * S * R);
     c->last_persistent = true;
+    c->last_chain = 0;
     c->last_pp_nt = c->env.persist_nt; c->last_pp_Wg = Wg; c->last_pp_m = m; c->last_pp_lds = lds;
     return PHYLO_OK;
 }
@@ -2193,12 +2224,17 @@
     b.rec = p.use_rec ? c->d_rec : nullptr;
     b.lazy = p.lazy ? 1 : 0; b.mark = c->d_mark; b.child_all = c->d_child; b.Pmat_all = c->d_Pmat;
     b.T = c->site_tile; b.ntiles = c->ntiles; b.tilev = c->d_tilev;
+    if (c->run.chain.taken && r > 0) {
+        b.anc_in = c->d_anc_next; b.adopt_list = c->d_adopt_list; b.adopt_cnt = c->d_adopt_cnt;
+        b.item_waves = c->run.chain.item_waves; b.item_parts = c->run.chain.parts;
+    }
     return b;
 }
 
 static int step_materialize(phylo_ctx* c, const pk_rank_args& b) {
     const sweep_plan& p = c->run.plan;
     const int Kl = c->Kloc, S = c->S;
+    if (c->run.chain.taken) return PHYLO_OK;
     if (p.mat_by_draws) {
         const int grouped = p.mat_draws_grouped ? 1 : 0;
         hipLaunchKernelGGL(pk_materialize_by_draws, dim3(grouped ? Kl / PK_MAT_GROUP : Kl), dim3(PK_COLS), 0, c->stream, b, grouped);
@@ -2289,6 +2325,19 @@
         return launch_check(c, "pk_rank_book_mat");
     }
     const int per = 64 / (w > 0 ? w : 64);
+    const sweep_chain_form& ch = c->run.chain;
+    if (ch.taken) {
+        const int items = b.r > 0 ? p.G * ch.item_waves : 0;
+        const dim3 grid(items + cdiv(K, per));
+        switch (w) {
+        case 8: hipLaunchKernelGGL(pk_rank_book_chain<8>, grid, dim3(64), lds * per, c->stream, b, items); break;
+        case 16: hipLaunchKernelGGL(pk_rank_book_chain<16>, grid, dim3(64), lds * per, c->stream, b, items); break;
+        case 32: hipLaunchKernelGGL(pk_rank_book_chain<32>, grid, dim3(64), lds * per, c->stream, b, items); break;
+        case 64: hipLaunchKernelGGL(pk_rank_book_chain<64>, grid, dim3(64), lds * per, c->stream, b, items); break;
+        default: return fail(c, PHYLO_ESTATE, "step_book: no pk_rank_book_chain of %d lanes", w);
+        }
+        return launch_check(c, "pk_rank_book_chain");
+    }
     const dim3 grid(cdiv(p.local_book ? c->Kloc : K, per));
     switch (w) {
     case 8: hipLaunchKernelGGL(pk_rank_book_packed<8>, grid, dim3(64), lds * per, c->stream, b); break;
@@ -2351,8 +2400,13 @@
 static int step_scan(phylo_ctx* c, int r) {
     const sweep_plan& p = c->run.plan;
     const bool last = r + 1 == p.R;
+    pp_anc_out ao{};
+    if (c->run.chain.taken && !last) {
+        ao.anc = c->d_anc_next; ao.list = c->d_adopt_list; ao.cnt = c->d_adopt_cnt;
+        ao.group_seeds = p.G > 1 ? c->d_group_seeds : nullptr; ao.seed = c->run.seed; ao.r_next = (uint32_t)(r + 1);
+    }
     return launch_scan(c, (const double*)(c->d_logw + (size_t)r * c->K), p.Kg, p.G, last ? (uint64_t*)nullptr : c->d_cdf[(r & 1) ^ 1],
-                       c->d_lse + r, p.lse_stride, (last && p.fold_logz) ? p.R : 0);
+                       c->d_lse + r, p.lse_stride, (last && p.fold_logz) ? p.R : 0, ao.anc ? &ao : nullptr);
 }
 
 static int sweep_step_impl(phylo_ctx* c, int phase) {
@@ -3418,6 +3472,56 @@
     return PHYLO_OK;
 }
 
+int phylo_debug_sweep_chain(int N, int K, int K_local, int S, int G, int M, int world, int transport, uint32_t flags, uint32_t switches,
+                            int multi_min, int scan_ancestors, int32_t* out) {
+    if (N < 2 || N > PK_MAX_TAXA || K < 1 || K_local < 1 || K_local > K || S < 1 || world < 1 || !out)
+        return fail(nullptr, PHYLO_EINVAL, "phylo_debug_sweep_chain: bad arguments");
+    sweep_facts f{};
+    f.N = N; f.K = K; f.Kloc = K_local; f.S = S; f.G = G; f.M = M; f.world = world;
+    f.ntiles = (S + pm_site_tile(S) - 1) / pm_site_tile(S);
+    f.transport = transport != 0;
+    sweep_facts_flags(f, flags);
+    f.env_eager_nodes = switches & 1; f.env_rehearse_sharded = switches & 2; f.env_replicated_book = switches & 4;
+    f.jc = switches & 8; f.coded_leaves = switches & 16; f.device_exchange = switches & 32;
+    char why[160];
+    if (sweep_refuses_batch(f, k_sweep_limits, why, sizeof why) || sweep_refuses_form(f, k_sweep_limits, why, sizeof why))
+        return fail(nullptr, PHYLO_EINVAL, "%s", why);
+    const sweep_chain_form ch = sweep_chain_form_of(sweep_plan_form(f, k_sweep_limits), S, multi_min, scan_ancestors, k_sweep_limits);
+    out[0] = ch.taken ? 1 : 0; out[1] = ch.item_waves; out[2] = ch.parts;
+    return PHYLO_OK;
+}
+
+int phylo_debug_sweep_chain_of(phylo_ctx* c, int32_t* taken) {
+    if (!c || !taken) return fail(c, PHYLO_EINVAL, "phylo_debug_sweep_chain_of: NULL argument");
+    *taken = c->last_chain;
+    return PHYLO_OK;
+}
+
+int phylo_debug_scan_ancestors(phylo_ctx* c, const double* logw, int Kg, int G, const uint64_t* seeds, uint32_t r_next, int32_t* anc,
+                               int32_t* list, int32_t* cnt) {
+    CHK(bind(c));
+    if (!logw || !seeds || !anc || !list || !cnt || Kg < 1 || G < 1 || G > PK_MAX_GROUPS)
+        return fail(c, PHYLO_EINVAL, "phylo_debug_scan_ancestors: bad arguments");
+    const size_t K = (size_t)Kg * G;
+    void *dw, *dcdf, *dout, *dseed;
+    CHK(scratch_get(c, 0, K * 8, &dw));
+    CHK(scratch_get(c, 1, K * 8, &dcdf));
+    CHK(scratch_get(c, 2, (2 * K + (size_t)G) * 4, &dout));
+    CHK(scratch_get(c, 3, (size_t)G * 8, &dseed));
+    HIPCHK(c, hipMemcpyAsync(dw, logw, K * 8, hipMemcpyHostToDevice, c->stream));
+    HIPCHK(c, hipMemcpyAsync(dseed, seeds, (size_t)G * 8, hipMemcpyHostToDevice, c->stream));
+    HIPCHK(c, hipMemsetAsync(dout, 0xff, (2 * K + (size_t)G) * 4, c->stream));
+    pp_anc_out ao{};
+    ao.anc = (int32_t*)dout; ao.list = ao.anc + K; ao.cnt = ao.list + K;
+    ao.group_seeds = (const uint64_t*)dseed; ao.r_next = r_next;
+    CHK(launch_scan(c, (const double*)dw, Kg, G, (uint64_t*)dcdf, (double*)nullptr, 0, 0, &ao));
+    HIPCHK(c, hipMemcpyAsync(anc, ao.anc, K * 4, hipMemcpyDeviceToHost, c->stream));
+    HIPCHK(c, hipMemcpyAsync(list, ao.list, K * 4, hipMemcpyDeviceToHost, c->stream));
+    HIPCHK(c, hipMemcpyAsync(cnt, ao.cnt, (size_t)G * 4, hipMemcpyDeviceToHost, c->stream));
+    HIPCHK(c, hipStreamSynchronize(c->stream));
+    return PHYLO_OK;
+}
+
 int phylo_debug_pack_leaf_codes(const uint8_t* codes, int N, int S, uint8_t* packed, int64_t cap, int64_t* need) {
     if (N < 1 || S < 1 || !need || (packed && !codes)) return fail(nullptr, PHYLO_EINVAL, "phylo_debug_pack_leaf_codes: bad arguments");
     *need = (int64_t)pk_packed_bytes(N, S);
diff --git a/phylo_amd/csrc/phylo_kernels.h b/phylo_amd/csrc/phylo_kernels.h
--- a/phylo_amd/csrc/phylo_kernels.h
+++ b/phylo_amd/csrc/phylo_kernels.h
@@ -579,6 +579,10 @@
     int T, ntiles;
     double* tilev;
     unsigned long long* rec;
+    const int32_t* anc_in;
+    const int32_t* adopt_list;
+    const int32_t* adopt_cnt;
+    int item_waves, item_parts;
 };
 
 struct pk_book_lds {
@@ -668,7 +672,7 @@
     return lo;
 }
 
-template <int LP, bool KEY_LOOP>
+template <int LP, bool KEY_LOOP, bool ANC_IN = false>
 __device__ __forceinline__ void pk_book_packed(const pk_rank_args& a, int kg, bool local, const pk_book_lds& L, int sl, int lane) {
     const int n = a.n, N = a.N, k = kg - a.k0;
     const int grp = a.group_seeds ? kg / a.Kg : 0;
@@ -685,23 +689,29 @@
         for (int j = sl; j <= a.ldf_n; j += LP) L.ldf[j] = a.ldf[j];
         const int nb = (n + 3) / 4;
         uint64_t Rdraw;
+        if (ANC_IN) Rdraw = 0;
         if (KEY_LOOP && nb > LP - 1) {
             #pragma unroll 1
             for (int b = sl; b < nb; b += LP) {
                 const pm_u32x4 x = pm_philox4x32(kin, (uint32_t)a.r, PM_STREAM_PAIR, (uint32_t)b, seed);
                 L.key[b * 4 + 0] = x.x; L.key[b * 4 + 1] = x.y; L.key[b * 4 + 2] = x.z; L.key[b * 4 + 3] = x.w;
             }
-            const pm_u32x4 x = pm_philox4x32(kin, (uint32_t)a.r, PM_STREAM_RESAMPLE, 0u, seed);
-            Rdraw = ((uint64_t)x.y << 32) | x.x;
+            if (!ANC_IN) {
+                const pm_u32x4 x = pm_philox4x32(kin, (uint32_t)a.r, PM_STREAM_RESAMPLE, 0u, seed);
+                Rdraw = ((uint64_t)x.y << 32) | x.x;
+            }
         } else {
-            const bool res = sl == LP - 1;
+            const bool res = !ANC_IN && sl == LP - 1;
             const pm_u32x4 x = pm_philox4x32(kin, (uint32_t)a.r, res ? PM_STREAM_RESAMPLE : PM_STREAM_PAIR, res ? 0u : (uint32_t)sl, seed);
             if (sl < nb) { L.key[sl * 4 + 0] = x.x; L.key[sl * 4 + 1] = x.y; L.key[sl * 4 + 2] = x.z; L.key[sl * 4 + 3] = x.w; }
-            const int src = (lane & ~(LP - 1)) + LP - 1;
-            Rdraw = ((uint64_t)(uint32_t)__shfl((int)x.y, src, 64) << 32) | (uint32_t)__shfl((int)x.x, src, 64);
+            if (!ANC_IN) {
+                const int src = (lane & ~(LP - 1)) + LP - 1;
+                Rdraw = ((uint64_t)(uint32_t)__shfl((int)x.y, src, 64) << 32) | (uint32_t)__shfl((int)x.x, src, 64);
+            }
         }
         int anc = kg;
-        if (a.r > 0) anc = gbase + pk_cdf_search_group<LP>(a.cdf + gbase, a.group_seeds ? a.Kg : a.K, Rdraw, sl, lane);
+        if (ANC_IN) { if (a.r > 0) anc = gbase + a.anc_in[kg]; }
+        else if (a.r > 0) anc = gbase + pk_cdf_search_group<LP>(a.cdf + gbase, a.group_seeds ? a.Kg : a.K, Rdraw, sl, lane);
         const int32_t* ro = a.roots_old + (size_t)anc * N;
         const int32_t* co = a.cnt_old + (size_t)anc * N;
         const double* rl = a.rootll_old + (size_t)anc * N;
@@ -1072,6 +1082,69 @@
         if (slot > 0) return a.cache + (size_t)(slot - 1) * node_sz;
     }
     return a.pool_ptrs[owner] + ((size_t)rho * a.Kloc + (kap - owner * a.Kloc)) * node_sz;
+}
+
+typedef __attribute__((address_space(4))) const int32_t pk_ci32;
+#define PK_ITEM_ROWS 2
+__device__ __forceinline__ void pk_mat_listed(const pk_rank_args& a, int wg, int lane) {
+    typedef __attribute__((address_space(4))) const double cdbl;
+    constexpr int U = PK_ITEM_ROWS;
+    const int W = a.item_waves, Q = a.item_parts, rho = a.r - 1;
+    const int g = __builtin_amdgcn_readfirstlane(wg / W), w = wg - g * W;
+    const int n = ((pk_ci32*)a.adopt_cnt)[g] * Q;
+    if (w >= n) return;
+    pk_ci32* list = (pk_ci32*)(a.adopt_list + (size_t)g * a.Kg);
+    const size_t node_sz = (size_t)a.S * 4;
+    const int qlen = (a.S + Q - 1) / Q;
+    for (int item = w; item < n; item += W) {
+        const int e = __builtin_amdgcn_readfirstlane(item / Q), q = item - e * Q;
+        const int kap = g * a.Kg + list[e];
+        const size_t slot = (size_t)rho * a.K + kap;
+        pk_ci32* ch = (pk_ci32*)(a.child_all + slot * 2);
+        const cdbl* P = (const cdbl*)(a.Pmat_all + slot * 32);
+        const int c0 = ch[0], c1 = ch[1];
+        double Pl[16], Pr[16];
+#pragma unroll
+        for (int j = 0; j < 16; ++j) { Pl[j] = P[j]; Pr[j] = P[16 + j]; }
+        const double* Lp = c0 < a.N ? a.leaves + (size_t)c0 * node_sz : a.pool + (size_t)(c0 - a.N) * node_sz;
+        const double* Rp = c1 < a.N ? a.leaves + (size_t)c1 * node_sz : a.pool + (size_t)(c1 - a.N) * node_sz;
+        double* out = a.pool + slot * node_sz;
+        const int s0 = q * qlen, s1 = s0 + qlen < a.S ? s0 + qlen : a.S;
+        for (int s = s0 + lane; s < s1; s += U * 64) {
+            double Lv[U][4], Rv[U][4];
+#pragma unroll
+            for (int u = 0; u < U; ++u) {
+                const int su = s + u * 64 < s1 ? s + u * 64 : s;
+                pk_load4(Lp + (size_t)su * 4, Lv[u]);
+                pk_load4(Rp + (size_t)su * 4, Rv[u]);
+            }
+#pragma unroll
+            for (int u = 0; u < U; ++u) {
+                double o[4];
+                pk_merge_site(Lv[u], Rv[u], Pl, Pr, o);
+                if (s + u * 64 < s1) pk_store4(out + (size_t)(s + u * 64) * 4, o);
+            }
+        }
+        if (lane == 0) a.mark[(size_t)rho * a.K + kap] = 1u;
+    }
+}
+
+template <int LP>
+__global__ __launch_bounds__(64, LP == 64 ? 5 : 1) void pk_rank_book_chain(const pk_rank_args a, int item_wgs) {
+    extern __shared__ __attribute__((aligned(16))) char smem[];
+    if ((int)blockIdx.x < item_wgs) {
+        pk_mat_listed(a, (int)blockIdx.x, (int)threadIdx.x);
+        return;
+    }
+    const int lane = threadIdx.x, sub = lane / LP, sl = lane & (LP - 1);
+    const int count = a.tab_ptrs ? a.Kloc : a.K;
+    int idx = ((int)blockIdx.x - item_wgs) * (64 / LP) + sub;
+    if (idx >= count) idx = count - 1;
+    const int kg = a.tab_ptrs ? a.k0 + idx : idx;
+    const pk_book_lds L = pk_book_carve(smem + (size_t)sub * pk_book_lds_bytes(a.N), a.N);
+    const bool local = kg >= a.k0 && kg < a.k0 + a.Kloc;
+    pk_book_packed<LP, LP == 64, true>(a, kg, local, L, sl, lane);
+    pk_book_tail<LP>(a, kg, local, false, a.mirror && a.r > 0, L, sl, lane);
 }
 
 __device__ __forceinline__ void pk_build_leaf_table(const double* __restrict__ P , double (*tab)[4], int t) {
diff --git a/phylo_amd/csrc/phylo_persist.h b/phylo_amd/csrc/phylo_persist.h
--- a/phylo_amd/csrc/phylo_persist.h
+++ b/phylo_amd/csrc/phylo_persist.h
@@ -265,6 +265,74 @@
     }
 }
 
+struct pp_anc_out {
+    int32_t* anc;
+    int32_t* list;
+    int32_t* cnt;
+    const uint64_t* group_seeds;
+    uint64_t seed;
+    uint32_t r_next;
+};
+template <int NT>
+__device__ __forceinline__ void pp_scan_ancestors(const unsigned long long* cdf, int Kg, int g, const pp_anc_out& o, unsigned char* flag,
+                                                  pp_scan_lds* sh) {
+    constexpr int NW = NT / 64, ME = NT == 512 ? 8 : 16;
+    const int tid = threadIdx.x, lane = tid & 63, wv = tid >> 6;
+    for (int k = tid; k < Kg; k += NT) flag[k] = 0;
+    __syncthreads();
+    const uint64_t seed = o.group_seeds ? o.group_seeds[g] : o.seed;
+    const unsigned long long total = cdf[Kg - 1];
+    int32_t* anc = o.anc + (size_t)g * Kg;
+    for (int base = 0; base < Kg; base += 4 * NT) {
+        unsigned long long thr[4];
+        int lo[4];
+#pragma unroll
+        for (int j = 0; j < 4; ++j) {
+            const int k = base + tid + NT * j;
+            const pm_u32x4 x = pm_philox4x32((uint32_t)(k < Kg ? k : Kg - 1), o.r_next, PM_STREAM_RESAMPLE, 0u, seed);
+            thr[j] = pm_mulhi64(((uint64_t)x.y << 32) | x.x, total);
+            lo[j] = 0;
+        }
+        for (int n = Kg; n > 1;) {
+            const int half = n >> 1;
+#pragma unroll
+            for (int j = 0; j < 4; ++j) lo[j] = cdf[lo[j] + half - 1] > thr[j] ? lo[j] : lo[j] + half;
+            n -= half;
+        }
+#pragma unroll
+        for (int j = 0; j < 4; ++j) {
+            const int k = base + tid + NT * j;
+            if (k < Kg) { anc[k] = lo[j]; flag[lo[j]] = 1; }
+        }
+    }
+    __syncthreads();
+    const int E = (Kg + NT - 1) / NT;
+    unsigned long long b[ME];
+    int mine = 0;
+#pragma unroll
+    for (int j = 0; j < ME; ++j) {
+        const int i = (wv * E + j) * 64 + lane;
+        b[j] = __ballot(j < E && i < Kg && flag[i < Kg ? i : 0] != 0);
+        mine += __popcll(b[j]);
+    }
+    if (lane == 0) sh->u[wv] = (unsigned long long)mine;
+    __syncthreads();
+    int off = 0, all = 0;
+#pragma unroll
+    for (int i = 0; i < NW; ++i) {
+        const int u = (int)sh->u[i];
+        if (i < wv) off += u;
+        all += u;
+    }
+    int32_t* list = o.list + (size_t)g * Kg;
+#pragma unroll
+    for (int j = 0; j < ME; ++j) {
+        if ((b[j] >> lane) & 1ull) list[off + __popcll(b[j] & ((1ull << lane) - 1ull))] = (wv * E + j) * 64 + lane;
+        off += __popcll(b[j]);
+    }
+    if (tid == 0) o.cnt[g] = all;
+}
+
 template <int NT>
 __global__ __launch_bounds__(NT) void pp_resample_scan(const double* logw, int Kg, uint64_t* __restrict__ cdf, double* lse_out, int lse_stride,
                                                        int logz_R) {
@@ -281,6 +349,18 @@
     }
     if (!cdf) return;
     __syncthreads();
+    unsigned long long* out = reinterpret_cast<unsigned long long*>(cdf) + (size_t)g * Kg;
+    for (int k = threadIdx.x; k < Kg; k += NT) out[k] = lcdf[k];
+}
+template <int NT>
+__global__ __launch_bounds__(NT) void pp_resample_scan_anc(const double* logw, int Kg, uint64_t* __restrict__ cdf, double* lse_out, int lse_stride,
+                                                           const pp_anc_out ao) {
+    extern __shared__ __attribute__((aligned(16))) char smem[];
+    pp_scan_lds* sh = reinterpret_cast<pp_scan_lds*>(smem);
+    unsigned long long* lcdf = reinterpret_cast<unsigned long long*>(smem + ((sizeof(pp_scan_lds) + 15) & ~(size_t)15));
+    const int g = blockIdx.x;
+    pp_scan<NT>(logw + (size_t)g * Kg, Kg, lcdf, lse_out ? lse_out + (size_t)g * lse_stride : (double*)nullptr, sh, true);
+    pp_scan_ancestors<NT>(lcdf, Kg, g, ao, reinterpret_cast<unsigned char*>(lcdf + Kg), sh);
     unsigned long long* out = reinterpret_cast<unsigned long long*>(cdf) + (size_t)g * Kg;
     for (int k = threadIdx.x; k < Kg; k += NT) out[k] = lcdf[k];
 }
@@ -424,7 +504,9 @@
         if (lo + j < a.Kg) out[lo + j] = run + e[j];
 }
 #define PP_SCAN_KERNEL_MAX_KG 16384
-__host__ inline size_t pp_resample_scan_lds(int Kg) { return ((sizeof(pp_scan_lds) + 15) & ~(size_t)15) + (size_t)Kg * 8; }
+__host__ inline size_t pp_resample_scan_lds(int Kg, bool ancestors = false) {
+    return ((sizeof(pp_scan_lds) + 15) & ~(size_t)15) + (size_t)Kg * 8 + (ancestors ? ((size_t)Kg + 15) & ~(size_t)15 : 0);
+}
 
 template <bool STAGE>
 __device__ __forceinline__ void pp_part_a(const pp_args& a, int r, int kg, uint32_t kin, uint64_t seed, const pp_slot& L, int lane,
diff --git a/phylo_amd/csrc/phylo_sweep_plan.h b/phylo_amd/csrc/phylo_sweep_plan.h
--- a/phylo_amd/csrc/phylo_sweep_plan.h
+++ b/phylo_amd/csrc/phylo_sweep_plan.h
@@ -143,6 +143,26 @@
     return SCAN_IN_PLACE;
 }
 
+struct sweep_chain_form {
+    bool taken;
+    int item_waves;
+    int parts;
+};
+inline sweep_chain_form sweep_chain_form_of(const sweep_plan& p, int S, int multi_min, int scan_ancestors, const sweep_limits& L) {
+    const sweep_chain_form no{};
+    if (scan_ancestors == 0) return no;
+    if (!(p.use_rec && p.mat_after_book)) return no;
+    if (p.mat_barrier) return no;
+    if (p.R < 2) return no;
+    const sweep_scan_form s = sweep_scan_form_of(p.Kg, multi_min, true, L);
+    if (s != SCAN_LDS_512 && s != SCAN_LDS_1024) return no;
+    sweep_chain_form f{};
+    f.taken = true;
+    f.parts = (S + 127) / 128 < 8 ? (S + 127) / 128 : 8;
+    f.item_waves = p.Kg * f.parts < 128 ? p.Kg * f.parts : 128;
+    return f;
+}
+
 inline int sweep_plan_launches(const sweep_plan& p, int r) {
     if (r < 0) return 1;
     if (r >= p.R) return (p.fold_logz ? 0 : 1) + p.gather_launches;
```

After: 713.8 billion particle-site-likelihoods/s, median of 6. 1.06x the previous value.
